# Iamctb/ImageStitching

Measured on AMD Instinct MI355X. Metric: stitched megapixels/sec (9x12 MP vertical), higher is better.
Workload: dtype u8

## Files before the change

imagestitching_amd/__init__.py:

```python
from ._lib import (FILTER_BILINEAR, FILTER_NEAREST, HORIZONTAL, VERTICAL, StitchError, last_error)
from .stitch import (DEFAULT_OPTS, Bitmap, GroupJob, StitchGroup, Stitcher, StitchJob, StitchPlan, decode_files_device, decode_image, decode_png, encode_png, encode_png_batch_device, encode_png_device, encode_jpeg, encode_jpeg_device, encode_jpeg_batch_device, stitch_jpeg, stitch_jpeg_batch, image_info, last_phase_times, plan, set_phase_timing,
                     launch_jobs, stitch, stitch_batch, stitch_files, stitch_png, stitch_png_batch, decode_bitmaps, upload_bitmap, preview_device, preview_fit, thumbnail_layout, thumbnails, thumbnails_device, debug_cells, debug_png_grid, debug_jpeg_gpu_coefficients, scaled_size, decode_scale_fit, thumbnails_from_files, find_overlaps, find_overlaps_device, overlap_rows, crop_overlaps, image_color, icc_tables, convert_color_device)

__all__ = ["stitch", "stitch_batch", "launch_jobs", "stitch_png", "stitch_png_batch", "encode_png", "encode_png_device", "encode_png_batch_device", "encode_jpeg", "encode_jpeg_device", "stitch_jpeg", "decode_png", "decode_image", "decode_files_device", "image_info", "set_phase_timing", "last_phase_times", "stitch_files", "decode_bitmaps", "upload_bitmap", "preview_device", "preview_fit", "thumbnail_layout", "thumbnails", "thumbnails_device", "thumbnails_from_files", "find_overlaps", "find_overlaps_device", "overlap_rows", "crop_overlaps", "image_color", "icc_tables", "convert_color_device", "scaled_size", "decode_scale_fit", "debug_cells", "debug_png_grid", "debug_jpeg_gpu_coefficients", "Bitmap", "plan", "Stitcher", "StitchGroup", "GroupJob", "StitchJob", "StitchPlan", "StitchError",
           "DEFAULT_OPTS"]
```

imagestitching_amd/_lib.py:

```python
import ctypes as C
import os

import torch

_HERE = os.path.dirname(os.path.abspath(__file__))
LIB_PATH = os.path.join(_HERE, "libimagestitch.so")
if os.environ.get("IST_TUNING") == "1" and os.environ.get("IST_LIB_PATH"):
    LIB_PATH = os.environ["IST_LIB_PATH"]

VERTICAL, HORIZONTAL = 0, 1
MODE_MIN, MODE_MAX, MODE_ORIGINAL = 0, 1, 2
PLATFORM_OTHER, PLATFORM_IOS, PLATFORM_ANDROID = 0, 1, 2
FILTER_NEAREST, FILTER_BILINEAR, FILTER_AREA, FILTER_CUBIC = 0, 1, 2, 3
PATH_FILL, PATH_COPY, PATH_SAMPLE, PATH_GENERAL, PATH_SAMPLE_LDS, PATH_SWAP_LDS, PATH_SAMPLE_STREAM, PATH_AREA_STREAM, PATH_CUBIC_STREAM = range(9)
SPLIT_IMAGE, SPLIT_BAND, SPLIT_ROWS, SPLIT_AUTO = 0, 1, 2, 3
THUMB_FILL, THUMB_FIT = 0, 1
TURN_FLIP_X, TURN_FLIP_Y, TURN_TRANSPOSE = 1, 2, 4

IST_OK, IST_NOTHING_TO_DO = 0, 1
ERROR_NAMES = {-1: "IST_E_INVALID", -2: "IST_E_SIZE_UNAVAILABLE", -3: "IST_E_OUTPUT_SIZE", -4: "IST_E_NO_CONTEXT",
               -5: "IST_E_NO_DEVICE", -6: "IST_E_DECODE", -7: "IST_E_UNSUPPORTED", -8: "IST_E_NOMEM", -9: "IST_E_HIP"}


class ImageDesc(C.Structure):
    _fields_ = [("width", C.c_int32), ("height", C.c_int32), ("orientation", C.c_int32),
                ("bmp_width", C.c_int32), ("bmp_height", C.c_int32), ("opaque", C.c_int32),
                ("file_size", C.c_int64)]


class Limits(C.Structure):
    _fields_ = [("platform", C.c_int32), ("reserved", C.c_int32), ("max_side", C.c_double),
                ("max_pixels", C.c_double), ("max_super_sample", C.c_double)]


class Rect(C.Structure):
    _fields_ = [("image", C.c_int32), ("orientation", C.c_int32),
                ("dx", C.c_double), ("dy", C.c_double), ("dw", C.c_double), ("dh", C.c_double)]


class Plan(C.Structure):
    _fields_ = [("out_w", C.c_double), ("out_h", C.c_double), ("scale_down", C.c_double),
                ("super_sample", C.c_double), ("canvas_w", C.c_int64), ("canvas_h", C.c_int64),
                ("big_task", C.c_int32), ("n_rects", C.c_int32), ("rects", C.POINTER(Rect))]


class Op(C.Structure):
    _fields_ = [("kind", C.c_int32), ("image", C.c_int32), ("m", C.c_double * 6), ("s", C.c_double * 4),
                ("d", C.c_double * 4), ("rgba", C.c_uint8 * 4), ("reserved", C.c_int32)]


class Region(C.Structure):
    _fields_ = [("x", C.c_int32), ("y", C.c_int32), ("w", C.c_int32), ("h", C.c_int32)]


class Part(C.Structure):
    _fields_ = [("image", C.c_int32), ("op", C.c_int32), ("slot", C.c_int32),
                ("X0", C.c_int32), ("Y0", C.c_int32), ("X1", C.c_int32), ("Y1", C.c_int32),
                ("sx0", C.c_int32), ("sy0", C.c_int32), ("sx1", C.c_int32), ("sy1", C.c_int32), ("in_place", C.c_int32)]


class FlatCell(C.Structure):
    _fields_ = [("path", C.c_int32), ("image", C.c_int32), ("X0", C.c_int32), ("Y0", C.c_int32), ("X1", C.c_int32), ("Y1", C.c_int32),
                ("src_offset", C.c_int64), ("bg", C.c_uint32), ("opaque", C.c_int32)]


class DebugCell(C.Structure):
    _fields_ = [("path", C.c_int32), ("tile_w", C.c_int32), ("tile_h", C.c_int32), ("sub_h", C.c_int32),
                ("X0", C.c_int32), ("Y0", C.c_int32), ("X1", C.c_int32), ("Y1", C.c_int32), ("tiles", C.c_int64)]


class StitchRequest(C.Structure):
    _fields_ = [("images", C.POINTER(ImageDesc)), ("src", C.POINTER(C.c_void_p)), ("src_pitch", C.POINTER(C.c_size_t)),
                ("n_images", C.c_int32), ("direction", C.c_int32), ("mode", C.c_int32), ("gap", C.c_double),
                ("limits", C.POINTER(Limits)), ("filter", C.c_int32), ("reserved", C.c_int32)]


class JobInfo(C.Structure):
    _fields_ = [("canvas_w", C.c_int64), ("canvas_h", C.c_int64), ("n_ops", C.c_int32), ("n_cells", C.c_int32),
                ("n_tiles", C.c_int64), ("out_pixels", C.c_int64), ("src_pixels_touched", C.c_int64),
                ("algorithmic_bytes", C.c_int64), ("tiles_fill", C.c_int64), ("tiles_copy", C.c_int64),
                ("tiles_sample", C.c_int64), ("tiles_general", C.c_int64)]


class Preview(C.Structure):
    _fields_ = [("box_w", C.c_double), ("box_h", C.c_double), ("width", C.c_int32), ("height", C.c_int32),
                ("pixels", C.POINTER(C.c_uint8))]


class ThumbSpec(C.Structure):
    _fields_ = [("cell_w", C.c_int32), ("cell_h", C.c_int32), ("mode", C.c_int32), ("apply_orientation", C.c_int32)]


class ThumbItem(C.Structure):
    _fields_ = [("width", C.c_int32), ("height", C.c_int32), ("src_x", C.c_int32), ("src_y", C.c_int32), ("src_w", C.c_int32),
                ("src_h", C.c_int32), ("turn", C.c_int32), ("reserved", C.c_int32), ("offset", C.c_int64)]


class OverlapOpts(C.Structure):
    _fields_ = [("tolerance", C.c_int32), ("min_rows", C.c_int32), ("min_informative", C.c_int32), ("reserved", C.c_int32)]


class Overlap(C.Structure):
    _fields_ = [("header", C.c_int32), ("footer", C.c_int32), ("overlap", C.c_int32), ("reserved", C.c_int32), ("cost", C.c_int64)]


class JpegCoefInfo(C.Structure):
    _fields_ = [("ok", C.c_int32), ("launches", C.c_int32), ("ncomp", C.c_int32), ("reserved", C.c_int32),
                ("blocks_x", C.c_int32 * 3), ("blocks_y", C.c_int32 * 3)]


class ColorTables(C.Structure):
    _fields_ = [("kind", C.c_int32), ("mq", (C.c_int32 * 3) * 3), ("dec", (C.c_uint16 * 256) * 3)]


COLOR_PROFILE_IGNORE, COLOR_PROFILE_SRGB = 0, 1
COLOR_NONE, COLOR_IDENTITY, COLOR_CONVERT, COLOR_UNSUPPORTED = 0, 1, 2, 3

SYMBOLS = [
    ("ist_abi_version", C.c_int, []),
    ("ist_last_error", C.c_char_p, []),
    ("ist_device_count", C.c_int, []),
    ("ist_debug_device_allocs", C.c_int64, []),
    ("ist_debug_live_handles", C.c_int, [C.POINTER(C.c_int64)]),
    ("ist_debug_gpu_entropy_files", C.c_int64, []),
    ("ist_debug_gpu_entropy_sync_launches", C.c_int64, []),
    ("ist_debug_jpeg_gpu_coefficients", C.c_int, [C.c_void_p, C.c_char_p, C.c_int64, C.POINTER(C.c_void_p), C.POINTER(C.c_int64), C.POINTER(JpegCoefInfo)]),
    ("ist_debug_direct_images", C.c_int64, []),
    ("ist_debug_host_sink_stitches", C.c_int64, []),
    ("ist_debug_flat_launches", C.c_int64, []),
    ("ist_debug_duplex_stitches", C.c_int64, []),
    ("ist_debug_batch_launches", C.c_int64, []),
    ("ist_debug_png_batch_launches", C.c_int64, []),
    ("ist_limits_default", None, [C.c_int, C.POINTER(Limits)]),
    ("ist_limits_unlimited", None, [C.POINTER(Limits)]),
    ("ist_plan_compute", C.c_int, [C.POINTER(ImageDesc), C.c_int, C.c_int, C.c_int, C.c_double, C.POINTER(Limits), C.POINTER(Plan)]),
    ("ist_plan_free", None, [C.POINTER(Plan)]),
    ("ist_plan_ops", C.c_int, [C.POINTER(Plan), C.POINTER(ImageDesc), C.c_int, C.POINTER(Op), C.POINTER(C.c_int)]),
    ("ist_op_box", C.c_int, [C.POINTER(Op), C.c_int64, C.c_int64, C.c_int, C.POINTER(C.c_int32)]),
    ("ist_debug_flat_form", C.c_int, [C.c_int64, C.c_int64, C.POINTER(C.c_uint8), C.POINTER(Op), C.c_int, C.POINTER(ImageDesc), C.c_int, C.c_int,
                                      C.POINTER(Region), C.POINTER(C.c_int64), C.POINTER(C.c_int64), C.POINTER(FlatCell), C.c_int, C.POINTER(C.c_int)]),
    ("ist_debug_cells", C.c_int, [C.c_int64, C.c_int64, C.POINTER(C.c_uint8), C.POINTER(Op), C.c_int, C.POINTER(ImageDesc), C.c_int, C.c_int,
                                  C.POINTER(Region), C.POINTER(DebugCell), C.c_int, C.POINTER(C.c_int), C.POINTER(C.c_int), C.POINTER(C.c_int)]),
    ("ist_shard_parts", C.c_int, [C.POINTER(Op), C.c_int, C.c_int64, C.c_int64, C.POINTER(ImageDesc), C.c_int, C.c_int, C.c_int, C.c_int,
                                  C.POINTER(Part), C.c_int, C.POINTER(C.c_int)]),
    ("ist_shard_row_cuts", C.c_int, [C.c_int64, C.c_int, C.POINTER(C.c_int32)]),
    ("ist_shard_resolve", C.c_int, [C.POINTER(Op), C.c_int, C.c_int64, C.c_int64, C.POINTER(ImageDesc), C.c_int, C.c_int, C.c_int]),
    ("ist_ctx_create", C.c_void_p, [C.c_int]),
    ("ist_ctx_destroy", None, [C.c_void_p]),
    ("ist_ctx_sync", C.c_int, [C.c_void_p]),
    ("ist_ctx_set_png_level", C.c_int, [C.c_void_p, C.c_int]),
    ("ist_ctx_set_png_color", C.c_int, [C.c_void_p, C.c_int]),
    ("ist_ctx_set_png_filter", C.c_int, [C.c_void_p, C.c_int]),
    ("ist_ctx_set_png_match", C.c_int, [C.c_void_p, C.c_int]),
    ("ist_job_create", C.c_void_p, [C.c_void_p, C.c_int64, C.c_int64, C.POINTER(C.c_uint8), C.POINTER(Op), C.c_int,
                                    C.POINTER(ImageDesc), C.c_int, C.c_int, C.POINTER(Region)]),
    ("ist_job_info_get", C.c_int, [C.c_void_p, C.POINTER(JobInfo)]),
    ("ist_job_preferred_dst_pitch", C.c_size_t, [C.c_void_p]),
    ("ist_job_launch", C.c_int, [C.c_void_p, C.POINTER(C.c_void_p), C.POINTER(C.c_size_t), C.c_int, C.c_void_p, C.c_size_t, C.c_void_p]),
    ("ist_jobs_launch", C.c_int, [C.POINTER(C.c_void_p), C.c_int, C.POINTER(C.c_void_p), C.POINTER(C.c_size_t), C.POINTER(C.c_int),
                                  C.POINTER(C.c_void_p), C.POINTER(C.c_size_t), C.c_void_p]),
    ("ist_job_destroy", None, [C.c_void_p]),
    ("ist_group_create", C.c_void_p, [C.POINTER(C.c_int), C.c_int]),
    ("ist_group_destroy", None, [C.c_void_p]),
    ("ist_group_slots", C.c_int, [C.c_void_p]),
    ("ist_group_device", C.c_int, [C.c_void_p, C.c_int]),
    ("ist_group_job_create", C.c_void_p, [C.c_void_p, C.c_int64, C.c_int64, C.POINTER(C.c_uint8), C.POINTER(Op), C.c_int,
                                          C.POINTER(ImageDesc), C.c_int, C.c_int, C.c_int]),
    ("ist_group_job_destroy", None, [C.c_void_p]),
    ("ist_group_job_parts", C.c_int, [C.c_void_p, C.POINTER(Part), C.c_int, C.POINTER(C.c_int)]),
    ("ist_group_job_launch", C.c_int, [C.c_void_p, C.POINTER(C.c_void_p), C.POINTER(C.c_size_t), C.c_int, C.c_void_p, C.c_size_t]),
    ("ist_group_sync", C.c_int, [C.c_void_p]),
    ("ist_group_stitch_rgba8", C.c_int, [C.c_void_p, C.POINTER(ImageDesc), C.POINTER(C.c_void_p), C.POINTER(C.c_size_t), C.c_int,
                                         C.c_int, C.c_int, C.c_double, C.POINTER(Limits), C.c_int, C.c_int, C.POINTER(Plan),
                                         C.POINTER(C.POINTER(C.c_uint8))]),
    ("ist_stitch_rgba8_multi", C.c_int, [C.POINTER(C.c_int), C.c_int, C.POINTER(ImageDesc), C.POINTER(C.c_void_p), C.POINTER(C.c_size_t), C.c_int,
                                         C.c_int, C.c_int, C.c_double, C.POINTER(Limits), C.c_int, C.c_int, C.POINTER(Plan),
                                         C.POINTER(C.POINTER(C.c_uint8))]),
    ("ist_stitch_rgba8", C.c_int, [C.c_void_p, C.POINTER(ImageDesc), C.POINTER(C.c_void_p), C.POINTER(C.c_size_t), C.c_int,
                                   C.c_int, C.c_int, C.c_double, C.POINTER(Limits), C.c_int, C.POINTER(Plan),
                                   C.POINTER(C.POINTER(C.c_uint8))]),
    ("ist_stitch_rgba8_batch", C.c_int, [C.c_void_p, C.POINTER(StitchRequest), C.c_int, C.POINTER(Plan), C.POINTER(C.POINTER(C.c_uint8))]),
    ("ist_stitch_png_batch", C.c_int, [C.c_void_p, C.POINTER(StitchRequest), C.c_int, C.POINTER(Plan), C.POINTER(C.POINTER(C.c_uint8)),
                                       C.POINTER(C.c_int64)]),
    ("ist_render_rgba8", C.c_int, [C.c_void_p, C.c_int64, C.c_int64, C.POINTER(C.c_uint8), C.POINTER(Op), C.c_int,
                                   C.POINTER(ImageDesc), C.POINTER(C.c_void_p), C.POINTER(C.c_size_t), C.c_int, C.c_int,
                                   C.POINTER(Region), C.c_void_p, C.c_size_t]),
    ("ist_free", None, [C.c_void_p]),
    ("ist_pool_trim", None, []),
    ("ist_png_info", C.c_int, [C.c_void_p, C.c_int64, C.POINTER(C.c_int32), C.POINTER(C.c_int32)]),
    ("ist_png_decode_rgba8", C.c_int, [C.c_void_p, C.c_int64, C.c_void_p, C.c_size_t, C.c_int64]),
    ("ist_jpeg_info", C.c_int, [C.c_void_p, C.c_int64, C.POINTER(C.c_int32), C.POINTER(C.c_int32), C.POINTER(C.c_int32)]),
    ("ist_jpeg_decode_rgba8", C.c_int, [C.c_void_p, C.c_void_p, C.c_int64, C.c_void_p, C.c_size_t, C.c_int64]),
    ("ist_image_info", C.c_int, [C.c_void_p, C.c_int64, C.POINTER(C.c_int32), C.POINTER(C.c_int32), C.POINTER(C.c_int32)]),
    ("ist_image_decode_rgba8", C.c_int, [C.c_void_p, C.c_void_p, C.c_int64, C.c_void_p, C.c_size_t, C.c_int64]),
    ("ist_decode_files_device", C.c_int, [C.c_void_p, C.POINTER(C.c_char_p), C.POINTER(C.c_int64), C.c_int, C.POINTER(C.c_void_p), C.POINTER(C.c_size_t),
                                          C.POINTER(C.c_int64), C.POINTER(ImageDesc)]),
    ("ist_jpeg_scaled_size", C.c_int, [C.c_int32, C.c_int32, C.c_int32, C.POINTER(C.c_int32), C.POINTER(C.c_int32)]),
    ("ist_decode_scale_fit", C.c_int, [C.c_int32, C.c_int32, C.c_int32, C.c_int32]),
    ("ist_image_decode_rgba8_scaled", C.c_int, [C.c_void_p, C.c_void_p, C.c_int64, C.c_int32, C.c_void_p, C.c_size_t, C.c_int64]),
    ("ist_decode_files_device_scaled", C.c_int, [C.c_void_p, C.POINTER(C.c_char_p), C.POINTER(C.c_int64), C.c_int, C.POINTER(C.c_int32),
                                                 C.POINTER(C.c_void_p), C.POINTER(C.c_size_t), C.POINTER(C.c_int64), C.POINTER(ImageDesc)]),
    ("ist_debug_jpeg_scaled_launches", C.c_int64, []),
    ("ist_ctx_set_timing", C.c_int, [C.c_void_p, C.c_int]),
    ("ist_ctx_last_timing", C.c_int, [C.c_void_p, C.POINTER(C.c_double), C.c_int]),
    ("ist_stitch_files_png", C.c_int, [C.c_void_p, C.POINTER(C.c_char_p), C.POINTER(C.c_int64), C.c_int, C.c_int, C.c_int, C.c_double,
                                       C.POINTER(Limits), C.c_int, C.POINTER(Plan), C.POINTER(C.POINTER(C.c_uint8)), C.POINTER(C.c_int64)]),
    ("ist_stitch_paths_png", C.c_int, [C.c_void_p, C.POINTER(C.c_char_p), C.c_int, C.c_int, C.c_int, C.c_double,
                                       C.POINTER(Limits), C.c_int, C.POINTER(Plan), C.POINTER(C.POINTER(C.c_uint8)), C.POINTER(C.c_int64)]),
    ("ist_png_bound", C.c_int64, [C.c_int64, C.c_int64]),
    ("ist_png_encode_device", C.c_int, [C.c_void_p, C.c_void_p, C.c_size_t, C.c_int64, C.c_int64, C.c_void_p, C.c_int64,
                                        C.POINTER(C.c_int64), C.c_void_p]),
    ("ist_png_encode_batch_device", C.c_int, [C.c_void_p, C.POINTER(C.c_void_p), C.POINTER(C.c_size_t), C.POINTER(C.c_int64), C.POINTER(C.c_int64),
                                              C.c_int, C.POINTER(C.c_void_p), C.POINTER(C.c_int64), C.POINTER(C.c_int64), C.c_void_p]),
    ("ist_png_encode_rgba8", C.c_int, [C.c_void_p, C.c_void_p, C.c_size_t, C.c_int64, C.c_int64,
                                       C.POINTER(C.POINTER(C.c_uint8)), C.POINTER(C.c_int64)]),
    ("ist_render_png", C.c_int, [C.c_void_p, C.c_int64, C.c_int64, C.POINTER(C.c_uint8), C.POINTER(Op), C.c_int,
                                 C.POINTER(ImageDesc), C.POINTER(C.c_void_p), C.POINTER(C.c_size_t), C.c_int, C.c_int,
                                 C.POINTER(C.POINTER(C.c_uint8)), C.POINTER(C.c_int64)]),
    ("ist_stitch_png", C.c_int, [C.c_void_p, C.POINTER(ImageDesc), C.POINTER(C.c_void_p), C.POINTER(C.c_size_t), C.c_int,
                                 C.c_int, C.c_int, C.c_double, C.POINTER(Limits), C.c_int, C.POINTER(Plan),
                                 C.POINTER(C.POINTER(C.c_uint8)), C.POINTER(C.c_int64)]),
    ("ist_bitmap_upload", C.c_void_p, [C.c_void_p, C.POINTER(ImageDesc), C.c_void_p, C.c_size_t]),
    ("ist_bitmaps_decode", C.c_int, [C.c_void_p, C.POINTER(C.c_char_p), C.POINTER(C.c_int64), C.c_int, C.POINTER(C.c_void_p)]),
    ("ist_bitmaps_decode_scaled", C.c_int, [C.c_void_p, C.POINTER(C.c_char_p), C.POINTER(C.c_int64), C.c_int, C.POINTER(C.c_int32), C.POINTER(C.c_void_p)]),
    ("ist_bitmap_desc", C.c_int, [C.c_void_p, C.POINTER(ImageDesc)]),
    ("ist_bitmap_download", C.c_int, [C.c_void_p, C.c_void_p, C.c_size_t, C.c_int64]),
    ("ist_bitmap_retain", None, [C.c_void_p]),
    ("ist_bitmap_release", None, [C.c_void_p]),
    ("ist_stitch_bitmaps_rgba8", C.c_int, [C.c_void_p, C.POINTER(C.c_void_p), C.c_int, C.c_int, C.c_int, C.c_double, C.POINTER(Limits), C.c_int,
                                           C.POINTER(Plan), C.POINTER(C.POINTER(C.c_uint8))]),
    ("ist_stitch_bitmaps_png", C.c_int, [C.c_void_p, C.POINTER(C.c_void_p), C.c_int, C.c_int, C.c_int, C.c_double, C.POINTER(Limits), C.c_int,
                                         C.POINTER(Plan), C.POINTER(C.POINTER(C.c_uint8)), C.POINTER(C.c_int64)]),
    ("ist_debug_bitmap_bytes", C.c_int64, []),
    ("ist_preview_fit", C.c_int, [C.c_int64, C.c_int64, C.c_double, C.c_double, C.POINTER(C.c_int32), C.POINTER(C.c_int32)]),
    ("ist_preview_device", C.c_int, [C.c_void_p, C.c_void_p, C.c_size_t, C.c_int64, C.c_int64, C.c_int, C.c_void_p, C.c_size_t,
                                     C.c_int32, C.c_int32, C.c_void_p]),
    ("ist_stitch_png_preview", C.c_int, [C.c_void_p, C.POINTER(ImageDesc), C.POINTER(C.c_void_p), C.POINTER(C.c_size_t), C.c_int,
                                         C.c_int, C.c_int, C.c_double, C.POINTER(Limits), C.c_int, C.POINTER(Plan),
                                         C.POINTER(C.POINTER(C.c_uint8)), C.POINTER(C.c_int64), C.POINTER(Preview)]),
    ("ist_stitch_bitmaps_png_preview", C.c_int, [C.c_void_p, C.POINTER(C.c_void_p), C.c_int, C.c_int, C.c_int, C.c_double, C.POINTER(Limits), C.c_int,
                                                 C.POINTER(Plan), C.POINTER(C.POINTER(C.c_uint8)), C.POINTER(C.c_int64), C.POINTER(Preview)]),
    ("ist_stitch_files_png_preview", C.c_int, [C.c_void_p, C.POINTER(C.c_char_p), C.POINTER(C.c_int64), C.c_int, C.c_int, C.c_int, C.c_double,
                                               C.POINTER(Limits), C.c_int, C.POINTER(Plan), C.POINTER(C.POINTER(C.c_uint8)), C.POINTER(C.c_int64),
                                               C.POINTER(Preview)]),
    ("ist_stitch_paths_png_preview", C.c_int, [C.c_void_p, C.POINTER(C.c_char_p), C.c_int, C.c_int, C.c_int, C.c_double,
                                               C.POINTER(Limits), C.c_int, C.POINTER(Plan), C.POINTER(C.POINTER(C.c_uint8)), C.POINTER(C.c_int64),
                                               C.POINTER(Preview)]),
    ("ist_bitmap_preview", C.c_int, [C.c_void_p, C.c_void_p, C.c_int32, C.c_int32, C.c_void_p, C.c_size_t]),
    ("ist_debug_preview_launches", C.c_int64, []),
    ("ist_debug_preview_geometry", C.c_int, [C.c_int64, C.c_int64, C.c_int32, C.c_int32, C.POINTER(C.c_int32)]),
    ("ist_debug_png_grid", C.c_int, [C.c_int64, C.c_int64, C.c_int, C.POINTER(C.c_int64)]),
    ("ist_thumb_layout", C.c_int, [C.POINTER(ImageDesc), C.c_int, C.POINTER(ThumbSpec), C.POINTER(ThumbItem), C.POINTER(C.c_int64)]),
    ("ist_thumbs_device", C.c_int, [C.c_void_p, C.POINTER(ImageDesc), C.POINTER(C.c_void_p), C.POINTER(C.c_size_t), C.c_int, C.POINTER(ThumbSpec),
                                    C.c_void_p, C.c_int64, C.POINTER(ThumbItem), C.c_void_p]),
    ("ist_bitmaps_thumbs", C.c_int, [C.c_void_p, C.POINTER(C.c_void_p), C.c_int, C.POINTER(ThumbSpec), C.POINTER(ThumbItem),
                                     C.POINTER(C.POINTER(C.c_uint8))]),
    ("ist_debug_thumb_launches", C.c_int64, []),
    ("ist_jpeg_quant_tables", C.c_int, [C.c_int, C.POINTER(C.c_uint8), C.POINTER(C.c_uint8)]),
    ("ist_jpeg_bound", C.c_int64, [C.c_int64, C.c_int64, C.c_int]),
    ("ist_jpeg_encode_device", C.c_int, [C.c_void_p, C.c_void_p, C.c_size_t, C.c_int64, C.c_int64, C.c_int, C.c_int, C.c_void_p, C.c_int64,
                                         C.POINTER(C.c_int64), C.c_void_p]),
    ("ist_jpeg_encode_rgba8", C.c_int, [C.c_void_p, C.c_void_p, C.c_size_t, C.c_int64, C.c_int64, C.c_int, C.c_int,
                                        C.POINTER(C.POINTER(C.c_uint8)), C.POINTER(C.c_int64)]),
    ("ist_stitch_jpeg", C.c_int, [C.c_void_p, C.POINTER(ImageDesc), C.POINTER(C.c_void_p), C.POINTER(C.c_size_t), C.c_int,
                                  C.c_int, C.c_int, C.c_double, C.POINTER(Limits), C.c_int, C.c_int, C.c_int, C.POINTER(Plan),
                                  C.POINTER(C.POINTER(C.c_uint8)), C.POINTER(C.c_int64)]),
    ("ist_stitch_bitmaps_jpeg", C.c_int, [C.c_void_p, C.POINTER(C.c_void_p), C.c_int, C.c_int, C.c_int, C.c_double, C.POINTER(Limits), C.c_int,
                                          C.c_int, C.c_int, C.POINTER(Plan), C.POINTER(C.POINTER(C.c_uint8)), C.POINTER(C.c_int64)]),
    ("ist_debug_jpeg_encode_launches", C.c_int64, []),
    ("ist_jpeg_batch_layout", C.c_int64, [C.POINTER(C.c_int64), C.POINTER(C.c_int64), C.POINTER(C.c_int), C.c_int, C.c_int64, C.c_void_p, C.c_int64]),
    ("ist_jpeg_encode_batch_device", C.c_int, [C.c_void_p, C.POINTER(C.c_void_p), C.POINTER(C.c_size_t), C.POINTER(C.c_int64), C.POINTER(C.c_int64),
                                               C.POINTER(C.c_int), C.POINTER(C.c_int), C.c_int, C.POINTER(C.c_void_p), C.POINTER(C.c_int64),
                                               C.POINTER(C.c_int64), C.c_void_p]),
    ("ist_stitch_jpeg_batch", C.c_int, [C.c_void_p, C.POINTER(StitchRequest), C.c_int, C.POINTER(C.c_int), C.POINTER(C.c_int), C.POINTER(Plan),
                                        C.POINTER(C.POINTER(C.c_uint8)), C.POINTER(C.c_int64)]),
    ("ist_debug_jpeg_batch_launches", C.c_int64, []),
    ("ist_jpeg_optimal_table", C.c_int, [C.POINTER(C.c_int64), C.POINTER(C.c_uint8), C.POINTER(C.c_uint8), C.POINTER(C.c_int)]),
    ("ist_debug_jpeg_histogram_launches", C.c_int64, []),
    ("ist_debug_jpeg_counts", C.c_int, [C.c_void_p, C.POINTER(C.c_int64), C.c_int64]),
# ... 46 lines not shown
```

imagestitching_amd/csrc/ist_ctx.h:

```cpp
#ifndef IST_CTX_H_
#define IST_CTX_H_

#include <hip/hip_runtime_api.h>

#include <atomic>
#include <memory>
#include <mutex>
#include <vector>

#include "ist_jpeg.h"

#include "ist_device.h"
#include "ist_host.h"
#include "ist_internal.h"
#include "ist_launch.h"

struct ist_ctx {
  int device = 0;
  ist::DevBuf scratch_src;
  ist::DevBuf scratch_dst;
  ist::DevBuf scratch_dec;
  ist::DevBuf scratch_huff;
  ist::DevBuf scratch_png;
  ist::DevBuf scratch_file;
  ist::DevBuf scratch_jpg;
  ist::DevBuf scratch_jpg_counts;
  ist::DevBuf scratch_arena;
  ist::DevBuf scratch_ent;
  std::vector<ist::Event> img_event;
  std::vector<ist::DevBuf> img_huff;
  std::unique_ptr<ist::WorkerPool> workers;
  std::vector<ist::ScanBuf> scan_bufs;
  std::vector<ist::ScanBuf> file_bufs;
  ist::Event render_done;
  static constexpr int kTablePool = 32;
  std::vector<ist::DevBuf> table_pool;
  std::mutex table_mu;
  std::mutex mu;
  std::atomic<uint32_t> settings{ist::kDefaultSettings};
  std::unique_ptr<ist::Stager> stager;
  double last_ms[IST_PHASE_COUNT] = {0, 0, 0, 0, 0, 0, 0, 0};
  struct LastUse : ist::Event { ~LastUse() { if (e) (void)hipEventSynchronize(e); } };
  static constexpr int kBatchRing = 4;
  struct BatchSlot { ist::PinnedBuf host; ist::DevBuf dev; bool pending = false; LastUse done; };
  BatchSlot batch_ring[kBatchRing];
  int batch_next = 0;
  std::mutex batch_mu;
  struct BatchHalf {
    ist::DevBuf tab, src, dst;
    ist::DevBuf file;
    ist::Event kernel_done;
    ist::Event read_done;
  };
  BatchHalf batch_half[2];
  ist::DevBuf scratch_prev;
  LastUse prev_done; bool prev_pending = false; hipStream_t prev_last = nullptr;
  ist_job* prev_job = nullptr;
  int64_t prev_job_key[5] = {0, 0, 0, 0, 0};
  std::mutex prev_mu;
  ist::DevBuf prev_out;
  ist::Event prev_ready;
  ist::DevBuf scratch_ovl;
  ist::PinnedBuf ovl_host;
  int64_t ovl_rows = 0;
  size_t ovl_sig_at = 0;
  ist::Stream stream;
  ist::Stream aux;
  ist::Stream render;
  ist::Stream png2;
  ist::Stream prev_stream;
  std::vector<ist::Stream> img_stream;
  std::vector<hipStream_t> streams() const {
    std::vector<hipStream_t> v;
    for (const ist::Stream* s : {&stream, &aux, &render, &png2, &prev_stream}) if (*s) v.push_back(*s);
    for (const ist::Stream& s : img_stream) v.push_back(s);
    return v;
  }
};

namespace ist {
inline Settings settings_of(const ist_ctx* ctx) { return ctx ? settings_unpack(ctx->settings.load(std::memory_order_relaxed)) : Settings{}; }
struct DevTables {
  DevOp* ops = nullptr;
  DevCell* cells = nullptr;
  DevBand* bands = nullptr;
  int32_t* stacks = nullptr;
  DevTile* tiles = nullptr;
};
}

struct ist_job {
  ist_ctx* ctx = nullptr;
  ist::Compiled host;
  std::unique_ptr<ist::FlatTwin> flat;
  ist::DevTables flat_dt;
  ist::DevBuf d_tables;
  static constexpr int kStreams = 4;
  hipStream_t launched_on[kStreams] = {nullptr, nullptr, nullptr, nullptr};
  int n_launched_on = 0;
  bool launched = false, launched_many = false;
  std::mutex launch_mu;
  ist::DevTables dt;
  int max_image = -1;
};

#define IST_HIP(expr) do { const hipError_t e_ = (expr); if (e_ != hipSuccess) return ist::fail(IST_E_HIP, std::string(#expr) + ": " + hipGetErrorString(e_)); } while (0)
#define IST_HIP_OR(expr, msg) do { if ((expr) != hipSuccess) { (void)hipGetLastError(); return ist::fail(IST_E_HIP, msg); } } while (0)

namespace ist {

inline size_t arena_take(size_t* off, size_t bytes) { const size_t at = *off; *off += round256(bytes); return at; }

ist_job* job_compile(ist_ctx* ctx, int64_t canvas_w, int64_t canvas_h, const uint8_t clear_rgba[4], const ist_op* ops, int n_ops,
                     const ist_image_desc* images, int n_images, int filter, const ist_region* clip);
struct TableLayout { size_t bytes[2][5] = {}; size_t at[2][5] = {}; const void* from[2][5] = {}; size_t total = 0; };
TableLayout table_layout(const ist_job& job);
void pack_tables(const TableLayout& L, uint8_t* blob);
void point_tables(ist_job* job, const TableLayout& L, uint8_t* base);
int job_launch_args(const ist_job* job, const void* const* src, const size_t* src_pitch, int n_images, void* dst, size_t dst_pitch,
                    LaunchArgs* out, const Compiled** out_run, bool* out_flat);
void note_launch_stream(ist_job* job, void* stream);
void count_flat_launches(int64_t n);

int batch_take_slot(ist_ctx* ctx, size_t bytes, ist_ctx::BatchSlot** out);

inline Stager& stager_of(ist_ctx* ctx) { if (!ctx->stager) ctx->stager.reset(new Stager(ctx->device)); return *ctx->stager; }
inline WorkerPool& workers_of(ist_ctx* ctx) { if (!ctx->workers) ctx->workers.reset(new WorkerPool()); return *ctx->workers; }
int ensure_aux(ist_ctx* ctx);
int ensure_render(ist_ctx* ctx);
int read_back_pooled(const void* dev, size_t bytes, hipStream_t stream, uint8_t** out);
int png_to_host(ist_ctx* ctx, const PngForm& form, const void* canvas, size_t pitch, int64_t w, int64_t h, void* dfile, uint8_t** out_png, int64_t* out_len,
                const std::function<int(int64_t, void*)>& need_rows = nullptr, int64_t slab_rows_hint = 0, ist_preview* preview = nullptr);

int jpeg_to_host(ist_ctx* ctx, const void* canvas, size_t pitch, int64_t w, int64_t h, int quality, int subsampling, uint8_t** out_jpeg,
                 int64_t* out_len);
int jpeg_check_options(const char* who, int quality, int subsampling);
int jpeg_check_export(const char* who, int64_t w, int64_t h, int quality, int subsampling);

int preview_check(ist_preview* pv);
inline void preview_clear(ist_preview* pv) { if (pv) { pv->width = pv->height = 0; pv->pixels = nullptr; } }
int preview_enqueue(ist_ctx* ctx, const void* src, size_t src_pitch, int64_t w, int64_t h, bool opaque, void* dst, size_t dst_pitch,
                    int32_t pw, int32_t ph, hipStream_t stream);
void bitmap_view(const ist_bitmap* b, int* device, const uint8_t** row0, size_t* pitch, ist_image_desc* desc);
int overlap_run(ist_ctx* ctx, const void* const* src, const size_t* pitch, const ist_image_desc* descs, int n, const ist_overlap_opts* opts,
                ist_overlap* out);
int overlap_check_desc(const ist_image_desc& d, int i);
struct PreviewTail {
  ist_ctx* ctx; const void* canvas; size_t pitch; int64_t w, h; ist_preview* pv;
  int32_t pw = 0, ph = 0;
  uint8_t* host = nullptr;
  bool queued = false;
  PreviewTail(ist_ctx* c, const void* cv, size_t p, int64_t w_, int64_t h_, ist_preview* v) : ctx(c), canvas(cv), pitch(p), w(w_), h(h_), pv(v) {}
  ~PreviewTail();
  int prepare();
  int queue(hipStream_t reader);
  int finish();
};

}

#endif
```

imagestitching_amd/csrc/ist_decode.cpp:

```cpp
#include <hip/hip_runtime_api.h>

#include <algorithm>
#include <atomic>
#include <chrono>
#include <cstdio>
#include <cstdlib>
#include <cstring>
#include <mutex>

#include "ist_decode.h"
#include "ist_webp.h"

using namespace ist;

namespace {
std::atomic<int64_t> g_gpu_entropy_files{0};
std::atomic<int64_t> g_gpu_entropy_sync_launches{0};

void jpeg_layout(const JpegImage& J, size_t* off, JpegDevLayout* L, int denom = 1) {
  std::memset(L, 0, sizeof(*L));
  for (int c = 0; c < J.ncomp; ++c) {
    const JpegComp& C = J.comp[c];
    const size_t nblk = static_cast<size_t>(C.blocks_x) * C.blocks_y;
    const size_t S = denom > 1 ? static_cast<size_t>(jpeg_scaled_idct_size(8 / denom, C.h, C.v, J.hmax, J.vmax)) : 8;
    L->coef[c] = arena_take(off, nblk * 128);
    L->q[c] = arena_take(off, 128);
    L->plane[c] = arena_take(off, nblk * S * S);
  }
}
void jpeg_layout_sparse(const JpegImage& J, size_t* off, JpegDevLayout* L) {
  for (int c = 0; c < J.ncomp; ++c) {
    const JpegComp& C = J.comp[c];
    if (!C.sparse) continue;
    const size_t nblk = static_cast<size_t>(C.blocks_x) * C.blocks_y;
    L->ent[c] = arena_take(off, C.ent.size() * 4 + 4); L->start[c] = arena_take(off, nblk * 4); L->cnt[c] = arena_take(off, nblk);
  }
}

JpegDeviceJob jpeg_device_job(const JpegImage& J, uint8_t* d, const JpegDevLayout& L, uint8_t* d_out, size_t out_pitch) {
  JpegDeviceJob job;
  job.width = J.width; job.height = J.height; job.ncomp = J.ncomp; job.hmax = J.hmax; job.vmax = J.vmax; job.rgb = J.rgb;
  for (int c = 0; c < 3; ++c) { job.d_coef[c] = nullptr; job.q_host[c] = nullptr; job.d_plane[c] = nullptr; job.h[c] = job.v[c] = 1; job.blocks_x[c] = job.blocks_y[c] = 0; }
  for (int c = 0; c < J.ncomp; ++c) {
    const JpegComp& C = J.comp[c];
    job.d_coef[c] = reinterpret_cast<int16_t*>(d + L.coef[c]);
    job.q_host[c] = C.q;
    job.d_plane[c] = d + L.plane[c];
    job.h[c] = C.h; job.v[c] = C.v; job.blocks_x[c] = C.blocks_x; job.blocks_y[c] = C.blocks_y;
  }
  job.out = d_out; job.out_pitch = out_pitch;
  return job;
}

int jpeg_enqueue(const JpegImage& J, uint8_t* d, uint8_t* d_ent, const JpegDevLayout& L, uint8_t* d_out, size_t out_pitch, hipStream_t stream, bool coef_on_device = false,
                 bool chroma_done = false, int denom = 1) {
  JpegDeviceJob job = jpeg_device_job(J, d, L, d_out, out_pitch);
  job.chroma_done = chroma_done; job.denom = denom;
  for (int c = 0; c < J.ncomp; ++c) {
    const JpegComp& C = J.comp[c];
    const size_t nblk = static_cast<size_t>(C.blocks_x) * C.blocks_y;
    int16_t* d_coef = reinterpret_cast<int16_t*>(d + L.coef[c]);
    if (coef_on_device) {
    } else if (C.sparse) {
      IST_HIP(hipMemsetAsync(d_coef, 0, nblk * 128, stream));
      if (!d_ent) return fail(IST_E_INVALID, "JPEG sparse coefficients without a device arena");
      if (!C.ent.empty()) IST_HIP(hipMemcpyAsync(d_ent + L.ent[c], C.ent.data(), C.ent.size() * 4, hipMemcpyHostToDevice, stream));
      IST_HIP(hipMemcpyAsync(d_ent + L.start[c], C.start.data(), nblk * 4, hipMemcpyHostToDevice, stream));
      IST_HIP(hipMemcpyAsync(d_ent + L.cnt[c], C.cnt.data(), nblk, hipMemcpyHostToDevice, stream));
      const int rc = jpeg_launch_scatter(reinterpret_cast<const uint32_t*>(d_ent + L.ent[c]), reinterpret_cast<const uint32_t*>(d_ent + L.start[c]), d_ent + L.cnt[c], d_coef, static_cast<int>(nblk), stream);
      if (rc) return rc;
    } else {
      if (C.coef.size() != nblk * 64) return fail(IST_E_DECODE, "JPEG component without coefficients");
      IST_HIP(hipMemcpyAsync(d_coef, C.coef.data(), nblk * 128, hipMemcpyHostToDevice, stream));
    }
  }
  return denom > 1 ? jpeg_launch_reconstruct_scaled(job, stream) : jpeg_launch_reconstruct(job, stream);
}

bool valid_denom(int d) { return d == 1 || d == 2 || d == 4 || d == 8; }

int jpeg_decode_rgba8(const char* who, ist_ctx* ctx, const uint8_t* file, int64_t len, int denom, uint8_t* out, size_t out_pitch, int64_t out_rows) {
  if (!ctx) return fail(IST_E_NO_CONTEXT, "无法获取绘图上下文");
  JpegImage J;
  int rc = jpeg_parse_and_entropy_decode(file, len, &J, false);
  if (rc) return rc;
  int sw = J.width, sh = J.height;
  jpeg_scaled_size(J.width, J.height, denom, &sw, &sh);
  if (!out || out_pitch < static_cast<size_t>(sw) * 4 || out_rows < sh) return fail(IST_E_INVALID, std::string(who) + ": output buffer too small");
  const bool to_srgb = settings_of(ctx).color_profile == IST_COLOR_PROFILE_SRGB;
  std::lock_guard<std::mutex> lock(ctx->mu);
  DeviceGuard g(ctx->device);
  size_t off = 0;
  JpegDevLayout L;
  jpeg_layout(J, &off, &L, denom);
  jpeg_layout_sparse(J, &off, &L);
  const size_t row = static_cast<size_t>(sw) * 4;
  const size_t o_out = arena_take(&off, row * sh);
  uint8_t* d = nullptr;
  rc = ctx->scratch_arena.grow(off);
  if (rc) return rc;
  d = static_cast<uint8_t*>(ctx->scratch_arena.p);
  rc = jpeg_enqueue(J, d, d, L, d + o_out, row, ctx->stream, false, false, denom);
  if (rc) return rc;
  if (to_srgb) {
    ist_color_tables t;
    if (image_color_tables(file, len, &t) == IST_COLOR_CONVERT) { rc = launch_color_convert(d + o_out, row, sw, sh, t, ctx->stream); if (rc) return rc; }
  }
  std::vector<RowsCopy> down{RowsCopy{d + o_out, nullptr, out, out_pitch, row, static_cast<size_t>(sh)}};
  rc = stager_of(ctx).download(down, ctx->stream);
  (void)hipStreamSynchronize(ctx->stream);
  return rc;
}

bool is_jpeg(const uint8_t* f, int64_t n) { return f && n >= 2 && f[0] == 0xFF && f[1] == 0xD8; }
bool is_misc(const uint8_t* f, int64_t n) { return f && n >= 4 && ((f[0] == 'B' && f[1] == 'M') || !std::memcmp(f, "GIF8", 4)); }
}

extern "C" {

int ist_jpeg_info(const uint8_t* file, int64_t len, int32_t* width, int32_t* height, int32_t* orientation) {
  JpegImage J;
  const int rc = jpeg_parse_and_entropy_decode(file, len, &J, true);
  if (rc) return rc;
  if (width) *width = J.width;
  if (height) *height = J.height;
  if (orientation) *orientation = J.orientation;
  return IST_OK;
}

int ist_jpeg_decode_rgba8(ist_ctx* ctx, const uint8_t* file, int64_t len, uint8_t* out, size_t out_pitch, int64_t out_rows) {
  return jpeg_decode_rgba8("ist_jpeg_decode_rgba8", ctx, file, len, 1, out, out_pitch, out_rows);
}

int ist_misc_info(const uint8_t* file, int64_t len, int32_t* w, int32_t* h);
int ist_misc_decode_rgba8(const uint8_t* file, int64_t len, uint8_t* out, size_t pitch, int64_t out_rows);

int ist_image_info(const uint8_t* file, int64_t len, int32_t* width, int32_t* height, int32_t* orientation) {
  if (is_jpeg(file, len)) return ist_jpeg_info(file, len, width, height, orientation);
  if (is_webp(file, len)) return webp_info(file, len, width, height, orientation);
  if (orientation) *orientation = 0;
  if (is_misc(file, len)) return ist_misc_info(file, len, width, height);
  return ist_png_info(file, len, width, height);
}

int ist_image_decode_rgba8(ist_ctx* ctx, const uint8_t* file, int64_t len, uint8_t* out, size_t out_pitch, int64_t out_rows) {
  if (is_jpeg(file, len)) return ist_jpeg_decode_rgba8(ctx, file, len, out, out_pitch, out_rows);
  if (is_misc(file, len)) return ist_misc_decode_rgba8(file, len, out, out_pitch, out_rows);
  if (is_webp(file, len)) return webp_decode_rgba8(file, len, out, out_pitch, out_rows);
  return ist_png_decode_rgba8(file, len, out, out_pitch, out_rows);
}

int ist_image_decode_rgba8_scaled(ist_ctx* ctx, const uint8_t* file, int64_t len, int32_t denom, uint8_t* out, size_t out_pitch, int64_t out_rows) {
  if (!valid_denom(denom)) return fail(IST_E_INVALID, "ist_image_decode_rgba8_scaled: the file's denominator " + std::to_string(denom) + " is not 1, 2, 4 or 8");
  if (is_jpeg(file, len)) return jpeg_decode_rgba8("ist_image_decode_rgba8_scaled", ctx, file, len, denom, out, out_pitch, out_rows);
  return ist_image_decode_rgba8(ctx, file, len, out, out_pitch, out_rows);
}

int ist_jpeg_scaled_size(int32_t w, int32_t h, int32_t denom, int32_t* sw, int32_t* sh) {
  if (w < 1 || h < 1 || !valid_denom(denom) || !sw || !sh) return fail(IST_E_INVALID, "ist_jpeg_scaled_size: bad argument");
  int a = 0, b = 0;
  jpeg_scaled_size(w, h, denom, &a, &b);
  *sw = a; *sh = b;
  return IST_OK;
}

int ist_decode_scale_fit(int32_t w, int32_t h, int32_t min_w, int32_t min_h) {
  if (w < 1 || h < 1 || min_w < 1 || min_h < 1) return fail(IST_E_INVALID, "ist_decode_scale_fit: bad argument");
  for (int d = 8; d > 1; d /= 2)
    if ((static_cast<int64_t>(w) + d - 1) / d >= min_w && (static_cast<int64_t>(h) + d - 1) / d >= min_h) return d;
  return 1;
}

}

namespace ist {

Phases::Phases(ist_ctx* c, bool timing) : ctx(c), record(timing) {
  static const bool env = std::getenv("IST_TIMING") != nullptr;
  print = env; on = env || record;
  if (record) for (double& v : c->last_ms) v = 0.0;
  t_prev = std::chrono::steady_clock::now();
}
void Phases::lap(int phase, const char* what, hipStream_t st) {
  if (!on) return;
  if (st) (void)hipStreamSynchronize(st);
  const auto t = std::chrono::steady_clock::now();
  const double ms = std::chrono::duration<double, std::milli>(t - t_prev).count();
  if (print) std::fprintf(stderr, "[ist timing] %-28s %8.2f ms\n", what, ms);
  if (record && phase >= 0 && phase < IST_PHASE_COUNT) ctx->last_ms[phase] += ms;
  t_prev = t;
}

constexpr int kImgStreams = 8;

static int ensure_image_lanes(ist_ctx* ctx, int n) {
  const size_t want = static_cast<size_t>(std::min(n, kImgStreams));
  while (ctx->img_stream.size() < want) {
    Stream st;
    const int rc = st.ensure();
    if (rc) return rc;
    ctx->img_stream.push_back(std::move(st));
  }
  while (ctx->img_event.size() < static_cast<size_t>(n)) {
    Event ev;
    const int rc = ev.ensure();
    if (rc) return rc;
    ctx->img_event.push_back(std::move(ev));
  }
  if (ctx->img_huff.size() < static_cast<size_t>(n)) ctx->img_huff.resize(static_cast<size_t>(n));
  if (ctx->scan_bufs.size() < static_cast<size_t>(n)) ctx->scan_bufs.resize(static_cast<size_t>(n));
  return IST_OK;
}

FileDecoder::FileDecoder(ist_ctx* ctx, const uint8_t* const* files, const int64_t* lens, int n, Phases* ph, int color_profile, const int32_t* denom)
    : ctx_(ctx), files_(files), lens_(lens), n_(n), ph_(ph), to_srgb_(color_profile == IST_COLOR_PROFILE_SRGB), denom_(denom), dec_(static_cast<size_t>(n)),
      on_gpu_(static_cast<size_t>(n), 0), taken_(static_cast<size_t>(n), 0), uploaded_(static_cast<size_t>(n), 0), started_(static_cast<size_t>(n), 0),
      chroma_done_(static_cast<size_t>(n), 0), jo_(static_cast<size_t>(n)) {}
FileDecoder::~FileDecoder() {
  join_all();
  for (int i = 0; i < n_; ++i) if (started_[static_cast<size_t>(i)]) (void)hipStreamSynchronize(stream_of(i));
  for (int i = 0; i < n_ && static_cast<size_t>(i) < ctx_->scan_bufs.size(); ++i) {
    ScanBuf& mine = dec_[static_cast<size_t>(i)].G.stream;
    if (mine.capacity() > ctx_->scan_bufs[static_cast<size_t>(i)].capacity() && mine.capacity() <= (8u << 20)) ctx_->scan_bufs[static_cast<size_t>(i)].swap(mine);
  }
}

int FileDecoder::headers() {
  static const bool gpu_huffman = std::getenv("IST_JPEG_HOST_HUFFMAN") == nullptr;
  gpu_huffman_ = gpu_huffman;
  for (int i = 0; i < n_; ++i) {
    Dec& D = dec_[static_cast<size_t>(i)];
    const uint8_t* f = files_[i]; const int64_t len = lens_[i];
    D.jpeg = is_jpeg(f, len);
    int rc;
    if (D.jpeg) {
      rc = jpeg_parse_and_entropy_decode(f, len, &D.J, true);
      D.w = D.J.width; D.h = D.J.height; D.orient = D.J.orientation;
    } else {
      int32_t w = 0, h = 0, o = 0;
      rc = ist_image_info(f, len, &w, &h, &o);
      D.w = w; D.h = h; D.orient = o;
    }
    if (rc != IST_OK) return fail(rc, "图片" + std::to_string(i) + "解码异常: " + g_last_error);
  }
  return IST_OK;
}
std::vector<ist_image_desc> FileDecoder::descs(const int64_t* lens) const {
  std::vector<ist_image_desc> descs(static_cast<size_t>(n_));
  for (int i = 0; i < n_; ++i) {
    const Dec& D = dec(i);
    ist_image_desc& d = descs[static_cast<size_t>(i)];
    std::memset(&d, 0, sizeof d);
    d.width = D.w; d.height = D.h; d.orientation = D.orient ? D.orient : 1; d.opaque = D.jpeg ? 1 : 0; d.file_size = lens[i];
    if (denom_of(i) > 1) { int sw = 0, sh = 0; jpeg_scaled_size(D.w, D.h, denom_of(i), &sw, &sh); d.bmp_width = sw; d.bmp_height = sh; }
  }
  return descs;
}
void FileDecoder::layout(size_t* off) { for (int i = 0; i < n_; ++i) if (dec_[static_cast<size_t>(i)].jpeg) jpeg_layout(dec_[static_cast<size_t>(i)].J, off, &jo_[static_cast<size_t>(i)], denom_of(i)); }
int FileDecoder::denom_of(int i) const { return denom_ && dec_[static_cast<size_t>(i)].jpeg ? denom_[i] : 1; }

int FileDecoder::start(uint8_t* arena, uint8_t* const* img, const size_t* pitch) {
  arena_ = arena; img_ = img; pitch_ = pitch;
  const int rc = ensure_image_lanes(ctx_, n_);
  if (rc) return rc;
  workers_of(ctx_).run(n_, [this](int i) { worker(i); });
  running_ = true;
  if (!ph_->on) return IST_OK;
  join_all();
  int rc2 = first_error(); if (rc2) return rc2;
  for (int i = 0; i < n_; ++i) if (uploaded_[static_cast<size_t>(i)]) (void)hipStreamSynchronize(stream_of(i));
  ph_->lap(IST_PHASE_HOST_DECODE, "decode on host threads (+ scan uploads)", nullptr);
  rc2 = huffman_all(ctx_->stream); if (rc2) return rc2;
  ph_->lap(IST_PHASE_ENTROPY_GPU, "entropy decode (GPU)", ctx_->stream);
  for (int i = 0; i < n_; ++i) { rc2 = take(i, ctx_->stream); if (rc2) return rc2; }
  ph_->lap(IST_PHASE_RECONSTRUCT, "H2D + JPEG reconstruct (GPU)", ctx_->stream);
  return IST_OK;
}

int FileDecoder::take(int i, hipStream_t consumer) {
  const size_t k = static_cast<size_t>(i);
  if (taken_[k]) return IST_OK;
  int rc = huffman_all(consumer);
  if (rc) return rc;
  rc = chroma_all(consumer);
  if (rc) return rc;
  taken_[k] = 1;
  rc = place(i, consumer);
  if (rc) return rc;
  const Dec& D = dec_[k];
  if (!to_srgb_ || D.color.kind != IST_COLOR_CONVERT) return IST_OK;
  int bw = D.w, bh = D.h;
  if (denom_of(i) > 1) jpeg_scaled_size(D.w, D.h, denom_of(i), &bw, &bh);
  return launch_color_convert(img_[i], pitch_[i], bw, bh, D.color, consumer);
}

int FileDecoder::place(int i, hipStream_t consumer) {
  const size_t k = static_cast<size_t>(i);
  int rc = IST_OK;
  Dec& D = dec_[k];
  if (on_gpu_[k]) return jpeg_enqueue(D.J, arena_, nullptr, jo_[k], img_[i], pitch_[i], consumer, true, chroma_done_[k] != 0, denom_of(i));
  const size_t row = static_cast<size_t>(D.w) * 4;
  if (!D.jpeg) {
    std::vector<RowsCopy> up;
    if (pitch_[i] != row) for (int y = 0; y < D.h; ++y) up.push_back(RowsCopy{img_[i] + static_cast<size_t>(y) * pitch_[i], D.px.data() + static_cast<size_t>(y) * row, nullptr, row, row, 1});
    else up.push_back(RowsCopy{img_[i], D.px.data(), nullptr, row, row, static_cast<size_t>(D.h)});
    return stager_of(ctx_).upload(up, consumer);
  }
  if (D.G.eligible) {
    D.G.eligible = false;
    JpegImage host;
    rc = jpeg_parse_and_entropy_decode(files_[i], lens_[i], &host, false, nullptr);
    if (rc) return fail(rc, "图片" + std::to_string(i) + "解码异常: " + g_last_error);
    D.J = std::move(host);
  }
  size_t need = 0;
  JpegDevLayout L = jo_[k];
  jpeg_layout_sparse(D.J, &need, &L);
  if (need) {
    (void)hipStreamSynchronize(consumer);
    rc = ctx_->scratch_ent.grow(need, need / 2);
    if (rc) return rc;
  }
  return jpeg_enqueue(D.J, arena_, static_cast<uint8_t*>(ctx_->scratch_ent.p), L, img_[i], pitch_[i], consumer, false, false, denom_of(i));
}

int FileDecoder::finish(hipStream_t consumer) {
  for (int i = 0; i < n_; ++i) { const int rc = take(i, consumer); if (rc) { join_all(); return rc; } }
  return IST_OK;
}
int FileDecoder::gpu_decoded() const { int g = 0; for (char v : on_gpu_) g += v ? 1 : 0; return g; }

hipStream_t FileDecoder::stream_of(int i) const { return ctx_->img_stream[static_cast<size_t>(i % kImgStreams) % ctx_->img_stream.size()]; }
void FileDecoder::join_all() { if (running_) { ctx_->workers->wait(); running_ = false; } }
int FileDecoder::first_error() {
  for (int i = 0; i < n_; ++i) if (dec_[static_cast<size_t>(i)].rc != IST_OK) return fail(dec_[static_cast<size_t>(i)].rc, "图片" + std::to_string(i) + "解码异常: " + dec_[static_cast<size_t>(i)].err);
  return IST_OK;
}
int FileDecoder::huffman_all(hipStream_t consumer) {
  if (huff_done_) return IST_OK;
  tl_mark("decoder: waiting for the per-image host work");
  join_all();
  tl_mark("decoder: host work of every image done");
  int rc = first_error();
  if (rc) return rc;
  huff_done_ = true;
  std::vector<JpegGpuItem> items; std::vector<int> who;
  for (int i = 0; i < n_; ++i) {
    const size_t k = static_cast<size_t>(i);
    Dec& D = dec_[k];
    if (!D.jpeg || !D.G.eligible) continue;
    JpegGpuItem it; it.J = &D.J; it.S = &D.G;
    for (int c = 0; c < 3; ++c) it.d_coef[c] = c < D.J.ncomp ? reinterpret_cast<int16_t*>(arena_ + jo_[k].coef[c]) : nullptr;
    if (uploaded_[k]) {
      it.d_stream = static_cast<const uint8_t*>(ctx_->img_huff[k].p);
      IST_HIP_OR(hipStreamWaitEvent(consumer, ctx_->img_event[k], 0), "hipStreamWaitEvent failed");
    }
    items.push_back(it); who.push_back(i);
  }
  std::vector<uint8_t> okv;
  int launches = 0;
  rc = jpeg_gpu_entropy_decode(items, &okv, consumer, &ctx_->scratch_huff, &launches);
  g_gpu_entropy_sync_launches.fetch_add(launches, std::memory_order_relaxed);
  if (rc) return rc;
  for (size_t q = 0; q < who.size(); ++q) {
    on_gpu_[static_cast<size_t>(who[q])] = okv[q] ? 1 : 0;
    if (okv[q]) g_gpu_entropy_files.fetch_add(1, std::memory_order_relaxed);
  }
  return IST_OK;
}
int FileDecoder::chroma_all(hipStream_t consumer) {
  if (chroma_batch_done_) return IST_OK;
  chroma_batch_done_ = true;
  std::vector<JpegDeviceJob> chroma;
  for (int i = 0; i < n_; ++i) {
    const size_t k = static_cast<size_t>(i);
    if (!on_gpu_[k] || dec_[k].J.ncomp != 3 || denom_of(i) > 1) continue;
    chroma.push_back(jpeg_device_job(dec_[k].J, arena_, jo_[k], nullptr, 0));
    chroma_done_[k] = 1;
  }
  if (!chroma.empty()) return jpeg_launch_chroma_idct(chroma.data(), static_cast<int>(chroma.size()), consumer);
  return IST_OK;
}
void FileDecoder::worker(int i) {
  const size_t k = static_cast<size_t>(i);
  Dec& D = dec_[k];
  DeviceGuard dg(ctx_->device);
  const uint8_t* f = files_[i]; const int64_t len = lens_[i];
  auto failed = [&](int rc) { D.rc = rc; D.err = g_last_error; };
  if (to_srgb_) image_color_tables(f, len, &D.color);
  if (!D.jpeg) {
    D.px.resize(static_cast<size_t>(D.w) * D.h * 4);
    const int rc = ist_image_decode_rgba8(nullptr, f, len, D.px.data(), static_cast<size_t>(D.w) * 4, D.h);
    if (rc) failed(rc);
    return;
  }
  JpegImage full;
  if (k < ctx_->scan_bufs.size()) D.G.stream.swap(ctx_->scan_bufs[k]);
  static const bool flip = tuning_mode() && std::getenv("IST_JPEG_SECOND_READ_444") != nullptr;
  std::vector<uint8_t> flipped;
  if (flip) {
    flipped.assign(f, f + len);
    for (int64_t q = 2; q + 12 < len; ++q) if (flipped[static_cast<size_t>(q)] == 0xFF && flipped[static_cast<size_t>(q) + 1] == 0xC0) { flipped[static_cast<size_t>(q) + 11] = 0x11; break; }
    f = flipped.data();
  }
  const int rc = jpeg_parse_and_entropy_decode(f, len, &full, false, gpu_huffman_ ? &D.G : nullptr);
  if (rc) { failed(rc); return; }
  bool same = full.width == D.w && full.height == D.h && full.ncomp == D.J.ncomp && full.hmax == D.J.hmax && full.vmax == D.J.vmax &&
              full.mcus_x == D.J.mcus_x && full.mcus_y == D.J.mcus_y;
  for (int c = 0; same && c < full.ncomp; ++c)
    same = full.comp[c].h == D.J.comp[c].h && full.comp[c].v == D.J.comp[c].v && full.comp[c].blocks_x == D.J.comp[c].blocks_x &&
           full.comp[c].blocks_y == D.J.comp[c].blocks_y;
  if (!same) { g_last_error = "JPEG frame header changed between two reads"; failed(IST_E_DECODE); return; }
  D.J = std::move(full);
  if (!D.G.eligible) return;
  const size_t bytes = D.G.stream.size();
  if (ctx_->img_huff[k].grow(bytes, bytes / 4)) return;
  hipStream_t st = stream_of(i);
  started_[k] = 1;
  if (hipMemcpyAsync(ctx_->img_huff[k].p, D.G.stream.data(), bytes, hipMemcpyHostToDevice, st) != hipSuccess ||
      hipEventRecord(ctx_->img_event[k], st) != hipSuccess) { (void)hipGetLastError(); return; }
  uploaded_[k] = 1;
}

int check_denoms(const char* who, const int32_t* denom, int n) {
  for (int i = 0; denom && i < n; ++i)
    if (!valid_denom(denom[i])) return fail(IST_E_INVALID, std::string(who) + ": the denominator of image " + std::to_string(i) + " is " + std::to_string(denom[i]) + ", not 1, 2, 4 or 8");
  return IST_OK;
}

int decode_files_locked(ist_ctx* ctx, const uint8_t* const* files, const int64_t* lens, int n, const int32_t* denom,
                        const std::function<int(const std::vector<ist_image_desc>&, uint8_t**, size_t*)>& place) {
  DeviceGuard g(ctx->device);
  const Settings set = settings_of(ctx);
  Phases ph(ctx, set.timing);
  FileDecoder fd(ctx, files, lens, n, &ph, set.color_profile, denom);
  int rc = fd.headers();
  if (rc) return rc;
  const std::vector<ist_image_desc> descs = fd.descs(lens);
  std::vector<uint8_t*> img(static_cast<size_t>(n), nullptr);
  std::vector<size_t> pitch(static_cast<size_t>(n), 0);
  rc = place(descs, img.data(), pitch.data());
  if (rc) return rc;
  size_t off = 0;
  fd.layout(&off);
  rc = ctx->scratch_dec.grow(off ? off : 256);
  if (rc) return rc;
  ph.lap(IST_PHASE_PLAN_ARENA, "device arena", nullptr);
  rc = fd.start(static_cast<uint8_t*>(ctx->scratch_dec.p), img.data(), pitch.data());
  if (rc == IST_OK) rc = fd.finish(ctx->stream);
  if (hipStreamSynchronize(ctx->stream) != hipSuccess) { (void)hipGetLastError(); if (rc == IST_OK) rc = fail(IST_E_HIP, "hipStreamSynchronize failed"); }
  return rc;
}

}

extern "C" {

int64_t ist_debug_gpu_entropy_files(void) { return g_gpu_entropy_files.load(std::memory_order_relaxed); }
int64_t ist_debug_gpu_entropy_sync_launches(void) { return g_gpu_entropy_sync_launches.load(std::memory_order_relaxed); }

int ist_debug_jpeg_gpu_coefficients(ist_ctx* ctx, const uint8_t* file, int64_t len, int16_t* const* planes, const int64_t* plane_elems,
                                    ist_jpeg_coef_info* info) {
  if (!file || len <= 0 || !info || (planes && !plane_elems)) return fail(IST_E_INVALID, "ist_debug_jpeg_gpu_coefficients: bad argument");
  std::memset(info, 0, sizeof *info);
  JpegImage J;
  JpegGpuScan G;
  int rc = jpeg_parse_and_entropy_decode(file, len, &J, false, &G);
  if (rc) return rc;
  if (!G.eligible) return fail(IST_E_UNSUPPORTED, "ist_debug_jpeg_gpu_coefficients: not a file the GPU entropy decoder takes");
  info->ncomp = J.ncomp;
  for (int c = 0; c < J.ncomp; ++c) { info->blocks_x[c] = J.comp[c].blocks_x; info->blocks_y[c] = J.comp[c].blocks_y; }
  if (!planes) return IST_OK;
  size_t off = 0, o_coef[3] = {0, 0, 0}, nblk[3] = {0, 0, 0};
  for (int c = 0; c < J.ncomp; ++c) {
    nblk[c] = static_cast<size_t>(J.comp[c].blocks_x) * J.comp[c].blocks_y;
    if (!planes[c] || plane_elems[c] < 0 || static_cast<uint64_t>(plane_elems[c]) < nblk[c] * 64) return fail(IST_E_INVALID, "ist_debug_jpeg_gpu_coefficients: plane " + std::to_string(c) + " is too small");
    o_coef[c] = arena_take(&off, nblk[c] * 128);
  }
  if (!ctx) return fail(IST_E_NO_CONTEXT, "无法获取绘图上下文");
  std::lock_guard<std::mutex> lock(ctx->mu);
  DeviceGuard g(ctx->device);
  rc = ctx->scratch_arena.grow(off);
  if (rc) return rc;
  uint8_t* d = static_cast<uint8_t*>(ctx->scratch_arena.p);
  JpegGpuItem it; it.J = &J; it.S = &G;
  for (int c = 0; c < 3; ++c) it.d_coef[c] = c < J.ncomp ? reinterpret_cast<int16_t*>(d + o_coef[c]) : nullptr;
  std::vector<JpegGpuItem> items(1, it);
  std::vector<uint8_t> okv;
  int launches = 0;
  rc = jpeg_gpu_entropy_decode(items, &okv, ctx->stream, &ctx->scratch_huff, &launches);
  g_gpu_entropy_sync_launches.fetch_add(launches, std::memory_order_relaxed);
  if (rc) return rc;
  info->launches = launches;
  info->ok = !okv.empty() && okv[0] ? 1 : 0;
  if (info->ok)
    for (int c = 0; c < J.ncomp; ++c) IST_HIP(hipMemcpyAsync(planes[c], d + o_coef[c], nblk[c] * 128, hipMemcpyDeviceToHost, ctx->stream));
  IST_HIP(hipStreamSynchronize(ctx->stream));
  return IST_OK;
}

int ist_ctx_set_color_profile(ist_ctx* ctx, int profile) {
  if (!ctx) return fail(IST_E_NO_CONTEXT, "无法获取绘图上下文");
  return settings_set(&ctx->settings, kColorProfile, profile);
}

int ist_color_convert_device(ist_ctx* ctx, void* ptr, size_t pitch, int64_t w, int64_t h, const ist_color_tables* tables, void* stream) {
  if (!ctx) return fail(IST_E_NO_CONTEXT, "无法获取绘图上下文");
  if (!ptr || !tables || w < 1 || h < 1) return fail(IST_E_INVALID, "ist_color_convert_device: bad argument");
  if (pitch / 4 < static_cast<uint64_t>(w) || (pitch & 3) || (reinterpret_cast<uintptr_t>(ptr) & 3)) return fail(IST_E_INVALID, "ist_color_convert_device: a short or unaligned pitch, or an unaligned pointer");
  if (tables->kind == IST_COLOR_IDENTITY) return IST_OK;
  if (tables->kind != IST_COLOR_CONVERT) return fail(IST_E_INVALID, "ist_color_convert_device: the tables are neither IST_COLOR_CONVERT nor IST_COLOR_IDENTITY");
  DeviceGuard g(ctx->device);
  return launch_color_convert(static_cast<uint8_t*>(ptr), pitch, w, h, *tables, stream);
}

int ist_ctx_set_timing(ist_ctx* ctx, int on) {
  if (!ctx) return fail(IST_E_NO_CONTEXT, "无法获取绘图上下文");
  return settings_set(&ctx->settings, kTiming, on != 0);
}

int ist_ctx_last_timing(ist_ctx* ctx, double* ms, int n) {
  if (!ctx || !ms || n < 0) return fail(IST_E_INVALID, "ist_ctx_last_timing: bad argument");
  for (int k = 0; k < n; ++k) ms[k] = k < IST_PHASE_COUNT ? ctx->last_ms[k] : 0.0;
  return IST_OK;
}

int ist_decode_files_device_scaled(ist_ctx* ctx, const uint8_t* const* files, const int64_t* lens, int n_images, const int32_t* denom, void* const* dst,
                                   const size_t* dst_pitch, const int64_t* dst_rows, ist_image_desc* out_descs) {
  if (!ctx) return fail(IST_E_NO_CONTEXT, "无法获取绘图上下文");
  if (n_images <= 0) return IST_NOTHING_TO_DO;
  if (!files || !lens || !dst || !dst_pitch || !dst_rows) return fail(IST_E_INVALID, "ist_decode_files_device: NULL argument");
  if (n_images > kMaxImages) return fail(IST_E_UNSUPPORTED, "more than 128 images in one call");
  const int rc = check_denoms("ist_decode_files_device_scaled", denom, n_images);
  if (rc) return rc;
  std::lock_guard<std::mutex> lock(ctx->mu);
  return decode_files_locked(ctx, files, lens, n_images, denom, [&](const std::vector<ist_image_desc>& descs, uint8_t** img, size_t* pitch) -> int {
    for (int i = 0; i < n_images; ++i) {
      const ist_image_desc& D = descs[static_cast<size_t>(i)];
      const int bw = bitmap_w(D), bh = bitmap_h(D);
      if (!dst[i] || dst_pitch[i] < static_cast<size_t>(bw) * 4 || (dst_pitch[i] & 3) || dst_rows[i] < bh || (reinterpret_cast<uintptr_t>(dst[i]) & 3))
        return fail(IST_E_INVALID, "ist_decode_files_device: the buffer of image " + std::to_string(i) + " is too small for " + std::to_string(bw) + "x" + std::to_string(bh));
      img[i] = static_cast<uint8_t*>(dst[i]);
      pitch[i] = dst_pitch[i];
      if (out_descs) out_descs[i] = D;
    }
    return IST_OK;
  });
}

int ist_decode_files_device(ist_ctx* ctx, const uint8_t* const* files, const int64_t* lens, int n_images, void* const* dst,
                            const size_t* dst_pitch, const int64_t* dst_rows, ist_image_desc* out_descs) {
  return ist_decode_files_device_scaled(ctx, files, lens, n_images, nullptr, dst, dst_pitch, dst_rows, out_descs);
}

}
```

imagestitching_amd/csrc/ist_decode.h:

```cpp
#ifndef IST_DECODE_H_
#define IST_DECODE_H_

#include <chrono>
#include <functional>
#include <string>
#include <vector>

#include "ist_ctx.h"
#include "ist_icc.h"

namespace ist {

struct Dec { int rc = 0; std::string err; bool jpeg = false; JpegImage J; JpegGpuScan G; int w = 0, h = 0, orient = 0; std::vector<uint8_t> px;
             ist_color_tables color = {}; };

struct Phases {
  ist_ctx* ctx; bool record, print, on;
  std::chrono::steady_clock::time_point t_prev;
  Phases(ist_ctx* c, bool timing);
  void lap(int phase, const char* what, hipStream_t st);
};

struct JpegDevLayout { size_t coef[3], q[3], plane[3], ent[3], start[3], cnt[3]; };

class FileDecoder {
 public:
  FileDecoder(ist_ctx* ctx, const uint8_t* const* files, const int64_t* lens, int n, Phases* ph, int color_profile, const int32_t* denom = nullptr);
  ~FileDecoder();
  int headers();
  const Dec& dec(int i) const { return dec_[static_cast<size_t>(i)]; }
  std::vector<ist_image_desc> descs(const int64_t* lens) const;
  void layout(size_t* off);
  int start(uint8_t* arena, uint8_t* const* img, const size_t* pitch);
  int take(int i, hipStream_t consumer);
  int finish(hipStream_t consumer);
  int gpu_decoded() const;

 private:
  hipStream_t stream_of(int i) const;
  int denom_of(int i) const;
  void join_all();
  int first_error();
  int huffman_all(hipStream_t consumer);
  int chroma_all(hipStream_t consumer);
  void worker(int i);
  int place(int i, hipStream_t consumer);

  ist_ctx* ctx_; const uint8_t* const* files_; const int64_t* lens_; int n_; Phases* ph_; const bool to_srgb_; const int32_t* denom_;
  std::vector<Dec> dec_;
  bool running_ = false;
  std::vector<char> on_gpu_, taken_, uploaded_, started_, chroma_done_;
  std::vector<JpegDevLayout> jo_;
  uint8_t* arena_ = nullptr; uint8_t* const* img_ = nullptr; const size_t* pitch_ = nullptr;
  bool gpu_huffman_ = true, huff_done_ = false, chroma_batch_done_ = false;
};

int check_denoms(const char* who, const int32_t* denom, int n);
int decode_files_locked(ist_ctx* ctx, const uint8_t* const* files, const int64_t* lens, int n, const int32_t* denom,
                        const std::function<int(const std::vector<ist_image_desc>&, uint8_t**, size_t*)>& place);

}

#endif
```

imagestitching_amd/csrc/ist_jpeg.cpp:

```cpp
#include <cstdlib>
#include <cstring>
#include <new>
#include <vector>

#include "ist_internal.h"
#include "ist_icc.h"
#include "ist_jpeg.h"

#include <emmintrin.h>

namespace ist {

namespace {

const uint8_t kZigzag[64] = {0, 1, 8, 16, 9, 2, 3, 10, 17, 24, 32, 25, 18, 11, 4, 5, 12, 19, 26, 33, 40, 48,
                             41, 34, 27, 20, 13, 6, 7, 14, 21, 28, 35, 42, 49, 56, 57, 50, 43, 36, 29, 22,
                             15, 23, 30, 37, 44, 51, 58, 59, 52, 45, 38, 31, 39, 46, 53, 60, 61, 54, 47, 55, 62, 63};

struct Huff {
  bool present = false;
  uint8_t bits[17] = {0};
  uint8_t vals[256] = {0};
  int32_t maxcode[18];
  int32_t valptr[17];
// ... 121 lines not shown
    if (jfif) J->rgb = false;
    else if (adobe) J->rgb = adobe_transform == 0;
    else J->rgb = J->comp[0].id == 'R' && J->comp[1].id == 'G' && J->comp[2].id == 'B';
  };
  auto latch = [&](int c) -> bool {
    if (latched[c]) return true;
    if (!have_q[J->comp[c].tq]) return false;
    std::memcpy(J->comp[c].q, qt[J->comp[c].tq], sizeof J->comp[c].q);
    latched[c] = true;
    return true;
  };
  int64_t pos = 2;
  *J = JpegImage();
  while (pos + 4 <= n) {
    if (f[pos] != 0xFF) { ++pos; continue; }
    const int m = f[pos + 1];
    if (m == 0xFF) { ++pos; continue; }
    if (m == 0xD8 || m == 0x01 || (m >= 0xD0 && m <= 0xD7)) { pos += 2; continue; }
    if (m == 0xD9) break;
    const int64_t len = be16(f + pos + 2);
    if (len < 2 || pos + 2 + len > n) return fail(IST_E_DECODE, "truncated JPEG segment");
    const uint8_t* d = f + pos + 4; const int64_t dl = len - 2;
    if (m == 0xE1 && J->orientation == 0) J->orientation = exif_orientation(d, static_cast<size_t>(dl));
    else if (m == 0xE0 && dl >= 14 && std::memcmp(d, "JFIF\0", 5) == 0) jfif = true;
    else if (m == 0xEE && dl >= 12 && std::memcmp(d, "Adobe", 5) == 0) { adobe = true; adobe_transform = d[11]; }
    else if (m == 0xDB) {
      int64_t o = 0;
      while (o < dl) {
        const int pq = d[o] >> 4, tq = d[o] & 15; ++o;
        if (tq > 3 || o + (pq ? 128 : 64) > dl) return fail(IST_E_DECODE, "bad JPEG quantisation table");
        for (int i = 0; i < 64; ++i) { qt[tq][kZigzag[i]] = static_cast<uint16_t>(pq ? be16(d + o + 2 * i) : d[o + i]); }
        o += pq ? 128 : 64;
        have_q[tq] = true;
      }
    } else if (m == 0xC4) {
      int64_t o = 0;
      while (o + 17 <= dl) {
        const int tc = d[o] >> 4, th = d[o] & 15;
        if (tc > 1 || th > 3) return fail(IST_E_DECODE, "bad JPEG Huffman table");
        Huff& h = tc ? ac[th] : dc[th];
        int cnt = 0;
        for (int i = 1; i <= 16; ++i) { h.bits[i] = d[o + i]; cnt += h.bits[i]; }
        if (cnt > 256 || o + 17 + cnt > dl) return fail(IST_E_DECODE, "bad JPEG Huffman table");
        std::memcpy(h.vals, d + o + 17, static_cast<size_t>(cnt));
        h.present = true;
        if (!h.build()) return fail(IST_E_DECODE, "bad JPEG Huffman table");
        o += 17 + cnt;
      }
    } else if (m == 0xDD) { if (dl >= 2) restart_interval = static_cast<int>(be16(d)); }
    else if (m == 0xC0 || m == 0xC1 || m == 0xC2) {
      if (have_sof) return fail(IST_E_DECODE, "JPEG with more than one frame header");
      progressive = (m == 0xC2);
      if (dl < 6) return fail(IST_E_DECODE, "bad JPEG frame header");
      if (d[0] != 8) return fail(IST_E_UNSUPPORTED, "only 8-bit JPEG is supported");
      J->height = static_cast<int>(be16(d + 1)); J->width = static_cast<int>(be16(d + 3)); J->ncomp = d[5];
      if (J->width < 1 || J->height < 1) return fail(IST_E_DECODE, "bad JPEG size");
      if (J->ncomp != 1 && J->ncomp != 3) return fail(IST_E_UNSUPPORTED, "only greyscale and YCbCr JPEG are supported");
      if (dl < 6 + 3 * J->ncomp) return fail(IST_E_DECODE, "bad JPEG frame header");
      int hmax = 1, vmax = 1;
      for (int c = 0; c < J->ncomp; ++c) {
        JpegComp& C = J->comp[c];
        C.id = d[6 + 3 * c]; C.h = d[7 + 3 * c] >> 4; C.v = d[7 + 3 * c] & 15; C.tq = d[8 + 3 * c];
        if (C.h < 1 || C.h > 2 || C.v < 1 || C.v > 2 || C.tq > 3) return fail(IST_E_UNSUPPORTED, "JPEG sampling factors beyond 2 are not supported");
        hmax = std::max(hmax, C.h); vmax = std::max(vmax, C.v);
        for (int p = 0; p < c; ++p) if (J->comp[p].id == C.id) return fail(IST_E_DECODE, "JPEG frame names a component twice");
      }
      if (J->ncomp == 3 && (J->comp[1].h != 1 || J->comp[1].v != 1 || J->comp[2].h != 1 || J->comp[2].v != 1))
        return fail(IST_E_UNSUPPORTED, "unusual JPEG sampling layout (chroma must be 1x1)");
      if (J->ncomp == 1) { J->comp[0].h = J->comp[0].v = 1; hmax = vmax = 1; }
      colour_space();
      J->hmax = hmax; J->vmax = vmax;
      J->mcus_x = (J->width + 8 * hmax - 1) / (8 * hmax); J->mcus_y = (J->height + 8 * vmax - 1) / (8 * vmax);
      for (int c = 0; c < J->ncomp; ++c) {
        JpegComp& C = J->comp[c];
        C.blocks_x = J->mcus_x * C.h; C.blocks_y = J->mcus_y * C.v;
      }
      have_sof = true;
      if (header_only) return IST_OK;
    } else if (m >= 0xC3 && m <= 0xCF && m != 0xC4 && m != 0xC8 && m != 0xCC) return fail(IST_E_UNSUPPORTED, "this JPEG process (lossless / arithmetic) is not supported");
    else if (m == 0xDA) {
      if (!have_sof) return fail(IST_E_DECODE, "JPEG scan before frame header");
      if (J->scans == 0) colour_space();
      if (dl < 1) return fail(IST_E_DECODE, "bad JPEG scan header");
      const int ns = d[0];
      if (ns < 1 || ns > J->ncomp || dl < 1 + 2 * ns + 3) return fail(IST_E_DECODE, "bad JPEG scan header");
      int ci[3], td[3], ta[3];
      for (int s = 0; s < ns; ++s) {
        const int id = d[1 + 2 * s]; ci[s] = -1;
        for (int c = 0; c < J->ncomp; ++c) if (J->comp[c].id == id) ci[s] = c;
        if (ci[s] < 0) return fail(IST_E_DECODE, "JPEG scan names an unknown component");
        for (int p = 0; p < s; ++p) if (ci[p] == ci[s]) return fail(IST_E_DECODE, "JPEG scan names a component twice");
        td[s] = d[2 + 2 * s] >> 4; ta[s] = d[2 + 2 * s] & 15;
        if (td[s] > 3 || ta[s] > 3) return fail(IST_E_DECODE, "JPEG scan uses an undefined Huffman table");
      }
      const int Ss = d[1 + 2 * ns], Se = d[2 + 2 * ns], Ah = d[3 + 2 * ns] >> 4, Al = d[3 + 2 * ns] & 15;
      if (progressive) {
        if (Ss > Se || Se > 63 || Al > 13 || Ah > 13 || (Ss == 0 && Se != 0) || (Ss > 0 && ns != 1) || (Ah != 0 && Ah != Al + 1))
          return fail(IST_E_DECODE, "bad progressive JPEG scan parameters");
      } else if (Ss != 0 || Se != 63 || Ah != 0 || Al != 0) return fail(IST_E_DECODE, "bad JPEG scan parameters");
      const bool dc_scan = Ss == 0, need_ac = !progressive || !dc_scan, need_dc = dc_scan && Ah == 0;
      for (int s = 0; s < ns; ++s) {
        if ((need_dc && !dc[td[s]].present) || (need_ac && !ac[ta[s]].present)) return fail(IST_E_DECODE, "JPEG scan uses an undefined Huffman table");
      }
      int mcu_blocks = 0;
      for (int s2 = 0; s2 < ns; ++s2) mcu_blocks += J->comp[ci[s2]].h * J->comp[ci[s2]].v;
      int dc_ids[2] = {-1, -1}, ac_ids[2] = {-1, -1}, dc_local[4] = {0, 0, 0, 0}, ac_local[4] = {0, 0, 0, 0};
      bool two_tables = true;
      for (int s2 = 0; s2 < ns; ++s2) {
        auto local = [&](int (&ids)[2], int id) { for (int q = 0; q < 2; ++q) { if (ids[q] == id) return q; if (ids[q] < 0) { ids[q] = id; return q; } } return -1; };
        dc_local[s2] = local(dc_ids, td[s2]); ac_local[s2] = local(ac_ids, ta[s2]);
        if (dc_local[s2] < 0 || ac_local[s2] < 0) two_tables = false;
      }
      if (gs && !progressive && J->scans == 0 && ns == J->ncomp && two_tables && mcu_blocks <= 10 &&
          (f + n) - (d + dl) < (1ll << 28)) {
        for (int c = 0; c < J->ncomp; ++c)
          if (!latch(c)) return fail(IST_E_DECODE, "JPEG component uses an undefined quantisation table");
        gs->slots = 0;
        for (int s2 = 0; s2 < ns; ++s2) {
          const JpegComp& C = J->comp[ci[s2]];
          for (int k = 0; k < C.h * C.v; ++k) { gs->slot_comp[gs->slots] = static_cast<uint8_t>(ci[s2]); gs->slot_idx[gs->slots] = static_cast<uint8_t>(k); ++gs->slots; }
          gs->dc_tab[ci[s2]] = static_cast<uint8_t>(dc_local[s2]); gs->ac_tab[ci[s2]] = static_cast<uint8_t>(ac_local[s2]);
        }
        std::memset(&gs->tables, 0, sizeof gs->tables);
        for (int t = 0; t < 4; ++t) {
          const bool is_ac = t >= 2;
          const int id = is_ac ? ac_ids[t - 2] : dc_ids[t];
          if (id < 0) continue;
          const Huff& h = is_ac ? ac[id] : dc[id];
          const int look_bits = is_ac ? kJpegAcLookBits : kJpegDcLookBits;
          uint16_t* look = is_ac ? gs->tables.look_ac[t - 2] : gs->tables.look_dc[t];
          int code = 0, k = 0;
          for (int l = 1; l <= look_bits; ++l) {
            for (int i = 0; i < h.bits[l]; ++i, ++k, ++code) {
              const uint16_t e = static_cast<uint16_t>((l << 8) | h.vals[k]);
              uint16_t* at = look + (static_cast<size_t>(code) << (look_bits - l));
              std::fill(at, at + (size_t{1} << (look_bits - l)), e);
            }
            code <<= 1;
          }
          JpegHuffTail& o = gs->tables.tail[t];
          for (int q = 0; q < 8; ++q) {
            const int l = 9 + q;
            o.lim[q] = static_cast<uint32_t>(h.mincode[l] + h.bits[l]) << (16 - l);
            if (q < 7) o.vptr[q] = static_cast<uint8_t>(h.valptr[l + 1]);
          }
          std::memcpy(o.vals, h.vals, sizeof o.vals);
        }
        const uint8_t* q = d + dl; const uint8_t* qe = f + n;
        gs->iv.clear();
        const uint32_t total_mcus = static_cast<uint32_t>(J->mcus_x) * static_cast<uint32_t>(J->mcus_y);
        const uint32_t ri = static_cast<uint32_t>(restart_interval);
        const uint32_t n_iv = ri ? (total_mcus + ri - 1) / ri : 0;
        bool in_sequence = n_iv <= kMaxGpuIntervals;
        gs->stream.clear();
        if (in_sequence && !gs->stream.reserve(static_cast<size_t>(qe - q) + static_cast<size_t>(n_iv) * 272 + 32)) return fail(IST_E_NOMEM, "out of memory for the JPEG scan");
        uint8_t* const base = gs->stream.data();
        uint8_t* out = base;
        size_t iv_start = 0; uint32_t next_rst = 0;
        auto close_interval = [&]() {
          const uint32_t k = static_cast<uint32_t>(gs->iv.size());
          const size_t at = static_cast<size_t>(out - base);
          JpegGpuInterval I;
          I.byte_off = static_cast<uint32_t>(iv_start); I.mcu0 = k * ri; I.n_mcus = std::min(ri, total_mcus - k * ri);
          I.bits = static_cast<int64_t>(at - iv_start) * 8;
          gs->iv.push_back(I);
          size_t pad = (256 - at % 256) % 256;
          if (pad < 16) pad += 256;
          std::memset(out, 0, pad);
          out += pad;
          iv_start = at + pad;
        };
        const __m128i all_ff = _mm_set1_epi8(static_cast<char>(0xFF));
        while (in_sequence && q < qe) {
          while (q + 16 <= qe) {
            const __m128i v = _mm_loadu_si128(reinterpret_cast<const __m128i*>(q));
            _mm_storeu_si128(reinterpret_cast<__m128i*>(out), v);
            const int m = _mm_movemask_epi8(_mm_cmpeq_epi8(v, all_ff));
            if (m) { const int k = __builtin_ctz(static_cast<unsigned>(m)); q += k; out += k; break; }
            q += 16; out += 16;
          }
          if (q >= qe) break;
          if (*q != 0xFF) { *out++ = *q++; continue; }
          if (q + 1 < qe && q[1] == 0x00) { *out++ = 0xFF; q += 2; continue; }
          if (q + 1 < qe && q[1] == 0xFF) { q += 1; continue; }
          if (q + 1 < qe && q[1] >= 0xD0 && q[1] <= 0xD7) {
            if (!ri || q[1] != 0xD0 + next_rst || gs->iv.size() + 1 >= n_iv) { in_sequence = false; break; }
            close_interval();
            next_rst = (next_rst + 1) & 7u;
            q += 2;
            continue;
          }
          break;
        }
        if (in_sequence && ri) {
          close_interval();
          if (gs->iv.size() != n_iv) in_sequence = false;
        }
        if (in_sequence) {
          if (ri) {
            gs->bits = static_cast<int64_t>(out - base) * 8;
          } else {
            gs->bits = static_cast<int64_t>(out - base) * 8;
            std::memset(out, 0, 16);
            out += 16;
          }
          gs->stream.set_size(static_cast<size_t>(out - base));
          gs->eligible = true;
          pos = q - f;
          J->scans++;
          continue;
        }
        gs->stream.clear(); gs->iv.clear();
      }
      for (int s = 0; s < ns; ++s)
        if (!latch(ci[s])) return fail(IST_E_DECODE, "JPEG component uses an undefined quantisation table");
      for (int c = 0; c < J->ncomp; ++c) {
        JpegComp& C = J->comp[c];
        const size_t nblk = static_cast<size_t>(C.blocks_x) * C.blocks_y;
        if (progressive) {
          if (C.coef.empty() && !C.coef.alloc_zero(nblk * 64)) return fail(IST_E_NOMEM, "out of memory for the JPEG coefficients");
        } else if (!C.sparse) {
          C.sparse = true;
          C.start.assign(nblk, 0); C.cnt.assign(nblk, 0);
          C.ent.reserve(2 * static_cast<size_t>(n) + 1024);
        }
      }
      BitReader br; br.p = d + dl; br.end = f + n;
      int pred[3] = {0, 0, 0}, eobrun = 0;
      const bool interleaved = ns > 1;
      int mx, my;
      if (interleaved) { mx = J->mcus_x; my = J->mcus_y; }
      else {
        const JpegComp& C = J->comp[ci[0]];
        mx = (((J->width * C.h + J->hmax - 1) / J->hmax) + 7) / 8;
        my = (((J->height * C.v + J->vmax - 1) / J->vmax) + 7) / 8;
      }
      int until_restart = restart_interval, next_rst = 0;
      for (int y = 0; y < my; ++y) {
        for (int x = 0; x < mx; ++x) {
          if (restart_interval && until_restart == 0) {
            br.reset();
            while (br.p + 1 < br.end && !(br.p[0] == 0xFF && br.p[1] >= 0xD0 && br.p[1] <= 0xD7)) ++br.p;
            if (br.p + 1 >= br.end) return fail(IST_E_DECODE, "JPEG restart marker missing");
            if ((br.p[1] & 7) != next_rst) return fail(IST_E_DECODE, "JPEG restart markers out of order");
            br.p += 2; next_rst = (next_rst + 1) & 7;
            pred[0] = pred[1] = pred[2] = 0; eobrun = 0;
            until_restart = restart_interval;
          }
          for (int s = 0; s < ns; ++s) {
            JpegComp& C = J->comp[ci[s]];
            const int bh = interleaved ? C.h : 1, bv = interleaved ? C.v : 1;
            for (int by = 0; by < bv; ++by) for (int bx = 0; bx < bh; ++bx) {
              const int gx = x * bh + bx, gy = y * bv + by;
              const size_t bi = static_cast<size_t>(gy) * C.blocks_x + gx;
              int16_t* blk = progressive ? C.coef.data() + bi * 64 : nullptr;
              if (!progressive) {
                const size_t first = C.ent.size();
                C.ent.resize(first + 64);
                uint32_t* e = C.ent.data() + first;
                int t = decode_symbol(br, dc[td[s]]);
                if (t < 0 || t > 11) return fail(IST_E_DECODE, "corrupt JPEG entropy data (DC)");
                const int diff = t ? extend(br.get(t), t) : 0;
                pred[s] += diff;
                if (pred[s]) *e++ = static_cast<uint32_t>(static_cast<uint16_t>(static_cast<int16_t>(pred[s])));
                const Huff& hac = ac[ta[s]];
                for (int k = 1; k < 64;) {
                  const int fa = hac.fast_ac[br.peek(16) >> 7];
                  if (fa) {
                    k += (fa >> 4) & 15;
                    if (k > 63) return fail(IST_E_DECODE, "corrupt JPEG entropy data (run)");
                    br.skip(fa & 15);
                    *e++ = (static_cast<uint32_t>(kZigzag[k]) << 16) | static_cast<uint16_t>(static_cast<int16_t>(fa >> 8));
                    ++k;
                    continue;
                  }
                  const int rs = decode_symbol(br, hac);
                  if (rs < 0) return fail(IST_E_DECODE, "corrupt JPEG entropy data (AC)");
                  const int r = rs >> 4, sz = rs & 15;
                  if (sz == 0) { if (r == 15) { k += 16; continue; } break; }
                  k += r;
                  if (k > 63) return fail(IST_E_DECODE, "corrupt JPEG entropy data (run)");
                  const int v = extend(br.get(sz), sz);
                  if (v) *e++ = (static_cast<uint32_t>(kZigzag[k]) << 16) | static_cast<uint16_t>(static_cast<int16_t>(v));
                  ++k;
                }
                const size_t used = static_cast<size_t>(e - (C.ent.data() + first));
                C.ent.resize(first + used);
                C.start[bi] = static_cast<uint32_t>(first);
                C.cnt[bi] = static_cast<uint8_t>(used);
              } else if (dc_scan && Ah == 0) {
                const int t = decode_symbol(br, dc[td[s]]);
                if (t < 0 || t > 11) return fail(IST_E_DECODE, "corrupt JPEG entropy data (DC)");
                pred[s] += t ? extend(br.get(t), t) : 0;
                blk[0] = static_cast<int16_t>(pred[s] * (1 << Al));
              } else if (dc_scan) {
                if (br.get(1)) blk[0] = static_cast<int16_t>(blk[0] | (1 << Al));
              } else if (Ah == 0) {
                if (eobrun > 0) { --eobrun; continue; }
                for (int k = Ss; k <= Se;) {
                  const int rs = decode_symbol(br, ac[ta[s]]);
                  if (rs < 0) return fail(IST_E_DECODE, "corrupt JPEG entropy data (AC)");
                  const int r = rs >> 4, sz = rs & 15;
                  if (sz == 0) {
                    if (r == 15) { k += 16; continue; }
                    eobrun = (1 << r) - 1;
                    if (r) eobrun += static_cast<int>(br.get(r));
                    break;
                  }
                  k += r;
                  if (k > Se) return fail(IST_E_DECODE, "corrupt JPEG entropy data (run)");
                  blk[kZigzag[k]] = static_cast<int16_t>(extend(br.get(sz), sz) * (1 << Al));
                  ++k;
                }
              } else {
                const int p1 = 1 << Al, m1 = -(1 << Al);
                auto refine = [&](int16_t* c) {
                  if (br.get(1) && (*c & p1) == 0) *c = static_cast<int16_t>(*c + (*c >= 0 ? p1 : m1));
                };
                int k = Ss;
                if (eobrun == 0) {
                  for (; k <= Se; ++k) {
                    const int rs = decode_symbol(br, ac[ta[s]]);
                    if (rs < 0) return fail(IST_E_DECODE, "corrupt JPEG entropy data (AC)");
                    int r = rs >> 4, val = 0;
                    const int sz = rs & 15;
                    if (sz) {
                      if (sz != 1) return fail(IST_E_DECODE, "corrupt JPEG entropy data (refinement)");
                      val = br.get(1) ? p1 : m1;
                    } else if (r != 15) {
                      eobrun = 1 << r;
                      if (r) eobrun += static_cast<int>(br.get(r));
                      break;
                    }
                    for (; k <= Se; ++k) {
                      int16_t* c = blk + kZigzag[k];
                      if (*c != 0) refine(c);
                      else if (--r < 0) break;
                    }
                    if (val) {
                      if (k > Se) return fail(IST_E_DECODE, "corrupt JPEG entropy data (run)");
                      blk[kZigzag[k]] = static_cast<int16_t>(val);
                    }
                  }
                }
                if (eobrun > 0) {
                  for (; k <= Se; ++k) { int16_t* c = blk + kZigzag[k]; if (*c != 0) refine(c); }
                  --eobrun;
                }
              }
            }
          }
// ... 64 lines not shown
```

imagestitching_amd/csrc/ist_jpeg.h:

```cpp
#ifndef IST_JPEG_H_
#define IST_JPEG_H_

#include <cstdint>
#include <cstdlib>
#include <utility>
#include <vector>

namespace ist {

class CoefBuf {
 public:
  CoefBuf() = default;
  ~CoefBuf() { std::free(p_); }
  CoefBuf(const CoefBuf&) = delete;
  CoefBuf& operator=(const CoefBuf&) = delete;
  CoefBuf(CoefBuf&& o) noexcept : p_(o.p_), n_(o.n_) { o.p_ = nullptr; o.n_ = 0; }
  CoefBuf& operator=(CoefBuf&& o) noexcept { if (this != &o) { std::free(p_); p_ = o.p_; n_ = o.n_; o.p_ = nullptr; o.n_ = 0; } return *this; }
  bool alloc_zero(size_t n) { std::free(p_); p_ = static_cast<int16_t*>(std::calloc(n ? n : 1, sizeof(int16_t))); n_ = p_ ? n : 0; return p_ != nullptr; }
  bool empty() const { return n_ == 0; }
  size_t size() const { return n_; }
  int16_t* data() { return p_; }
  const int16_t* data() const { return p_; }
  const int16_t* begin() const { return p_; }
  const int16_t* end() const { return p_ + n_; }
 private:
  int16_t* p_ = nullptr; size_t n_ = 0;
};

struct JpegComp {
  int id = 0, h = 1, v = 1, tq = 0;
  int blocks_x = 0, blocks_y = 0;
  uint16_t q[64];
  CoefBuf coef;
  bool sparse = false;
  std::vector<uint32_t> ent, start;
  std::vector<uint8_t> cnt;
};

struct JpegImage {
  int width = 0, height = 0, ncomp = 0;
  int hmax = 1, vmax = 1, mcus_x = 0, mcus_y = 0;
  int orientation = 0;
  int scans = 0;
  bool rgb = false;
  JpegComp comp[3];
};

struct alignas(16) JpegHuffTail {
  uint32_t lim[8];
  uint8_t vptr[8];
  uint8_t pad_[8];
  uint8_t vals[256];
};
#ifndef IST_AC_LOOK_BITS
#define IST_AC_LOOK_BITS 9
#endif
constexpr int kJpegDcLookBits = 9, kJpegAcLookBits = IST_AC_LOOK_BITS;
struct alignas(16) JpegGpuTables {
  uint16_t look_dc[2][1 << kJpegDcLookBits];
  uint16_t look_ac[2][1 << kJpegAcLookBits];
  JpegHuffTail tail[4];
};
struct JpegGpuInterval { uint32_t byte_off, mcu0, n_mcus; int64_t bits; };
class ScanBuf {
 public:
  ScanBuf() = default;
  ~ScanBuf() { std::free(p_); }
  ScanBuf(const ScanBuf&) = delete;
  ScanBuf& operator=(const ScanBuf&) = delete;
  ScanBuf(ScanBuf&& o) noexcept { swap(o); }
  ScanBuf& operator=(ScanBuf&& o) noexcept { swap(o); return *this; }
  void swap(ScanBuf& o) noexcept { std::swap(p_, o.p_); std::swap(n_, o.n_); std::swap(cap_, o.cap_); }
  const uint8_t* data() const { return p_; }
  uint8_t* data() { return p_; }
  size_t size() const { return n_; }
  size_t capacity() const { return cap_; }
  bool empty() const { return n_ == 0; }
  void clear() { n_ = 0; }
  void set_size(size_t n) { n_ = n; }
  bool reserve(size_t want) {
    if (want <= cap_) return true;
    std::free(p_);
    p_ = static_cast<uint8_t*>(std::malloc(want)); cap_ = p_ ? want : 0; n_ = 0;
    return p_ != nullptr;
  }
 private:
  uint8_t* p_ = nullptr; size_t n_ = 0, cap_ = 0;
};
struct JpegGpuScan {
  bool eligible = false;
  std::vector<JpegGpuInterval> iv;
  ScanBuf stream;
  int64_t bits = 0;
  int slots = 0;
  uint8_t slot_comp[10], slot_idx[10];
  uint8_t dc_tab[3], ac_tab[3];
  JpegGpuTables tables;
};

int jpeg_parse_and_entropy_decode(const uint8_t* file, int64_t len, JpegImage* out, bool header_only, JpegGpuScan* gpu_scan = nullptr);

struct JpegDeviceJob {
  int width, height, ncomp, hmax, vmax;
  int h[3], v[3], blocks_x[3], blocks_y[3];
  const int16_t* d_coef[3];
  const uint16_t* q_host[3];
  uint8_t* d_plane[3];
  bool rgb = false;
  uint8_t* out; size_t out_pitch;
  bool chroma_done = false;
  int denom = 1;
};
inline void jpeg_scaled_size(int w, int h, int denom, int* sw, int* sh) {
  const int64_t N = 8 / denom;
  *sw = static_cast<int>((w * N + 7) / 8); *sh = static_cast<int>((h * N + 7) / 8);
}
inline int jpeg_scaled_idct_size(int N, int h, int v, int hmax, int vmax) {
  int S = N;
  while (S < 8 && (hmax * N) % (h * S * 2) == 0 && (vmax * N) % (v * S * 2) == 0) S *= 2;
  return S;
}
int jpeg_launch_reconstruct_scaled(const JpegDeviceJob& job, void* stream);
int jpeg_launch_reconstruct(const JpegDeviceJob& job, void* stream);
int jpeg_launch_chroma_idct(const JpegDeviceJob* jobs, int n_jobs, void* stream);
int jpeg_launch_scatter(const uint32_t* d_ent, const uint32_t* d_start, const uint8_t* d_cnt, int16_t* d_coef, int n_blocks, void* stream);
std::vector<int16_t> jpeg_dense_coefficients(const JpegComp& c);

struct JpegGpuItem { const JpegImage* J; const JpegGpuScan* S; int16_t* d_coef[3]; const uint8_t* d_stream = nullptr; };
struct DevBuf;
int jpeg_gpu_entropy_decode(const std::vector<JpegGpuItem>& items, std::vector<uint8_t>* ok, void* stream, DevBuf* scratch = nullptr,
                            int* launches = nullptr);

}

#endif
```

imagestitching_amd/csrc/ist_jpeg_gpu.hip:

```cpp
#include <hip/hip_runtime.h>

#include <chrono>
#include <cstdio>
#include <cstdlib>
#include <cstring>
#include <string>
#include <vector>

#include "ist_host.h"
#include "ist_internal.h"
#include "ist_jpeg.h"

namespace ist {

namespace {

#ifndef IST_SUB_BITS
#define IST_SUB_BITS 1024
#endif
constexpr int kSubBits = IST_SUB_BITS;
#ifndef IST_SYNC_THREADS
#define IST_SYNC_THREADS 128
#endif
constexpr int kSyncThreads = IST_SYNC_THREADS;
// ... 424 lines not shown
      uint32_t sp = 0, scz = 0;
      if (live && i != 0) {
        const bool has_left = e > kGhosts - n_ghost;
        if (A.pass == 0) {
          if (it == 0 || !has_left) { sp = i * static_cast<uint32_t>(kSubBits); scz = 0; }
          else { sp = ex_p[e - 1]; scz = ex_cz[e - 1]; }
        } else {
          if (it == 0 || tid == 0) { sp = A.in_p[g - 1]; scz = A.in_cz[g - 1]; }
          else { sp = ex_p[e - 1]; scz = ex_cz[e - 1]; }
        }
      }
      const bool redo = live && !(have && st_p == sp && st_cz == scz);
      if (redo) {
        State S; S.p = sp; S.c = scz >> 8; S.z = scz & 255u;
        T = run_count(&sh, fast, pair, first_bit, S, limit, i * static_cast<uint32_t>(kSubBits) + kCheckBits, have, my_p, my_cz, T, ck
#ifdef IST_SYNC_DEBUG
                      , dbg_iters
#endif
                      );
        my_p = S.p; my_cz = (S.c << 8) | S.z;
        st_p = sp; st_cz = scz; have = true;
      }
      __syncthreads();
      if (live) { ex_p[e] = my_p; ex_cz[e] = my_cz; }
#ifdef IST_SYNC_DEBUG
      {
        const uint64_t now = wall_clock64();
        if (it == 0) { dbg_pass0 = now; dbg_c1 = clock64(); atomicMax(&dbg_max_iters, dbg_iters & 0xFFFFu); atomicAdd(&dbg_miss, dbg_iters >> 16); } else dbg_longest = max(dbg_longest, now - dbg_prev);
        dbg_prev = now; ++dbg_passes;
        dbg_redo_lanes += __syncthreads_count(redo ? 1 : 0);
      }
#endif
      if (!__syncthreads_or(redo ? 1 : 0)) { settled = true; break; }
    }
#ifdef IST_SYNC_DEBUG
    if (A.pass == 0 && tid == 0 && blockIdx.x < 8192) {
      uint32_t* q = g_sync_dbg + 8 * blockIdx.x;
      q[0] = dbg_passes; q[1] = static_cast<uint32_t>(wall_clock64() - dbg_t0); q[2] = static_cast<uint32_t>(dbg_staged - dbg_t0);
      q[3] = static_cast<uint32_t>(dbg_pass0 - dbg_staged); q[4] = static_cast<uint32_t>(dbg_longest); q[5] = dbg_redo_lanes;
      q[6] = static_cast<uint32_t>(dbg_c1 - dbg_c0); q[7] = dbg_max_iters | 0x80000000u | (min(dbg_miss, 0x7FFFu) << 16);
    }
#endif
  }
  if (live && owned) {
    atomicAdd(&tot[tid >> 7][0], T.blocks); atomicAdd(&tot[tid >> 7][1], static_cast<uint32_t>(T.dc[0]));
    atomicAdd(&tot[tid >> 7][2], static_cast<uint32_t>(T.dc[1])); atomicAdd(&tot[tid >> 7][3], static_cast<uint32_t>(T.dc[2]));
  }
  __syncthreads();
  if (tid < 4 * kHalves) A.half_total[(kHalves * blockIdx.x + (tid >> 2)) * 4 + (tid & 3)] = tot[tid >> 2][tid & 3];
  if (!live || !owned) return;
  const bool last = tid == kSyncThreads - 1 || i + 1 == static_cast<uint32_t>(sh.img.n_sub);
  if (A.pass == 0 || !settled || (last && (A.in_p[g] != my_p || A.in_cz[g] != my_cz))) {
    if (A.pass == 0 ? (tid == 0) : true) *A.changed = 1u;
  }
  A.out_p[g] = my_p; A.out_cz[g] = my_cz;
  A.tally[4 * g] = T.blocks; A.tally[4 * g + 1] = static_cast<uint32_t>(T.dc[0]); A.tally[4 * g + 2] = static_cast<uint32_t>(T.dc[1]); A.tally[4 * g + 3] = static_cast<uint32_t>(T.dc[2]);
  A.start_p[g] = st_p; A.start_cz[g] = st_cz;
  uint32_t* q = A.checks + 6 * static_cast<size_t>(g);
  q[0] = ck.p; q[1] = ck.cz; q[2] = ck.t.blocks; q[3] = static_cast<uint32_t>(ck.t.dc[0]); q[4] = static_cast<uint32_t>(ck.t.dc[1]); q[5] = static_cast<uint32_t>(ck.t.dc[2]);
}

struct WriteArgs { const DevImg* imgs; const uint16_t* sub_img; const uint32_t* p; const uint32_t* cz; const uint32_t* tally; const uint32_t* half_total; };

__global__ __launch_bounds__(kWriteThreads) void ist_jpeg_write_kernel(const WriteArgs A) {
  __shared__ WgShared<kWriteThreads> sh;
  __shared__ uint32_t slots[kWriteThreads * 33];
  uint32_t (*sc)[kWriteThreads] = reinterpret_cast<uint32_t (*)[kWriteThreads]>(slots);
  static_assert(4 * kWriteThreads <= kWriteThreads * 33, "the scan arrays fit in the slots");
  __shared__ uint32_t base[4];
  const int tid = threadIdx.x;
  const int g0 = blockIdx.x * kWriteThreads, g = g0 + tid;
  const DevImg* gimg = &A.imgs[A.sub_img[blockIdx.x]];
  const uint32_t first_bit = static_cast<uint32_t>(g0 - gimg->first_sub) * static_cast<uint32_t>(kSubBits);
  uint32_t* slot = slots + tid * 33;
#pragma unroll
  for (int q = 0; q < 32; ++q) slot[q] = 0u;
  if (tid < 4) base[tid] = 0u;
  load_record(&sh, gimg);
  load_stream(&sh, gimg, first_bit);
  const DevImg& I = sh.img;
  const uint32_t i = static_cast<uint32_t>(g - I.first_sub);
  const bool live = i < static_cast<uint32_t>(I.n_sub);
  {
    uint32_t acc[4] = {0u, 0u, 0u, 0u};
    for (int u = I.first_sub / kWriteThreads + tid; u < static_cast<int>(blockIdx.x); u += kWriteThreads)
      for (int c = 0; c < 4; ++c) acc[c] += A.half_total[4 * u + c];
    for (int c = 0; c < 4; ++c) if (acc[c]) atomicAdd(&base[c], acc[c]);
  }
  uint32_t mine[4];
  for (int c = 0; c < 4; ++c) { mine[c] = live ? A.tally[4 * g + c] : 0u; sc[c][tid] = mine[c]; }
  __syncthreads();
  for (int off = 1; off < kWriteThreads; off <<= 1) {
    uint32_t t[4];
    for (int c = 0; c < 4; ++c) t[c] = tid >= off ? sc[c][tid - off] : 0u;
    __syncthreads();
    for (int c = 0; c < 4; ++c) sc[c][tid] += t[c];
    __syncthreads();
  }
  uint32_t ex[4];
  for (int c = 0; c < 4; ++c) ex[c] = base[c] + sc[c][tid] - mine[c];
  __syncthreads();
  for (int k = tid; k < 4 * kWriteThreads; k += kWriteThreads) slots[k] = 0u;
  __syncthreads();
  if (!live) return;
  State S;
  if (i == 0) { S.p = 0; S.c = 0; S.z = 0; } else { S.p = A.p[g - 1]; S.c = A.cz[g - 1] >> 8; S.z = A.cz[g - 1] & 255u; }
  const uint64_t end = static_cast<uint64_t>(i + 1) * static_cast<uint64_t>(kSubBits);
  const uint32_t limit = static_cast<uint32_t>(end < static_cast<uint64_t>(I.bits) ? end : static_cast<uint64_t>(I.bits));
  run_write(&sh, first_bit, slot, S, limit, ex[0], static_cast<int32_t>(ex[1]), static_cast<int32_t>(ex[2]), static_cast<int32_t>(ex[3]));
}

}

int jpeg_gpu_entropy_decode(const std::vector<JpegGpuItem>& items, std::vector<uint8_t>* ok, void* stream_, DevBuf* scratch, int* launches) {
  hipStream_t stream = static_cast<hipStream_t>(stream_);
  if (launches) *launches = 0;
  const size_t n_img = items.size();
  static const bool timing = std::getenv("IST_TIMING") != nullptr;
  auto t_prev = std::chrono::steady_clock::now();
  auto lap = [&](const char* what) {
    if (!timing) return;
    (void)hipStreamSynchronize(stream);
    const auto t = std::chrono::steady_clock::now();
    std::fprintf(stderr, "[ist timing]   huffman/%-20s %7.2f ms\n", what, std::chrono::duration<double, std::milli>(t - t_prev).count());
    t_prev = t;
  };
  ok->assign(n_img, 0);
  if (n_img == 0) return IST_OK;
#define JG_HIP(e) do { const hipError_t e_ = (e); if (e_ != hipSuccess) return fail(IST_E_HIP, std::string(#e) + ": " + hipGetErrorString(e_)); } while (0)
  size_t off = 0;
  auto take = [&](size_t bytes) { const size_t at = off; off += (bytes + 255) & ~static_cast<size_t>(255); return at; };
  struct Unit { size_t item; uint32_t byte_off; };
  std::vector<Unit> units;
  std::vector<size_t> o_stream(n_img), o_tab(n_img), first_unit(n_img + 1);
  std::vector<DevImg> H;
  int64_t n_sub_total = 0;
  std::vector<char> skip(n_img, 0);
  {
    size_t total = 0;
    for (size_t k = 0; k < n_img; ++k) total += items[k].S->iv.empty() ? 1 : items[k].S->iv.size();
    while (total > 65535) {
      size_t worst = n_img, most = 1;
      for (size_t k = 0; k < n_img; ++k) if (!skip[k] && items[k].S->iv.size() > most) { most = items[k].S->iv.size(); worst = k; }
      if (worst == n_img) break;
      skip[worst] = 1; total -= most;
    }
  }
  for (size_t k = 0; k < n_img; ++k) {
    const JpegImage& J = *items[k].J; const JpegGpuScan& S = *items[k].S;
    first_unit[k] = units.size();
    if (skip[k]) { o_stream[k] = 0; continue; }
    if (S.bits >= (1ll << 32) - 65536) return fail(IST_E_UNSUPPORTED, "JPEG scan too large for the GPU entropy decoder");
    if (S.slots < 1 || S.slots > 10) return fail(IST_E_DECODE, "JPEG scan with more than 10 blocks per MCU");
    if (S.iv.empty() && S.stream.size() != static_cast<size_t>(S.bits / 8) + 16) return fail(IST_E_INVALID, "JPEG scan buffer without its padding");
    if (!S.iv.empty()) {
      int64_t at = 0;
      bool tiled = true;
      for (const JpegGpuInterval& V : S.iv) { tiled = tiled && V.n_mcus > 0 && static_cast<int64_t>(V.mcu0) == at; at += V.n_mcus; }
      if (!tiled || at != static_cast<int64_t>(J.mcus_x) * J.mcus_y) { skip[k] = 1; o_stream[k] = 0; continue; }
    }
    o_stream[k] = items[k].d_stream ? 0 : take(S.stream.size());
    const size_t n_units = S.iv.empty() ? 1 : S.iv.size();
    for (size_t u = 0; u < n_units; ++u) {
      DevImg I;
      std::memset(&I, 0, sizeof I);
      uint32_t byte_off = 0;
      if (S.iv.empty()) {
        I.bits = S.bits;
        I.total_blocks = J.mcus_x * J.mcus_y * S.slots;
      } else {
        const JpegGpuInterval& V = S.iv[u];
        if (V.byte_off % 256 != 0 || V.bits < 0 || V.bits % 8 != 0 || static_cast<size_t>(V.byte_off) + static_cast<size_t>(V.bits / 8) + 16 > S.stream.size() ||
            static_cast<int64_t>(V.mcu0) + V.n_mcus > static_cast<int64_t>(J.mcus_x) * J.mcus_y)
          return fail(IST_E_INVALID, "JPEG restart interval outside its scan");
        byte_off = V.byte_off;
        I.bits = V.bits;
        I.total_blocks = static_cast<int32_t>(V.n_mcus) * S.slots;
        I.mcu0 = static_cast<int32_t>(V.mcu0);
      }
      I.first_sub = static_cast<int32_t>(n_sub_total & 0x7fffffff);
      I.n_sub = static_cast<int32_t>((I.bits + kSubBits - 1) / kSubBits);
      if (I.n_sub < 1) I.n_sub = 1;
      n_sub_total += (static_cast<int64_t>(I.n_sub) + (kSyncThreads - 1)) & ~static_cast<int64_t>(kSyncThreads - 1);
      I.slots = S.slots; I.mcus_x = J.mcus_x;
      std::memcpy(I.slot_comp, S.slot_comp, 10); std::memcpy(I.slot_idx, S.slot_idx, 10);
      std::memcpy(I.dc_tab, S.dc_tab, 3); std::memcpy(I.ac_tab, S.ac_tab, 3);
      for (int c = 0; c < J.ncomp; ++c) {
        I.coef[c] = items[k].d_coef[c];
        I.h[c] = J.comp[c].h; I.v[c] = J.comp[c].v; I.blocks_x[c] = J.comp[c].blocks_x;
      }
      for (int c = J.ncomp; c < 3; ++c) I.h[c] = I.v[c] = 1;
      H.push_back(I);
      units.push_back(Unit{k, byte_off});
    }
  }
  first_unit[n_img] = units.size();
  const size_t n_unit = units.size();
  if (n_unit > 65535 || n_unit == 0) return IST_OK;
  if (n_sub_total >= (1ll << 31)) return fail(IST_E_UNSUPPORTED, "too much JPEG data for one GPU entropy-decode batch");
  const int ns = static_cast<int>(n_sub_total);
  const int n_half = ns / kWriteThreads;
  const size_t o_small = off;
  for (size_t k = 0; k < n_img; ++k) o_tab[k] = take(sizeof(items[k].S->tables));
  const size_t o_img = take(sizeof(DevImg) * n_unit), o_sub = take(2 * static_cast<size_t>(n_half));
  const size_t small_bytes = off - o_small;
  const size_t o_p0 = take(4 * static_cast<size_t>(ns)), o_p1 = take(4 * static_cast<size_t>(ns)), o_cz0 = take(4 * static_cast<size_t>(ns)), o_cz1 = take(4 * static_cast<size_t>(ns));
  const size_t o_sp = take(4 * static_cast<size_t>(ns)), o_scz = take(4 * static_cast<size_t>(ns));
  const size_t o_checks = take(24 * static_cast<size_t>(ns));
  const size_t o_tally = take(16 * static_cast<size_t>(ns)), o_half = take(16 * static_cast<size_t>(n_half)), o_flag = take(4), o_err = take(4 * n_unit);
  DevBuf one_off;
  DevBuf& block = scratch ? *scratch : one_off;
  if (block.grow(off, scratch ? off / 4 : 0)) return fail(IST_E_NOMEM, "out of device memory for the Huffman decoder");
  uint8_t* const d = static_cast<uint8_t*>(block.p);
  const size_t res_bytes = 256 + 16 * static_cast<size_t>(n_half) + 4 * n_unit;
  struct Pin { uint8_t* p; ~Pin() { if (p) pool_give(p); } } pin{static_cast<uint8_t*>(pool_take(small_bytes + res_bytes))};
  if (!pin.p) return fail(IST_E_NOMEM, "out of pinned host memory for the Huffman decoder");
  struct Idle { hipStream_t s; ~Idle() { (void)hipStreamSynchronize(s); } } idle{stream};
  uint8_t* hs = pin.p;
  volatile uint32_t* h_flag = reinterpret_cast<volatile uint32_t*>(pin.p + small_bytes);
  uint32_t* h_half = reinterpret_cast<uint32_t*>(pin.p + small_bytes + 256);
  uint32_t* h_err = h_half + 4 * static_cast<size_t>(n_half);
  std::memset(hs, 0, small_bytes);
  uint16_t* half_img = reinterpret_cast<uint16_t*>(hs + (o_sub - o_small));
  for (size_t k = 0; k < n_img; ++k) {
    const JpegGpuScan& S = *items[k].S;
    if (skip[k]) continue;
    if (!items[k].d_stream) JG_HIP(hipMemcpyAsync(d + o_stream[k], S.stream.data(), S.stream.size(), hipMemcpyHostToDevice, stream));
    std::memcpy(hs + (o_tab[k] - o_small), &S.tables, sizeof(S.tables));
  }
  for (size_t u = 0; u < n_unit; ++u) {
    const size_t k = units[u].item;
    H[u].stream = (items[k].d_stream ? items[k].d_stream : d + o_stream[k]) + units[u].byte_off;
    H[u].tables = reinterpret_cast<const JpegGpuTables*>(d + o_tab[k]);
    H[u].err = reinterpret_cast<uint32_t*>(d + o_err) + u;
    for (int i = 0; i < ((H[u].n_sub + (kSyncThreads - 1)) & ~(kSyncThreads - 1)); i += kWriteThreads) half_img[static_cast<size_t>((H[u].first_sub + i) / kWriteThreads)] = static_cast<uint16_t>(u);
  }
  JG_HIP(hipMemsetAsync(d + o_err, 0, 4 * n_unit, stream));
  std::memcpy(hs + (o_img - o_small), H.data(), sizeof(DevImg) * n_unit);
  JG_HIP(hipMemcpyAsync(d + o_small, hs, small_bytes, hipMemcpyHostToDevice, stream));
  lap("alloc + uploads");
  const DevImg* d_img = reinterpret_cast<const DevImg*>(d + o_img);
  const uint16_t* d_sub = reinterpret_cast<const uint16_t*>(d + o_sub);
  uint32_t* P[2] = {reinterpret_cast<uint32_t*>(d + o_p0), reinterpret_cast<uint32_t*>(d + o_p1)};
  uint32_t* CZ[2] = {reinterpret_cast<uint32_t*>(d + o_cz0), reinterpret_cast<uint32_t*>(d + o_cz1)};
  uint32_t* d_tally = reinterpret_cast<uint32_t*>(d + o_tally);
  uint32_t* d_half = reinterpret_cast<uint32_t*>(d + o_half);
  uint32_t* d_flag = reinterpret_cast<uint32_t*>(d + o_flag);
  int cur = 0, passes_run = 0;
  bool converged = false;
  for (int pass = 0; pass < kMaxPasses; ++pass) {
    passes_run = pass + 1;
    JG_HIP(hipMemsetAsync(d_flag, 0, 4, stream));
    SyncArgs A{d_img, d_sub, P[cur], CZ[cur], P[cur ^ 1], CZ[cur ^ 1], d_tally, reinterpret_cast<uint32_t*>(d + o_sp), reinterpret_cast<uint32_t*>(d + o_scz), reinterpret_cast<uint32_t*>(d + o_checks), d_half, d_flag, pass};
    hipLaunchKernelGGL(ist_jpeg_sync_kernel, dim3(static_cast<unsigned>(ns / kSyncThreads)), dim3(kSyncBlock), 0, stream, A);
    JG_HIP(hipGetLastError());
    cur ^= 1;
#ifdef IST_SYNC_DEBUG
    if (pass == 0) {
      JG_HIP(hipStreamSynchronize(stream));
      const unsigned nwg = std::min<unsigned>(8192u, static_cast<unsigned>(ns / kSyncThreads));
      std::vector<uint32_t> dbg(8 * static_cast<size_t>(nwg));
      JG_HIP(hipMemcpyFromSymbol(dbg.data(), HIP_SYMBOL(g_sync_dbg), dbg.size() * 4));
      std::vector<uint32_t> tot, p0, st, passes, longest, cyc, iters; uint64_t redo = 0; uint32_t tmin = 0, tmax = 0;
      for (unsigned w = 0; w < nwg; ++w) { const uint32_t* q = &dbg[8 * w]; if (!q[7]) continue; passes.push_back(q[0]); tot.push_back(q[1]); st.push_back(q[2]); p0.push_back(q[3]); longest.push_back(q[4]); redo += q[5];
        cyc.push_back(q[6]); iters.push_back(q[7] & 0xFFFFu); tmax += (q[7] >> 16) & 0x7FFFu; }
      auto pct = [](std::vector<uint32_t> v, double f) { std::sort(v.begin(), v.end()); return v.empty() ? 0u : v[static_cast<size_t>(f * (v.size() - 1))]; };
      std::fprintf(stderr, "[sync debug] %zu workgroups; ticks of 10 ns.  total p50 %u p90 %u max %u | staging p50 %u max %u | pass 0 p50 %u p90 %u max %u | passes p50 %u p90 %u max %u | longest later pass p50 %u max %u | lane re-decodes %llu | pass 0: clock64 ticks p50 %u, loop trips of the busiest lane p50 %u; misses (general step, all lanes of all workgroups, pass 0) %u\n",
                   tot.size(), pct(tot, .5), pct(tot, .9), pct(tot, 1.0), pct(st, .5), pct(st, 1.0), pct(p0, .5), pct(p0, .9), pct(p0, 1.0), pct(passes, .5), pct(passes, .9), pct(passes, 1.0),
                   pct(longest, .5), pct(longest, 1.0), static_cast<unsigned long long>(redo), pct(cyc, .5), pct(iters, .5), tmax - tmin);
    }
#endif
    if (pass == 0) continue;
    *h_flag = 1u;
    JG_HIP(hipMemcpyAsync(const_cast<uint32_t*>(h_flag), d_flag, 4, hipMemcpyDeviceToHost, stream));
    JG_HIP(hipStreamSynchronize(stream));
    tl_mark("huffman: synchronisation launch done, pass", static_cast<long>(pass));
    if (!*h_flag) { converged = true; break; }
  }
  if (launches) *launches = passes_run;
  if (timing) std::fprintf(stderr, "[ist timing] GPU Huffman: %d subsequences of %d bits, %s after %d launches\n", ns, kSubBits, converged ? "fixed point" : "NO fixed point", passes_run);
  if (!converged) { JG_HIP(hipStreamSynchronize(stream)); return IST_OK; }
  lap("sync passes");
  WriteArgs W{d_img, d_sub, P[cur], CZ[cur], d_tally, d_half};
  hipLaunchKernelGGL(ist_jpeg_write_kernel, dim3(static_cast<unsigned>(n_half)), dim3(kWriteThreads), 0, stream, W);
  JG_HIP(hipGetLastError());
  lap("write");
  const uint32_t* half = h_half; const uint32_t* err = h_err;
  JG_HIP(hipMemcpyAsync(h_half, d_half, 16 * static_cast<size_t>(n_half), hipMemcpyDeviceToHost, stream));
  JG_HIP(hipMemcpyAsync(h_err, d + o_err, 4 * n_unit, hipMemcpyDeviceToHost, stream));
  JG_HIP(hipStreamSynchronize(stream));
  tl_mark("huffman: writing pass done, validation read back");
  for (size_t k = 0; k < n_img; ++k) {
    bool good = !skip[k];
    for (size_t w = first_unit[k]; w < first_unit[k + 1]; ++w) {
      const DevImg& I = H[w];
      uint32_t blocks = 0;
      for (int u = I.first_sub / kWriteThreads; u < (I.first_sub + ((I.n_sub + (kSyncThreads - 1)) & ~(kSyncThreads - 1))) / kWriteThreads; ++u) blocks += half[4 * static_cast<size_t>(u)];
      good = good && blocks == static_cast<uint32_t>(I.total_blocks) && err[w] == 0;
    }
    (*ok)[k] = good ? 1 : 0;
  }
  lap("validation");
#undef JG_HIP
  return IST_OK;
}

}
// ... 1 lines not shown
```

imagestitching_amd/stitch.py:

```python
import ctypes as C
import os

import numpy as np

from . import _lib as L

_DIRECTIONS = {"vertical": L.VERTICAL, "horizontal": L.HORIZONTAL}
_MODES = {"min": L.MODE_MIN, "max": L.MODE_MAX, "original": L.MODE_ORIGINAL}
_FILTERS = {"nearest": L.FILTER_NEAREST, "bilinear": L.FILTER_BILINEAR, "area": L.FILTER_AREA, "cubic": L.FILTER_CUBIC}
FILTER_EDGE_AA = 0x100


def edge_aa_of(o):
    v = o.get("edgeAA")
    return (o.get("platform") is not None) if v is None else bool(v)


def _filter_of(o):
    return _FILTERS[o["filter"]] | (FILTER_EDGE_AA if edge_aa_of(o) else 0)
_PLATFORMS = {"ios": L.PLATFORM_IOS, "android": L.PLATFORM_ANDROID, "devtools": L.PLATFORM_OTHER,
              "windows": L.PLATFORM_OTHER, "mac": L.PLATFORM_OTHER, "other": L.PLATFORM_OTHER}

DEFAULT_OPTS = {
    "mode": "min",
# ... 518 lines not shown
        return
    st = stream if stream is not None else torch.cuda.current_stream(outs[0].device)
    handles = (C.c_void_p * n)(*[j._h for j in jobs])
    counts = (C.c_int * n)(*[j.n_images for j in jobs])
    total = max(1, sum(j.n_images for j in jobs))
    ptrs, pitches = (C.c_void_p * total)(), (C.c_size_t * total)()
    at = 0
    for j, ss in zip(jobs, srcs):
        if len(ss) > j.n_images:
            raise ValueError("launch_jobs: more sources than the job has images")
        for i, t in enumerate(ss):
            ptrs[at + i] = 0 if t is None else t.data_ptr()
            pitches[at + i] = 0 if t is None else t.stride(0)
        at += j.n_images
    dst = (C.c_void_p * n)(*[o.data_ptr() for o in outs])
    dpitch = (C.c_size_t * n)(*[o.stride(0) for o in outs])
    L.check(L.lib.ist_jobs_launch(handles, n, ptrs, pitches, counts, dst, dpitch, C.c_void_p(st.cuda_stream)))


def _take_pixels(out, w, h):
    import weakref
    raw = (C.c_uint8 * (w * h * 4)).from_address(C.addressof(out.contents))
    weakref.finalize(raw, L.lib.ist_free, C.cast(out, C.c_void_p))
    return np.frombuffer(raw, np.uint8).reshape(h, w, 4)


def render_ops(canvas_w, canvas_h, ops, n_ops, descs, srcs, filter="bilinear", clear=(0, 0, 0, 0), region=None, device=0):
    n = len(srcs)
    descs, ptrs, pitches, keep = _host_sources(srcs, descs=descs, holes=True)
    reg, rw, rh = None, int(canvas_w), int(canvas_h)
    if region is not None:
        x, y, w, h = [int(v) for v in region]
        reg = C.byref(L.Region(x, y, w, h))
        rw, rh = min(canvas_w, x + w) - max(0, x), min(canvas_h, y + h) - max(0, y)
    data = np.empty((rh, rw, 4), np.uint8)
    clr = (C.c_uint8 * 4)(*clear)
    f = (_FILTERS[filter] if isinstance(filter, str) else int(filter))
    L.check(L.lib.ist_render_rgba8(_ctx(device), int(canvas_w), int(canvas_h), clr, ops, int(n_ops), descs, ptrs, pitches, n,
                                   f, reg, data.ctypes.data, data.strides[0]))
    return data


def stitch_via_c_abi(images, direction, opts=None, device=0):
    r = stitch(images, direction, opts, device)
    if r is not None:
        r["data"] = r["data"].copy()
    return r


def _take_png(out, n, copy=True):
    if copy:
        try:
            return C.string_at(out, n.value)
        finally:
            L.lib.ist_free(out)
    import weakref
    arr = (C.c_uint8 * n.value).from_address(C.addressof(out.contents))
    weakref.finalize(arr, L.lib.ist_free, C.cast(out, C.c_void_p))
    return memoryview(arr).cast("B")


def decode_png(data):
    buf = bytes(data)
    w, h = C.c_int32(0), C.c_int32(0)
    L.check(L.lib.ist_png_info(buf, len(buf), C.byref(w), C.byref(h)))
    out = np.empty((h.value, w.value, 4), np.uint8)
    L.check(L.lib.ist_png_decode_rgba8(buf, len(buf), out.ctypes.data, out.strides[0], out.shape[0]))
    return out


def image_info(data):
    buf = bytes(data)
    w, h, o = C.c_int32(0), C.c_int32(0), C.c_int32(0)
    L.check(L.lib.ist_image_info(buf, len(buf), C.byref(w), C.byref(h), C.byref(o)))
    return w.value, h.value, o.value


_SCALES = (1, 2, 4, 8)


def scaled_size(w, h, scale):
    sw, sh = C.c_int32(0), C.c_int32(0)
    L.check(L.lib.ist_jpeg_scaled_size(int(w), int(h), int(scale), C.byref(sw), C.byref(sh)))
    return sw.value, sh.value


def decode_scale_fit(w, h, min_w, min_h):
    d = L.lib.ist_decode_scale_fit(int(w), int(h), int(min_w), int(min_h))
    L.check(d if d < 0 else 0)
    return d


def _scales(scale, blobs, who):
    n = len(blobs)
    ds = [int(d) for d in _per_file(scale, n, who + ": scale")]
    for i, d in enumerate(ds):
        if d not in _SCALES:
            raise L.StitchError(-1, "%s: the scale of image %d is %d, not 1, 2, 4 or 8" % (who, i, d))
    return ds, (None if all(d == 1 for d in ds) else (C.c_int32 * max(1, n))(*ds))


def _is_jpeg(buf):
    return buf[:2] == b"\xff\xd8"


def decode_image(data, device=0, scale=1, profile="ignore"):
    buf = bytes(data)
    _color_profile(profile)
    (d,), _ = _scales(scale, [buf], "decode_image")
    w, h, _ = image_info(buf)
    jpeg = _is_jpeg(buf)
    if jpeg and d > 1:
        w, h = scaled_size(w, h, d)
    out = np.empty((h, w, 4), np.uint8)
    ctx = _ctx_color(device, profile) if jpeg else None
    if d == 1:
        L.check(L.lib.ist_image_decode_rgba8(ctx, buf, len(buf), out.ctypes.data, out.strides[0], out.shape[0]))
    else:
        L.check(L.lib.ist_image_decode_rgba8_scaled(ctx, buf, len(buf), d, out.ctypes.data, out.strides[0], out.shape[0]))
    return out


def decode_files_device(blobs, device=0, out=None, scale=1, profile="ignore"):
    import torch
    n = len(blobs)
    _color_profile(profile)
    ds, cden = _scales(scale, blobs, "decode_files_device")
    sizes = [image_info(b) for b in blobs]
    sizes = [scaled_size(w, h, d) + (o,) if d > 1 and _is_jpeg(b) else (w, h, o) for (w, h, o), d, b in zip(sizes, ds, blobs)]
    dev = torch.device("cuda", device)
    if out is None:
        out = [torch.empty((h + 1, w, 4), dtype=torch.uint8, device=dev)[:h] for (w, h, _) in sizes]
    else:
        for d in {t.device for t in out}:
            torch.cuda.current_stream(d).synchronize()
    files = (C.c_char_p * n)(*blobs)
    lens = (C.c_int64 * n)(*[len(b) for b in blobs])
    dst, pitch, rows = (C.c_void_p * n)(), (C.c_size_t * n)(), (C.c_int64 * n)()
    for i, t in enumerate(out):
        dst[i], pitch[i], rows[i] = t.data_ptr(), t.stride(0), t.shape[0]
    descs = (L.ImageDesc * n)()
    ctx = _ctx_color(device, profile)
    if cden is None:
        L.check(L.lib.ist_decode_files_device(ctx, files, lens, n, dst, pitch, rows, descs))
    else:
        L.check(L.lib.ist_decode_files_device_scaled(ctx, files, lens, n, cden, dst, pitch, rows, descs))
    imgs = [{"width": d.width, "height": d.height, "orientation": d.orientation, "opaque": bool(d.opaque), "fileSize": d.file_size} for d in descs]
    for im, d in zip(imgs, descs):
        if d.bmp_width or d.bmp_height:
            im["bmpWidth"], im["bmpHeight"] = int(d.bmp_width), int(d.bmp_height)
    return out, imgs


def debug_jpeg_gpu_coefficients(blob, device=0):
    info = L.JpegCoefInfo()
    L.check(L.lib.ist_debug_jpeg_gpu_coefficients(None, blob, len(blob), None, None, C.byref(info)))
    planes = [np.zeros((info.blocks_y[c], info.blocks_x[c], 64), np.int16) for c in range(info.ncomp)]
    ptrs = (C.c_void_p * 3)(*[p.ctypes.data for p in planes])
    elems = (C.c_int64 * 3)(*[p.size for p in planes])
    L.check(L.lib.ist_debug_jpeg_gpu_coefficients(_ctx(device), blob, len(blob), ptrs, elems, C.byref(info)))
    return {"ok": bool(info.ok), "launches": int(info.launches), "planes": planes if info.ok else None}


PHASES = ("host_decode", "plan_arena", "entropy_gpu", "reconstruct", "stitch", "png", "d2h")


def last_phase_times(device=0):
    ms = (C.c_double * 8)()
    L.check(L.lib.ist_ctx_last_timing(_ctx(device), ms, 8))
    return {k: ms[i] for i, k in enumerate(PHASES)}


def set_phase_timing(on, device=0):
    L.check(L.lib.ist_ctx_set_timing(_ctx(device), 1 if on else 0))


def stitch_files(paths, direction, opts=None, out_path=None, device=0, copy=True):
    o = _merge(opts, color=True)
    form = _opts_png_form(o)
    _color_profile(o["colorProfile"])
    n = len(paths)
    if n == 0:
        return None
    cpaths = (C.c_char_p * n)(*[os.fsencode(p) for p in paths])
    cplan, out, ln = L.Plan(), C.POINTER(C.c_uint8)(), C.c_int64(0)
    pv = _preview_arg(o)
    fn = L.lib.ist_stitch_paths_png if pv is None else L.lib.ist_stitch_paths_png_preview
    _ctx_color(device, o["colorProfile"])
    size = _plan_size(L.check(fn(_ctx_png(device, form), cpaths, n, *_plan_args(direction, o), C.byref(cplan), C.byref(out), C.byref(ln),
                                 *([] if pv is None else [C.byref(pv)]))), cplan)
    if size is None:
        return None
    w, h = size
    res = {"width": w, "height": h, "png": _take_png(out, ln, copy)}
    if pv is not None:
        res["preview"] = _take_preview(pv)
    if out_path:
        with open(out_path, "wb") as f:
            f.write(res["png"])
    return res


def encode_png(pixels, device=0, level=None, color=None, row_filter=None, match=None):
    form = _png_form(level, color, row_filter, match)
    a, ptr, pitch = _host_rows(_rgba(pixels))
    out, n = C.POINTER(C.c_uint8)(), C.c_int64(0)
    L.check(L.lib.ist_png_encode_rgba8(_ctx_png(device, form), ptr, pitch, a.shape[1], a.shape[0], C.byref(out), C.byref(n)))
    return _take_png(out, n)


def stitch_png(images, direction, opts=None, device=0):
    o = _merge(opts, overlap=True)
    _opts_png_form(o)
    return _stitch(images, direction, o, device, "png")


def encode_png_device(canvas, out=None, stream=None, device=None, level=None, color=None, row_filter=None, match=None):
    form = _png_form(level, color, row_filter, match)
    import torch
    _check_canvas(canvas, "encode_png_device: ")
    h, w = int(canvas.shape[0]), int(canvas.shape[1])
    out, off, dst, cap = _file_out(out, L.lib.ist_png_bound(w, h), canvas.device)
    st = stream if stream is not None else torch.cuda.current_stream(canvas.device)
    n = C.c_int64(0)
    dev = canvas.device.index if device is None else device
    L.check(L.lib.ist_png_encode_device(_ctx_png(dev or 0, form), C.c_void_p(canvas.data_ptr()), canvas.stride(0), w, h,
                                        C.c_void_p(dst), cap, C.byref(n), C.c_void_p(st.cuda_stream)))
    return out[off:off + n.value], n.value


JPEG_SUBSAMPLING = {"444": 0, "420": 1}
JPEG_OPTIMIZE = 0x100


def _jpeg_args(quality, subsampling, optimize=False):
    if not isinstance(optimize, bool):
        raise TypeError("optimize: expected a bool")
    if isinstance(quality, bool) or not isinstance(quality, (int, np.integer)):
        raise TypeError("quality: expected an integer 1..100")
    if not 1 <= int(quality) <= 100:
        raise ValueError("quality must be 1..100")
    if str(subsampling) not in JPEG_SUBSAMPLING:
        raise ValueError("subsampling must be '420' or '444'")
    return int(quality), JPEG_SUBSAMPLING[str(subsampling)] | (JPEG_OPTIMIZE if optimize else 0)


def encode_jpeg(pixels, quality=90, subsampling="420", device=0, optimize=False):
    q, ss = _jpeg_args(quality, subsampling, optimize)
    a = _rgba(pixels)
    if a.shape[0] < 1 or a.shape[1] < 1:
        raise TypeError("expected an HxWx4 uint8 RGBA array")
    a, ptr, pitch = _host_rows(a, align=4)
    out, n = C.POINTER(C.c_uint8)(), C.c_int64(0)
    L.check(L.lib.ist_jpeg_encode_rgba8(_ctx(device), ptr, pitch, a.shape[1], a.shape[0], q, ss, C.byref(out), C.byref(n)))
    return _take_png(out, n)


def encode_jpeg_device(canvas, quality=90, subsampling="420", out=None, stream=None, optimize=False):
    import torch
    q, ss = _jpeg_args(quality, subsampling, optimize)
    _check_canvas(canvas, "encode_jpeg_device: ")
    h, w = int(canvas.shape[0]), int(canvas.shape[1])
    out, off, dst, cap = _file_out(out, L.lib.ist_jpeg_bound(w, h, ss), canvas.device)
    st = stream if stream is not None else torch.cuda.current_stream(canvas.device)
    n = C.c_int64(0)
    L.check(L.lib.ist_jpeg_encode_device(_ctx(canvas.device.index or 0), C.c_void_p(canvas.data_ptr()), canvas.stride(0), w, h, q, ss,
                                         C.c_void_p(dst), cap, C.byref(n), C.c_void_p(st.cuda_stream)))
    return out[off:off + n.value], n.value


def stitch_jpeg(images, direction, opts=None, device=0):
    opts = dict(opts or {})
    jpeg = _jpeg_args(opts.pop("quality", 90), opts.pop("subsampling", "420"), opts.pop("optimize", False))
    o = _merge(opts, overlap=True)
    _no_preview(o, "stitch_jpeg", "previews are built beside the PNG export")
    if o.get("devices") is not None:
        raise TypeError("stitch_jpeg: devices= does not apply (the JPEG export runs on one GPU)")
    return _stitch(images, direction, o, device, "jpeg", jpeg)


def _per_file(value, n, name):
    if isinstance(value, (list, tuple)):
        if len(value) != n:
            raise ValueError("%s: expected one value or a sequence of length %d, got %d" % (name, n, len(value)))
        return list(value)
    return [value] * n


def encode_jpeg_batch_device(canvases, quality=90, subsampling="420", outs=None, stream=None, optimize=False):
    canvases = list(canvases)
    n = len(canvases)
    if n == 0:
        return []
    args = []
    for k, (q, s, o) in enumerate(zip(_per_file(quality, n, "quality"), _per_file(subsampling, n, "subsampling"), _per_file(optimize, n, "optimize"))):
        try:
            args.append(_jpeg_args(q, s, o))
        except (TypeError, ValueError) as e:
            raise type(e)("file %d: %s" % (k, e)) from None
    qs, ss = (C.c_int * n)(*[a[0] for a in args]), (C.c_int * n)(*[a[1] for a in args])
    return _encode_batch_device(L.lib.ist_jpeg_encode_batch_device, _ctx, "encode_jpeg_batch_device", canvases,
                                lambda k, w, h: L.lib.ist_jpeg_bound(w, h, ss[k]), outs, stream, (qs, ss))


def stitch_jpeg_batch(requests, device=0):
    reqs = list(requests)
    if not reqs:
        return []
    n = len(reqs)
    plain, qs, ss = [], (C.c_int * n)(), (C.c_int * n)()
    for k, r in enumerate(reqs):
        if not isinstance(r, (tuple, list)) or len(r) not in (2, 3):
            raise TypeError("request %d: expected (images, direction) or (images, direction, opts)" % k)
        opts = dict(r[2] or {}) if len(r) == 3 else {}
# ... 472 lines not shown
```

include/imagestitch.h:

```cpp
#ifndef IMAGESTITCH_H_
#define IMAGESTITCH_H_

#include <stddef.h>
#include <stdint.h>

#ifdef __cplusplus
extern "C" {
#endif

#define IST_API __attribute__((visibility("default")))

#define IST_ABI_VERSION 2

enum {
  IST_OK = 0,
  IST_NOTHING_TO_DO = 1,
  IST_E_INVALID = -1,
  IST_E_SIZE_UNAVAILABLE = -2,
  IST_E_OUTPUT_SIZE = -3,
  IST_E_NO_CONTEXT = -4,
  IST_E_NO_DEVICE = -5,
  IST_E_DECODE = -6,
  IST_E_UNSUPPORTED = -7,
  IST_E_NOMEM = -8,
  IST_E_HIP = -9
};

enum { IST_VERTICAL = 0, IST_HORIZONTAL = 1 };
enum { IST_MODE_MIN = 0, IST_MODE_MAX = 1, IST_MODE_ORIGINAL = 2 };
enum { IST_PLATFORM_OTHER = 0, IST_PLATFORM_IOS = 1, IST_PLATFORM_ANDROID = 2 };
enum { IST_OP_FILL = 0, IST_OP_DRAW = 1, IST_OP_HOLE = 2 };
enum { IST_FILTER_NEAREST = 0, IST_FILTER_BILINEAR = 1, IST_FILTER_AREA = 2, IST_FILTER_CUBIC = 3 };
enum { IST_FILTER_EDGE_AA = 0x100 };

typedef struct ist_image_desc {
  int32_t width, height;
  int32_t orientation;
  int32_t bmp_width, bmp_height;
  int32_t opaque;
  int64_t file_size;
} ist_image_desc;

typedef struct ist_limits {
  int32_t platform;
  int32_t reserved;
  double max_side;
  double max_pixels;
  double max_super_sample;
} ist_limits;

typedef struct ist_rect {
  int32_t image, orientation;
  double dx, dy, dw, dh;
} ist_rect;

typedef struct ist_plan {
  double out_w, out_h;
  double scale_down;
  double super_sample;
  int64_t canvas_w, canvas_h;
  int32_t big_task;
  int32_t n_rects;
  ist_rect* rects;
} ist_plan;

typedef struct ist_op {
  int32_t kind, image;
  double m[6];
  double s[4];
  double d[4];
  uint8_t rgba[4];
  int32_t reserved;
} ist_op;

typedef struct ist_region { int32_t x, y, w, h; } ist_region;

typedef struct ist_job_info {
  int64_t canvas_w, canvas_h;
  int32_t n_ops, n_cells;
  int64_t n_tiles;
  int64_t out_pixels;
  int64_t src_pixels_touched;
  int64_t algorithmic_bytes;
  int64_t tiles_fill, tiles_copy, tiles_sample, tiles_general;
} ist_job_info;

typedef struct ist_ctx ist_ctx;
typedef struct ist_job ist_job;

IST_API int ist_abi_version(void);
IST_API const char* ist_last_error(void);
IST_API int ist_device_count(void);
IST_API int64_t ist_debug_device_allocs(void);
IST_API int ist_debug_live_handles(int64_t out[4]);
IST_API int64_t ist_debug_gpu_entropy_files(void);
IST_API int64_t ist_debug_gpu_entropy_sync_launches(void);
typedef struct ist_jpeg_coef_info {
  int32_t ok, launches, ncomp, reserved;
  int32_t blocks_x[3], blocks_y[3];
} ist_jpeg_coef_info;
IST_API int ist_debug_jpeg_gpu_coefficients(ist_ctx* ctx, const uint8_t* file, int64_t len, int16_t* const* planes, const int64_t* plane_elems,
                                            ist_jpeg_coef_info* info);
IST_API int64_t ist_debug_direct_images(void);
IST_API int64_t ist_debug_host_sink_stitches(void);
IST_API int64_t ist_debug_flat_launches(void);
IST_API int64_t ist_debug_duplex_stitches(void);
IST_API int64_t ist_debug_batch_launches(void);

IST_API void ist_limits_default(int platform, ist_limits* out);
IST_API void ist_limits_unlimited(ist_limits* out);
IST_API int ist_plan_compute(const ist_image_desc* images, int n_images, int direction, int mode, double gap,
                             const ist_limits* limits, ist_plan* out);
IST_API void ist_plan_free(ist_plan* plan);
IST_API int ist_plan_ops(const ist_plan* plan, const ist_image_desc* images, int n_images, ist_op* ops, int* n_ops);
IST_API int ist_op_box(const ist_op* op, int64_t canvas_w, int64_t canvas_h, int filter, int32_t box[4]);
typedef struct ist_flat_cell {
  int32_t path, image;
  int32_t X0, Y0, X1, Y1;
  int64_t src_offset;
  uint32_t bg;
  int32_t opaque;
} ist_flat_cell;
IST_API int ist_debug_flat_form(int64_t canvas_w, int64_t canvas_h, const uint8_t clear_rgba[4], const ist_op* ops, int n_ops,
                                const ist_image_desc* images, int n_images, int filter, const ist_region* clip, int64_t* pitch,
                                int64_t* dst_offset, ist_flat_cell* cells, int max_cells, int* n_cells);
enum { IST_PATH_FILL = 0, IST_PATH_COPY = 1, IST_PATH_SAMPLE = 2, IST_PATH_GENERAL = 3, IST_PATH_SAMPLE_LDS = 4, IST_PATH_SWAP_LDS = 5,
       IST_PATH_SAMPLE_STREAM = 6, IST_PATH_AREA_STREAM = 7, IST_PATH_CUBIC_STREAM = 8 };
typedef struct ist_debug_cell {
  int32_t path;
  int32_t tile_w, tile_h, sub_h;
  int32_t X0, Y0, X1, Y1;
  int64_t tiles;
} ist_debug_cell;
IST_API int ist_debug_cells(int64_t canvas_w, int64_t canvas_h, const uint8_t clear_rgba[4], const ist_op* ops, int n_ops,
                            const ist_image_desc* images, int n_images, int filter, const ist_region* clip, ist_debug_cell* cells,
                            int max_cells, int* n_cells, int* kernel_kind, int* tile_table);

enum { IST_SPLIT_IMAGE = 0, IST_SPLIT_BAND = 1, IST_SPLIT_ROWS = 2, IST_SPLIT_AUTO = 3 };
typedef struct ist_part {
  int32_t image, op;
  int32_t slot;
  int32_t X0, Y0, X1, Y1;
  int32_t sx0, sy0, sx1, sy1;
  int32_t in_place;
} ist_part;
IST_API int ist_shard_parts(const ist_op* ops, int n_ops, int64_t canvas_w, int64_t canvas_h, const ist_image_desc* images,
                            int n_images, int filter, int n_slots, int split, ist_part* parts, int max_parts, int* n_parts);
IST_API int ist_shard_row_cuts(int64_t canvas_h, int n_slots, int32_t* cuts);
IST_API int ist_shard_resolve(const ist_op* ops, int n_ops, int64_t canvas_w, int64_t canvas_h, const ist_image_desc* images,
                              int n_images, int filter, int split);

IST_API ist_ctx* ist_ctx_create(int device);
IST_API void ist_ctx_destroy(ist_ctx* ctx);
IST_API int ist_ctx_sync(ist_ctx* ctx);
IST_API int ist_ctx_set_png_level(ist_ctx* ctx, int level);
enum { IST_PNG_RGBA = 0, IST_PNG_RGB = 1 };
IST_API int ist_ctx_set_png_color(ist_ctx* ctx, int color);
enum { IST_PNG_FILTER_PAETH = 0, IST_PNG_FILTER_ADAPTIVE = 1 };
IST_API int ist_ctx_set_png_filter(ist_ctx* ctx, int filter);
enum { IST_PNG_MATCH_RUN = 0, IST_PNG_MATCH_WINDOW = 1 };
IST_API int ist_ctx_set_png_match(ist_ctx* ctx, int match);
IST_API ist_job* ist_job_create(ist_ctx* ctx, int64_t canvas_w, int64_t canvas_h, const uint8_t clear_rgba[4],
                                const ist_op* ops, int n_ops, const ist_image_desc* images, int n_images,
                                int filter, const ist_region* clip);
IST_API int ist_job_info_get(const ist_job* job, ist_job_info* out);
IST_API size_t ist_job_preferred_dst_pitch(const ist_job* job);
IST_API int ist_job_launch(ist_job* job, const void* const* src, const size_t* src_pitch, int n_images,
                           void* dst, size_t dst_pitch, void* stream);
IST_API int ist_jobs_launch(ist_job* const* jobs, int n_jobs, const void* const* src, const size_t* src_pitch, const int* n_images,
                            void* const* dst, const size_t* dst_pitch, void* stream);
IST_API void ist_job_destroy(ist_job* job);

IST_API int ist_stitch_rgba8(ist_ctx* ctx, const ist_image_desc* images, const uint8_t* const* src,
                             const size_t* src_pitch, int n_images, int direction, int mode, double gap,
                             const ist_limits* limits, int filter, ist_plan* out_plan, uint8_t** out_pixels);
typedef struct ist_stitch_request {
  const ist_image_desc* images;
  const uint8_t* const* src;
  const size_t* src_pitch;
  int32_t n_images;
  int32_t direction, mode;
  double gap;
  const ist_limits* limits;
  int32_t filter;
  int32_t reserved;
} ist_stitch_request;
IST_API int ist_stitch_rgba8_batch(ist_ctx* ctx, const ist_stitch_request* reqs, int n_reqs, ist_plan* out_plans, uint8_t** out_pixels);
IST_API int ist_render_rgba8(ist_ctx* ctx, int64_t canvas_w, int64_t canvas_h, const uint8_t clear_rgba[4],
                             const ist_op* ops, int n_ops, const ist_image_desc* images,
                             const uint8_t* const* src, const size_t* src_pitch, int n_images, int filter,
                             const ist_region* region, uint8_t* dst, size_t dst_pitch);
IST_API void ist_free(void* p);
IST_API void ist_pool_trim(void);

typedef struct ist_group ist_group;
typedef struct ist_group_job ist_group_job;
IST_API ist_group* ist_group_create(const int* devices, int ndev);
IST_API void ist_group_destroy(ist_group* g);
IST_API int ist_group_slots(const ist_group* g);
IST_API int ist_group_device(const ist_group* g, int slot);
IST_API ist_group_job* ist_group_job_create(ist_group* g, int64_t canvas_w, int64_t canvas_h, const uint8_t clear_rgba[4],
                                            const ist_op* ops, int n_ops, const ist_image_desc* images, int n_images, int filter,
                                            int split);
IST_API void ist_group_job_destroy(ist_group_job* job);
IST_API int ist_group_job_parts(const ist_group_job* job, ist_part* parts, int max_parts, int* n_parts);
IST_API int ist_group_job_launch(ist_group_job* job, const void* const* src, const size_t* src_pitch, int n_parts, void* dst,
                                 size_t dst_pitch);
IST_API int ist_group_sync(ist_group* g);
IST_API int ist_group_stitch_rgba8(ist_group* g, const ist_image_desc* images, const uint8_t* const* src, const size_t* src_pitch,
                                   int n_images, int direction, int mode, double gap, const ist_limits* limits, int filter,
                                   int split, ist_plan* out_plan, uint8_t** out_pixels);
IST_API int ist_stitch_rgba8_multi(const int* devices, int ndev, const ist_image_desc* images, const uint8_t* const* src,
                                   const size_t* src_pitch, int n_images, int direction, int mode, double gap,
                                   const ist_limits* limits, int filter, int split, ist_plan* out_plan, uint8_t** out_pixels);

IST_API int ist_png_info(const uint8_t* file, int64_t len, int32_t* width, int32_t* height);
IST_API int ist_png_decode_rgba8(const uint8_t* file, int64_t len, uint8_t* out, size_t out_pitch, int64_t out_rows);
IST_API int ist_jpeg_info(const uint8_t* file, int64_t len, int32_t* width, int32_t* height, int32_t* orientation);
IST_API int ist_jpeg_decode_rgba8(ist_ctx* ctx, const uint8_t* file, int64_t len, uint8_t* out, size_t out_pitch, int64_t out_rows);
IST_API int ist_image_info(const uint8_t* file, int64_t len, int32_t* width, int32_t* height, int32_t* orientation);
IST_API int ist_image_decode_rgba8(ist_ctx* ctx, const uint8_t* file, int64_t len, uint8_t* out, size_t out_pitch, int64_t out_rows);

IST_API int ist_decode_files_device(ist_ctx* ctx, const uint8_t* const* files, const int64_t* lens, int n_images,
                                    void* const* dst, const size_t* dst_pitch, const int64_t* dst_rows, ist_image_desc* out_descs);
enum { IST_PHASE_HOST_DECODE = 0, IST_PHASE_PLAN_ARENA = 1, IST_PHASE_ENTROPY_GPU = 2, IST_PHASE_RECONSTRUCT = 3, IST_PHASE_STITCH = 4,
       IST_PHASE_PNG = 5, IST_PHASE_D2H = 6, IST_PHASE_COUNT = 8 };
IST_API int ist_ctx_set_timing(ist_ctx* ctx, int on);
IST_API int ist_ctx_last_timing(ist_ctx* ctx, double* ms, int n);

IST_API int ist_jpeg_scaled_size(int32_t w, int32_t h, int32_t denom, int32_t* sw, int32_t* sh);
IST_API int ist_decode_scale_fit(int32_t w, int32_t h, int32_t min_w, int32_t min_h);
IST_API int ist_image_decode_rgba8_scaled(ist_ctx* ctx, const uint8_t* file, int64_t len, int32_t denom, uint8_t* out, size_t out_pitch,
                                          int64_t out_rows);
IST_API int ist_decode_files_device_scaled(ist_ctx* ctx, const uint8_t* const* files, const int64_t* lens, int n_images, const int32_t* denom,
                                           void* const* dst, const size_t* dst_pitch, const int64_t* dst_rows, ist_image_desc* out_descs);
IST_API int64_t ist_debug_jpeg_scaled_launches(void);

IST_API int ist_stitch_files_png(ist_ctx* ctx, const uint8_t* const* files, const int64_t* lens, int n_images,
                                 int direction, int mode, double gap, const ist_limits* limits, int filter,
                                 ist_plan* out_plan, uint8_t** out_png, int64_t* out_len);
IST_API int ist_stitch_paths_png(ist_ctx* ctx, const char* const* paths, int n_images,
                                 int direction, int mode, double gap, const ist_limits* limits, int filter,
                                 ist_plan* out_plan, uint8_t** out_png, int64_t* out_len);

IST_API int64_t ist_png_bound(int64_t w, int64_t h);
IST_API int ist_png_encode_device(ist_ctx* ctx, const void* canvas, size_t pitch, int64_t w, int64_t h, void* out,
                                  int64_t out_cap, int64_t* out_len, void* stream);
IST_API int ist_png_encode_batch_device(ist_ctx* ctx, const void* const* canvases, const size_t* pitch,
                                        const int64_t* w, const int64_t* h, int n, void* const* out,
                                        const int64_t* out_cap, int64_t* out_len, void* stream);
IST_API int64_t ist_debug_png_batch_launches(void);
IST_API int ist_png_encode_rgba8(ist_ctx* ctx, const uint8_t* pixels, size_t pitch, int64_t w, int64_t h,
                                 uint8_t** out_png, int64_t* out_len);
IST_API int ist_render_png(ist_ctx* ctx, int64_t canvas_w, int64_t canvas_h, const uint8_t clear_rgba[4],
                           const ist_op* ops, int n_ops, const ist_image_desc* images, const uint8_t* const* src,
// ... 127 lines not shown
```

Before: 820,400.

## Move JPEG scan byte de-stuffing from host threads onto the GPU

Uploads the raw JPEG entropy-coded scan and removes the 0xFF00 stuffing bytes on the device. It uses three kernels: a per-chunk count, a single-block prefix scan, and a compaction that writes the cleaned stream. The goal is to take the serial host pass that builds the de-stuffed stream off the decode critical path. In exchange it adds a synchronous readback of per-image kept counts and flags before the Huffman batch, plus a host fallback that re-parses any image the device path rejects.

```diff
diff --git a/imagestitching_amd/__init__.py b/imagestitching_amd/__init__.py
--- a/imagestitching_amd/__init__.py
+++ b/imagestitching_amd/__init__.py
@@ -1,6 +1,6 @@
 from ._lib import (FILTER_BILINEAR, FILTER_NEAREST, HORIZONTAL, VERTICAL, StitchError, last_error)
 from .stitch import (DEFAULT_OPTS, Bitmap, GroupJob, StitchGroup, Stitcher, StitchJob, StitchPlan, decode_files_device, decode_image, decode_png, encode_png, encode_png_batch_device, encode_png_device, encode_jpeg, encode_jpeg_device, encode_jpeg_batch_device, stitch_jpeg, stitch_jpeg_batch, image_info, last_phase_times, plan, set_phase_timing,
-                     launch_jobs, stitch, stitch_batch, stitch_files, stitch_png, stitch_png_batch, decode_bitmaps, upload_bitmap, preview_device, preview_fit, thumbnail_layout, thumbnails, thumbnails_device, debug_cells, debug_png_grid, debug_jpeg_gpu_coefficients, scaled_size, decode_scale_fit, thumbnails_from_files, find_overlaps, find_overlaps_device, overlap_rows, crop_overlaps, image_color, icc_tables, convert_color_device)
+                     launch_jobs, stitch, stitch_batch, stitch_files, stitch_png, stitch_png_batch, decode_bitmaps, upload_bitmap, preview_device, preview_fit, thumbnail_layout, thumbnails, thumbnails_device, debug_cells, debug_png_grid, debug_jpeg_gpu_coefficients, debug_jpeg_destuff, scaled_size, decode_scale_fit, thumbnails_from_files, find_overlaps, find_overlaps_device, overlap_rows, crop_overlaps, image_color, icc_tables, convert_color_device)
 
-__all__ = ["stitch", "stitch_batch", "launch_jobs", "stitch_png", "stitch_png_batch", "encode_png", "encode_png_device", "encode_png_batch_device", "encode_jpeg", "encode_jpeg_device", "stitch_jpeg", "decode_png", "decode_image", "decode_files_device", "image_info", "set_phase_timing", "last_phase_times", "stitch_files", "decode_bitmaps", "upload_bitmap", "preview_device", "preview_fit", "thumbnail_layout", "thumbnails", "thumbnails_device", "thumbnails_from_files", "find_overlaps", "find_overlaps_device", "overlap_rows", "crop_overlaps", "image_color", "icc_tables", "convert_color_device", "scaled_size", "decode_scale_fit", "debug_cells", "debug_png_grid", "debug_jpeg_gpu_coefficients", "Bitmap", "plan", "Stitcher", "StitchGroup", "GroupJob", "StitchJob", "StitchPlan", "StitchError",
+__all__ = ["stitch", "stitch_batch", "launch_jobs", "stitch_png", "stitch_png_batch", "encode_png", "encode_png_device", "encode_png_batch_device", "encode_jpeg", "encode_jpeg_device", "stitch_jpeg", "decode_png", "decode_image", "decode_files_device", "image_info", "set_phase_timing", "last_phase_times", "stitch_files", "decode_bitmaps", "upload_bitmap", "preview_device", "preview_fit", "thumbnail_layout", "thumbnails", "thumbnails_device", "thumbnails_from_files", "find_overlaps", "find_overlaps_device", "overlap_rows", "crop_overlaps", "image_color", "icc_tables", "convert_color_device", "scaled_size", "decode_scale_fit", "debug_cells", "debug_png_grid", "debug_jpeg_gpu_coefficients", "debug_jpeg_destuff", "Bitmap", "plan", "Stitcher", "StitchGroup", "GroupJob", "StitchJob", "StitchPlan", "StitchError",
            "DEFAULT_OPTS"]
diff --git a/imagestitching_amd/_lib.py b/imagestitching_amd/_lib.py
--- a/imagestitching_amd/_lib.py
+++ b/imagestitching_amd/_lib.py
@@ -125,6 +125,10 @@
     ("ist_debug_gpu_entropy_files", C.c_int64, []),
     ("ist_debug_gpu_entropy_sync_launches", C.c_int64, []),
     ("ist_debug_jpeg_gpu_coefficients", C.c_int, [C.c_void_p, C.c_char_p, C.c_int64, C.POINTER(C.c_void_p), C.POINTER(C.c_int64), C.POINTER(JpegCoefInfo)]),
+    ("ist_debug_gpu_destuffed_files", C.c_int64, []),
+    ("ist_debug_gpu_destuff_fallbacks", C.c_int64, []),
+    ("ist_debug_jpeg_destuff", C.c_int, [C.c_void_p, C.c_char_p, C.c_int64, C.c_void_p, C.c_int64, C.POINTER(C.c_int64), C.POINTER(C.c_int32)]),
+    ("ist_debug_jpeg_destuff_host", C.c_int, [C.c_char_p, C.c_int64, C.c_void_p, C.c_int64, C.POINTER(C.c_int64)]),
     ("ist_debug_direct_images", C.c_int64, []),
     ("ist_debug_host_sink_stitches", C.c_int64, []),
     ("ist_debug_flat_launches", C.c_int64, []),
diff --git a/imagestitching_amd/csrc/ist_ctx.h b/imagestitching_amd/csrc/ist_ctx.h
--- a/imagestitching_amd/csrc/ist_ctx.h
+++ b/imagestitching_amd/csrc/ist_ctx.h
@@ -29,6 +29,8 @@
   ist::DevBuf scratch_ent;
   std::vector<ist::Event> img_event;
   std::vector<ist::DevBuf> img_huff;
+  std::vector<ist::DevBuf> img_raw, img_meta;
+  ist::DevBuf destuff_res;
   std::unique_ptr<ist::WorkerPool> workers;
   std::vector<ist::ScanBuf> scan_bufs;
   std::vector<ist::ScanBuf> file_bufs;
diff --git a/imagestitching_amd/csrc/ist_decode.cpp b/imagestitching_amd/csrc/ist_decode.cpp
--- a/imagestitching_amd/csrc/ist_decode.cpp
+++ b/imagestitching_amd/csrc/ist_decode.cpp
@@ -16,6 +16,8 @@
 namespace {
 std::atomic<int64_t> g_gpu_entropy_files{0};
 std::atomic<int64_t> g_gpu_entropy_sync_launches{0};
+std::atomic<int64_t> g_gpu_destuffed_files{0};
+std::atomic<int64_t> g_gpu_destuff_fallbacks{0};
 
 void jpeg_layout(const JpegImage& J, size_t* off, JpegDevLayout* L, int denom = 1) {
   std::memset(L, 0, sizeof(*L));
@@ -209,13 +211,15 @@
   }
   if (ctx->img_huff.size() < static_cast<size_t>(n)) ctx->img_huff.resize(static_cast<size_t>(n));
   if (ctx->scan_bufs.size() < static_cast<size_t>(n)) ctx->scan_bufs.resize(static_cast<size_t>(n));
-  return IST_OK;
+  if (ctx->img_raw.size() < static_cast<size_t>(n)) ctx->img_raw.resize(static_cast<size_t>(n));
+  if (ctx->img_meta.size() < static_cast<size_t>(n)) ctx->img_meta.resize(static_cast<size_t>(n));
+  return ctx->destuff_res.grow(8 * static_cast<size_t>(std::max(n, kMaxImages)));
 }
 
 FileDecoder::FileDecoder(ist_ctx* ctx, const uint8_t* const* files, const int64_t* lens, int n, Phases* ph, int color_profile, const int32_t* denom)
     : ctx_(ctx), files_(files), lens_(lens), n_(n), ph_(ph), to_srgb_(color_profile == IST_COLOR_PROFILE_SRGB), denom_(denom), dec_(static_cast<size_t>(n)),
       on_gpu_(static_cast<size_t>(n), 0), taken_(static_cast<size_t>(n), 0), uploaded_(static_cast<size_t>(n), 0), started_(static_cast<size_t>(n), 0),
-      chroma_done_(static_cast<size_t>(n), 0), jo_(static_cast<size_t>(n)) {}
+      chroma_done_(static_cast<size_t>(n), 0), jo_(static_cast<size_t>(n)), raw_(static_cast<size_t>(n), 0) {}
 FileDecoder::~FileDecoder() {
   join_all();
   for (int i = 0; i < n_; ++i) if (started_[static_cast<size_t>(i)]) (void)hipStreamSynchronize(stream_of(i));
@@ -228,6 +232,8 @@
 int FileDecoder::headers() {
   static const bool gpu_huffman = std::getenv("IST_JPEG_HOST_HUFFMAN") == nullptr;
   gpu_huffman_ = gpu_huffman;
+  static const bool gpu_destuff = [] { const char* v = std::getenv("IST_JPEG_GPU_DESTUFF"); return !(tuning_mode() && v && !std::strcmp(v, "0")); }();
+  gpu_destuff_ = gpu_huffman && gpu_destuff;
   for (int i = 0; i < n_; ++i) {
     Dec& D = dec_[static_cast<size_t>(i)];
     const uint8_t* f = files_[i]; const int64_t len = lens_[i];
@@ -269,7 +275,9 @@
   join_all();
   int rc2 = first_error(); if (rc2) return rc2;
   for (int i = 0; i < n_; ++i) if (uploaded_[static_cast<size_t>(i)]) (void)hipStreamSynchronize(stream_of(i));
-  ph_->lap(IST_PHASE_HOST_DECODE, "decode on host threads (+ scan uploads)", nullptr);
+  rc2 = resolve_destuff(ctx_->stream); if (rc2) return rc2;
+  for (int i = 0; i < n_; ++i) if (uploaded_[static_cast<size_t>(i)]) (void)hipStreamSynchronize(stream_of(i));
+  ph_->lap(IST_PHASE_HOST_DECODE, "decode on host threads (+ scan uploads, de-stuffing)", nullptr);
   rc2 = huffman_all(ctx_->stream); if (rc2) return rc2;
   ph_->lap(IST_PHASE_ENTROPY_GPU, "entropy decode (GPU)", ctx_->stream);
   for (int i = 0; i < n_; ++i) { rc2 = take(i, ctx_->stream); if (rc2) return rc2; }
@@ -342,6 +350,8 @@
   join_all();
   tl_mark("decoder: host work of every image done");
   int rc = first_error();
+  if (rc) return rc;
+  rc = resolve_destuff(consumer);
   if (rc) return rc;
   huff_done_ = true;
   std::vector<JpegGpuItem> items; std::vector<int> who;
@@ -359,6 +369,7 @@
   }
   std::vector<uint8_t> okv;
   int launches = 0;
+  tl_mark("decoder: the Huffman batch starts");
   rc = jpeg_gpu_entropy_decode(items, &okv, consumer, &ctx_->scratch_huff, &launches);
   g_gpu_entropy_sync_launches.fetch_add(launches, std::memory_order_relaxed);
   if (rc) return rc;
@@ -394,8 +405,16 @@
     if (rc) failed(rc);
     return;
   }
+  scan_to_device(i, gpu_destuff_);
+}
+
+void FileDecoder::scan_to_device(int i, bool on_device) {
+  const size_t k = static_cast<size_t>(i);
+  Dec& D = dec_[k];
+  const uint8_t* f = files_[i]; const int64_t len = lens_[i];
+  auto failed = [&](int rc) { D.rc = rc; D.err = g_last_error; };
   JpegImage full;
-  if (k < ctx_->scan_bufs.size()) D.G.stream.swap(ctx_->scan_bufs[k]);
+  if (k < ctx_->scan_bufs.size() && D.G.stream.capacity() < ctx_->scan_bufs[k].capacity()) D.G.stream.swap(ctx_->scan_bufs[k]);
   static const bool flip = tuning_mode() && std::getenv("IST_JPEG_SECOND_READ_444") != nullptr;
   std::vector<uint8_t> flipped;
   if (flip) {
@@ -403,6 +422,8 @@
     for (int64_t q = 2; q + 12 < len; ++q) if (flipped[static_cast<size_t>(q)] == 0xFF && flipped[static_cast<size_t>(q) + 1] == 0xC0) { flipped[static_cast<size_t>(q) + 11] = 0x11; break; }
     f = flipped.data();
   }
+  D.G.eligible = false; D.G.raw = false; D.G.host_loop = false; D.G.want_raw = on_device;
+  auto left_the_path = [&]() { if (on_device) g_gpu_destuff_fallbacks.fetch_add(1, std::memory_order_relaxed); };
   const int rc = jpeg_parse_and_entropy_decode(f, len, &full, false, gpu_huffman_ ? &D.G : nullptr);
   if (rc) { failed(rc); return; }
   bool same = full.width == D.w && full.height == D.h && full.ncomp == D.J.ncomp && full.hmax == D.J.hmax && full.vmax == D.J.vmax &&
@@ -410,16 +431,65 @@
   for (int c = 0; same && c < full.ncomp; ++c)
     same = full.comp[c].h == D.J.comp[c].h && full.comp[c].v == D.J.comp[c].v && full.comp[c].blocks_x == D.J.comp[c].blocks_x &&
            full.comp[c].blocks_y == D.J.comp[c].blocks_y;
-  if (!same) { g_last_error = "JPEG frame header changed between two reads"; failed(IST_E_DECODE); return; }
+  if (!same) { left_the_path(); g_last_error = "JPEG frame header changed between two reads"; failed(IST_E_DECODE); return; }
   D.J = std::move(full);
+  if (D.G.host_loop) left_the_path();
   if (!D.G.eligible) return;
+  hipStream_t st = stream_of(i);
+  if (D.G.raw) {
+    raw_[k] = 1;
+    const size_t raw_len = static_cast<size_t>(D.G.scan_end - D.G.scan_begin), block = jpeg_destuff_block_bytes(raw_len), meta = jpeg_destuff_meta_bytes(raw_len);
+    if (ctx_->img_raw[k].grow(block, block / 4) || ctx_->img_huff[k].grow(block, block / 4) || ctx_->img_meta[k].grow(meta, meta / 4)) return;
+    started_[k] = 1;
+    if (hipMemcpyAsync(ctx_->img_raw[k].p, files_[i] + D.G.scan_begin, raw_len, hipMemcpyHostToDevice, st) != hipSuccess) { (void)hipGetLastError(); return; }
+    if (jpeg_launch_destuff(static_cast<const uint8_t*>(ctx_->img_raw[k].p), raw_len, static_cast<uint8_t*>(ctx_->img_huff[k].p), static_cast<uint32_t*>(ctx_->img_meta[k].p),
+                            static_cast<uint32_t*>(ctx_->destuff_res.p) + 2 * k, st) != IST_OK) return;
+    if (hipEventRecord(ctx_->img_event[k], st) != hipSuccess) { (void)hipGetLastError(); return; }
+    uploaded_[k] = 1;
+    return;
+  }
   const size_t bytes = D.G.stream.size();
   if (ctx_->img_huff[k].grow(bytes, bytes / 4)) return;
-  hipStream_t st = stream_of(i);
   started_[k] = 1;
   if (hipMemcpyAsync(ctx_->img_huff[k].p, D.G.stream.data(), bytes, hipMemcpyHostToDevice, st) != hipSuccess ||
       hipEventRecord(ctx_->img_event[k], st) != hipSuccess) { (void)hipGetLastError(); return; }
   uploaded_[k] = 1;
+}
+
+int FileDecoder::resolve_destuff(hipStream_t consumer) {
+  if (destuff_done_) return IST_OK;
+  join_all();
+  int rc = first_error();
+  if (rc) return rc;
+  destuff_done_ = true;
+  bool any = false, any_up = false;
+  for (int i = 0; i < n_; ++i) { any = any || raw_[static_cast<size_t>(i)]; any_up = any_up || (raw_[static_cast<size_t>(i)] && uploaded_[static_cast<size_t>(i)]); }
+  if (!any) return IST_OK;
+  struct Pin { uint32_t* p; ~Pin() { if (p) pool_give(p); } } pin{static_cast<uint32_t*>(pool_take(8 * static_cast<size_t>(n_)))};
+  if (!pin.p) return fail(IST_E_NOMEM, "out of pinned host memory for the de-stuffing results");
+  if (any_up) {
+    for (int i = 0; i < n_; ++i)
+      if (raw_[static_cast<size_t>(i)] && uploaded_[static_cast<size_t>(i)]) IST_HIP_OR(hipStreamWaitEvent(consumer, ctx_->img_event[static_cast<size_t>(i)], 0), "hipStreamWaitEvent failed");
+    const hipError_t e = hipMemcpyAsync(pin.p, ctx_->destuff_res.p, 8 * static_cast<size_t>(n_), hipMemcpyDeviceToHost, consumer);
+    const hipError_t e2 = hipStreamSynchronize(consumer);
+    if (e != hipSuccess || e2 != hipSuccess) { (void)hipGetLastError(); return fail(IST_E_HIP, "reading back the de-stuffing results failed"); }
+    tl_mark("decoder: de-stuffing results read back");
+  }
+  for (int i = 0; i < n_; ++i) {
+    const size_t k = static_cast<size_t>(i);
+    if (!raw_[k]) continue;
+    Dec& D = dec_[k];
+    const uint64_t raw_len = static_cast<uint64_t>(D.G.scan_end - D.G.scan_begin), kept = pin.p[2 * k], flag = pin.p[2 * k + 1];
+    if (uploaded_[k] && flag == 0 && kept <= raw_len && kept >= (raw_len + 1) / 2) {
+      D.G.destuffed = static_cast<int64_t>(kept); D.G.bits = static_cast<int64_t>(kept) * 8;
+      g_gpu_destuffed_files.fetch_add(1, std::memory_order_relaxed);
+      continue;
+    }
+    g_gpu_destuff_fallbacks.fetch_add(1, std::memory_order_relaxed);
+    raw_[k] = 0; uploaded_[k] = 0;
+    scan_to_device(i, false);
+  }
+  return first_error();
 }
 
 int check_denoms(const char* who, const int32_t* denom, int n) {
@@ -458,16 +528,68 @@
 
 int64_t ist_debug_gpu_entropy_files(void) { return g_gpu_entropy_files.load(std::memory_order_relaxed); }
 int64_t ist_debug_gpu_entropy_sync_launches(void) { return g_gpu_entropy_sync_launches.load(std::memory_order_relaxed); }
+int64_t ist_debug_gpu_destuffed_files(void) { return g_gpu_destuffed_files.load(std::memory_order_relaxed); }
+int64_t ist_debug_gpu_destuff_fallbacks(void) { return g_gpu_destuff_fallbacks.load(std::memory_order_relaxed); }
+
+int ist_debug_jpeg_destuff(ist_ctx* ctx, const uint8_t* file, int64_t len, uint8_t* out, int64_t cap, int64_t* out_len, int32_t* flag) {
+  if (!file || len <= 0 || !out_len || !flag || (out && cap < 0)) return fail(IST_E_INVALID, "ist_debug_jpeg_destuff: bad argument");
+  *out_len = 0; *flag = 0;
+  JpegImage J;
+  JpegGpuScan G;
+  G.want_raw = true;
+  int rc = jpeg_parse_and_entropy_decode(file, len, &J, false, &G);
+  if (rc) return rc;
+  if (!G.eligible || !G.raw) return fail(IST_E_UNSUPPORTED, "ist_debug_jpeg_destuff: not a file whose scan is de-stuffed on the device");
+  if (!ctx) return fail(IST_E_NO_CONTEXT, "无法获取绘图上下文");
+  std::lock_guard<std::mutex> lock(ctx->mu);
+  DeviceGuard g(ctx->device);
+  const size_t raw_len = static_cast<size_t>(G.scan_end - G.scan_begin), block = jpeg_destuff_block_bytes(raw_len);
+  size_t off = 0;
+  const size_t o_raw = arena_take(&off, block), o_out = arena_take(&off, block), o_meta = arena_take(&off, jpeg_destuff_meta_bytes(raw_len)), o_res = arena_take(&off, 8);
+  rc = ctx->scratch_arena.grow(off);
+  if (rc) return rc;
+  uint8_t* d = static_cast<uint8_t*>(ctx->scratch_arena.p);
+  uint32_t res[2] = {0, 0};
+  IST_HIP(hipMemcpyAsync(d + o_raw, file + G.scan_begin, raw_len, hipMemcpyHostToDevice, ctx->stream));
+  rc = jpeg_launch_destuff(d + o_raw, raw_len, d + o_out, reinterpret_cast<uint32_t*>(d + o_meta), reinterpret_cast<uint32_t*>(d + o_res), ctx->stream);
+  if (rc == IST_OK && hipMemcpyAsync(res, d + o_res, 8, hipMemcpyDeviceToHost, ctx->stream) != hipSuccess) { (void)hipGetLastError(); rc = fail(IST_E_HIP, "ist_debug_jpeg_destuff: readback failed"); }
+  IST_HIP(hipStreamSynchronize(ctx->stream));
+  if (rc) return rc;
+  if (res[0] > raw_len) return fail(IST_E_HIP, "ist_debug_jpeg_destuff: the device kept more bytes than the scan has");
+  *out_len = static_cast<int64_t>(res[0]) + 16; *flag = static_cast<int32_t>(res[1]);
+  if (!out) return IST_OK;
+  if (cap < *out_len) return fail(IST_E_INVALID, "ist_debug_jpeg_destuff: the output buffer is too small");
+  IST_HIP(hipMemcpy(out, d + o_out, static_cast<size_t>(*out_len), hipMemcpyDeviceToHost));
+  return IST_OK;
+}
+
+int ist_debug_jpeg_destuff_host(const uint8_t* file, int64_t len, uint8_t* out, int64_t cap, int64_t* out_len) {
+  if (!file || len <= 0 || !out_len || (out && cap < 0)) return fail(IST_E_INVALID, "ist_debug_jpeg_destuff_host: bad argument");
+  *out_len = 0;
+  JpegImage J;
+  JpegGpuScan G;
+  const int rc = jpeg_parse_and_entropy_decode(file, len, &J, false, &G);
+  if (rc) return rc;
+  if (!G.eligible || !G.iv.empty()) return fail(IST_E_UNSUPPORTED, "ist_debug_jpeg_destuff_host: not a file whose scan is one de-stuffed stream");
+  *out_len = static_cast<int64_t>(G.stream.size());
+  if (!out) return IST_OK;
+  if (cap < *out_len) return fail(IST_E_INVALID, "ist_debug_jpeg_destuff_host: the output buffer is too small");
+  std::memcpy(out, G.stream.data(), G.stream.size());
+  return IST_OK;
+}
 
 int ist_debug_jpeg_gpu_coefficients(ist_ctx* ctx, const uint8_t* file, int64_t len, int16_t* const* planes, const int64_t* plane_elems,
                                     ist_jpeg_coef_info* info) {
   if (!file || len <= 0 || !info || (planes && !plane_elems)) return fail(IST_E_INVALID, "ist_debug_jpeg_gpu_coefficients: bad argument");
+  const bool on_device = info->reserved == 1;
   std::memset(info, 0, sizeof *info);
   JpegImage J;
   JpegGpuScan G;
+  G.want_raw = on_device;
   int rc = jpeg_parse_and_entropy_decode(file, len, &J, false, &G);
   if (rc) return rc;
   if (!G.eligible) return fail(IST_E_UNSUPPORTED, "ist_debug_jpeg_gpu_coefficients: not a file the GPU entropy decoder takes");
+  if (on_device && !G.raw) return fail(IST_E_UNSUPPORTED, "ist_debug_jpeg_gpu_coefficients: not a file whose scan is de-stuffed on the device");
   info->ncomp = J.ncomp;
   for (int c = 0; c < J.ncomp; ++c) { info->blocks_x[c] = J.comp[c].blocks_x; info->blocks_y[c] = J.comp[c].blocks_y; }
   if (!planes) return IST_OK;
@@ -477,6 +599,8 @@
     if (!planes[c] || plane_elems[c] < 0 || static_cast<uint64_t>(plane_elems[c]) < nblk[c] * 64) return fail(IST_E_INVALID, "ist_debug_jpeg_gpu_coefficients: plane " + std::to_string(c) + " is too small");
     o_coef[c] = arena_take(&off, nblk[c] * 128);
   }
+  const size_t raw_len = G.raw ? static_cast<size_t>(G.scan_end - G.scan_begin) : 0, block = G.raw ? jpeg_destuff_block_bytes(raw_len) : 0;
+  const size_t o_raw = arena_take(&off, block), o_scan = arena_take(&off, block), o_meta = arena_take(&off, G.raw ? jpeg_destuff_meta_bytes(raw_len) : 0), o_res = arena_take(&off, 8);
   if (!ctx) return fail(IST_E_NO_CONTEXT, "无法获取绘图上下文");
   std::lock_guard<std::mutex> lock(ctx->mu);
   DeviceGuard g(ctx->device);
@@ -484,6 +608,17 @@
   if (rc) return rc;
   uint8_t* d = static_cast<uint8_t*>(ctx->scratch_arena.p);
   JpegGpuItem it; it.J = &J; it.S = &G;
+  if (G.raw) {
+    uint32_t res[2] = {0, 0};
+    IST_HIP(hipMemcpyAsync(d + o_raw, file + G.scan_begin, raw_len, hipMemcpyHostToDevice, ctx->stream));
+    rc = jpeg_launch_destuff(d + o_raw, raw_len, d + o_scan, reinterpret_cast<uint32_t*>(d + o_meta), reinterpret_cast<uint32_t*>(d + o_res), ctx->stream);
+    if (rc == IST_OK && hipMemcpyAsync(res, d + o_res, 8, hipMemcpyDeviceToHost, ctx->stream) != hipSuccess) { (void)hipGetLastError(); rc = fail(IST_E_HIP, "ist_debug_jpeg_gpu_coefficients: readback failed"); }
+    IST_HIP(hipStreamSynchronize(ctx->stream));
+    if (rc) return rc;
+    if (res[1] || res[0] > raw_len) return fail(IST_E_UNSUPPORTED, "ist_debug_jpeg_gpu_coefficients: the device flagged the scan (an FF that no 00 follows)");
+    G.destuffed = res[0]; G.bits = static_cast<int64_t>(res[0]) * 8;
+    it.d_stream = d + o_scan;
+  }
   for (int c = 0; c < 3; ++c) it.d_coef[c] = c < J.ncomp ? reinterpret_cast<int16_t*>(d + o_coef[c]) : nullptr;
   std::vector<JpegGpuItem> items(1, it);
   std::vector<uint8_t> okv;
diff --git a/imagestitching_amd/csrc/ist_decode.h b/imagestitching_amd/csrc/ist_decode.h
--- a/imagestitching_amd/csrc/ist_decode.h
+++ b/imagestitching_amd/csrc/ist_decode.h
@@ -44,6 +44,8 @@
   int huffman_all(hipStream_t consumer);
   int chroma_all(hipStream_t consumer);
   void worker(int i);
+  void scan_to_device(int i, bool on_device);
+  int resolve_destuff(hipStream_t consumer);
   int place(int i, hipStream_t consumer);
 
   ist_ctx* ctx_; const uint8_t* const* files_; const int64_t* lens_; int n_; Phases* ph_; const bool to_srgb_; const int32_t* denom_;
@@ -52,7 +54,8 @@
   std::vector<char> on_gpu_, taken_, uploaded_, started_, chroma_done_;
   std::vector<JpegDevLayout> jo_;
   uint8_t* arena_ = nullptr; uint8_t* const* img_ = nullptr; const size_t* pitch_ = nullptr;
-  bool gpu_huffman_ = true, huff_done_ = false, chroma_batch_done_ = false;
+  std::vector<char> raw_;
+  bool gpu_huffman_ = true, gpu_destuff_ = true, destuff_done_ = false, huff_done_ = false, chroma_batch_done_ = false;
 };
 
 int check_denoms(const char* who, const int32_t* denom, int n);
diff --git a/imagestitching_amd/csrc/ist_jpeg.cpp b/imagestitching_amd/csrc/ist_jpeg.cpp
--- a/imagestitching_amd/csrc/ist_jpeg.cpp
+++ b/imagestitching_amd/csrc/ist_jpeg.cpp
@@ -297,6 +297,16 @@
         const uint32_t ri = static_cast<uint32_t>(restart_interval);
         const uint32_t n_iv = ri ? (total_mcus + ri - 1) / ri : 0;
         bool in_sequence = n_iv <= kMaxGpuIntervals;
+        gs->raw = false;
+        if (gs->want_raw && !ri && qe - q > 2 && qe[-2] == 0xFF && qe[-1] == 0xD9) {
+          gs->raw = true; gs->scan_begin = q - f; gs->scan_end = n - 2;
+          gs->stream.clear(); gs->bits = 0; gs->destuffed = 0;
+          gs->eligible = true;
+          pos = n - 2;
+          J->scans++;
+          continue;
+        }
+        gs->host_loop = true;
         gs->stream.clear();
         if (in_sequence && !gs->stream.reserve(static_cast<size_t>(qe - q) + static_cast<size_t>(n_iv) * 272 + 32)) return fail(IST_E_NOMEM, "out of memory for the JPEG scan");
         uint8_t* const base = gs->stream.data();
@@ -342,6 +352,7 @@
           if (gs->iv.size() != n_iv) in_sequence = false;
         }
         if (in_sequence) {
+          gs->destuffed = static_cast<int64_t>(out - base);
           if (ri) {
             gs->bits = static_cast<int64_t>(out - base) * 8;
           } else {
diff --git a/imagestitching_amd/csrc/ist_jpeg.h b/imagestitching_amd/csrc/ist_jpeg.h
--- a/imagestitching_amd/csrc/ist_jpeg.h
+++ b/imagestitching_amd/csrc/ist_jpeg.h
@@ -92,6 +92,9 @@
   std::vector<JpegGpuInterval> iv;
   ScanBuf stream;
   int64_t bits = 0;
+  int64_t destuffed = 0;
+  bool want_raw = false, raw = false, host_loop = false;
+  int64_t scan_begin = 0, scan_end = 0;
   int slots = 0;
   uint8_t slot_comp[10], slot_idx[10];
   uint8_t dc_tab[3], ac_tab[3];
@@ -131,6 +134,11 @@
 int jpeg_gpu_entropy_decode(const std::vector<JpegGpuItem>& items, std::vector<uint8_t>* ok, void* stream, DevBuf* scratch = nullptr,
                             int* launches = nullptr);
 
+constexpr size_t kDestuffChunk = 4096;
+inline size_t jpeg_destuff_block_bytes(size_t raw_len) { return (raw_len + 32 + 255) & ~static_cast<size_t>(255); }
+inline size_t jpeg_destuff_meta_bytes(size_t raw_len) { return 12 * ((raw_len + kDestuffChunk - 1) / kDestuffChunk) + 256; }
+int jpeg_launch_destuff(const uint8_t* d_raw, size_t raw_len, uint8_t* d_out, uint32_t* d_meta, uint32_t* d_result, void* stream);
+
 }
 
 #endif
diff --git a/imagestitching_amd/csrc/ist_jpeg_destuff.hip b/imagestitching_amd/csrc/ist_jpeg_destuff.hip
--- /dev/null
+++ b/imagestitching_amd/csrc/ist_jpeg_destuff.hip
@@ -0,0 +1,135 @@
+#include <hip/hip_runtime.h>
+
+#include <string>
+
+#include "ist_internal.h"
+#include "ist_jpeg.h"
+
+namespace ist {
+namespace {
+
+constexpr int kThreads = 256, kPerLane = 16;
+static_assert(kThreads * kPerLane == static_cast<int>(kDestuffChunk), "one lane per 16 bytes of a chunk");
+
+__device__ __forceinline__ void classify(const uint8_t* __restrict__ raw, uint32_t len, uint32_t pos, uint32_t w[4], uint32_t* valid,
+                                         uint32_t* drop, uint32_t* flag) {
+  *valid = 0; *drop = 0;
+  if (pos >= len) { w[0] = w[1] = w[2] = w[3] = 0; return; }
+  const uint4 v = *reinterpret_cast<const uint4*>(raw + pos);
+  w[0] = v.x; w[1] = v.y; w[2] = v.z; w[3] = v.w;
+  const uint32_t n = min(len - pos, static_cast<uint32_t>(kPerLane));
+  uint32_t prev = pos > 0 ? raw[pos - 1] : 0u, d = 0, f = 0;
+#pragma unroll
+  for (int j = 0; j < kPerLane; ++j) {
+    const uint32_t b = (w[j >> 2] >> (8 * (j & 3))) & 0xFFu;
+    if (static_cast<uint32_t>(j) < n) {
+      if (prev == 0xFFu) { if (b == 0u) d |= 1u << j; else f = 1u; }
+      prev = b;
+    }
+  }
+  if (pos + n == len && prev == 0xFFu) f = 1u;
+  *valid = n; *drop = d; *flag |= f;
+}
+
+__global__ void __launch_bounds__(kThreads) ist_jpeg_destuff_count_kernel(const uint8_t* __restrict__ raw, uint32_t len, uint32_t* __restrict__ cnt,
+                                                                          uint32_t* __restrict__ flg) {
+  __shared__ uint32_t s_cnt, s_flag;
+  if (threadIdx.x == 0) { s_cnt = 0; s_flag = 0; }
+  __syncthreads();
+  uint32_t w[4], valid, drop, flag = 0;
+  classify(raw, len, blockIdx.x * static_cast<uint32_t>(kDestuffChunk) + threadIdx.x * kPerLane, w, &valid, &drop, &flag);
+  if (drop) atomicAdd(&s_cnt, static_cast<uint32_t>(__popc(drop)));
+  if (flag) atomicOr(&s_flag, 1u);
+  __syncthreads();
+  if (threadIdx.x == 0) { cnt[blockIdx.x] = s_cnt; flg[blockIdx.x] = s_flag; }
+}
+
+__device__ __forceinline__ uint32_t block_inclusive_sum(uint32_t v, uint32_t* s) {
+  s[threadIdx.x] = v;
+  __syncthreads();
+  for (int d = 1; d < kThreads; d <<= 1) {
+    const uint32_t add = static_cast<int>(threadIdx.x) >= d ? s[threadIdx.x - d] : 0u;
+    __syncthreads();
+    s[threadIdx.x] += add;
+    __syncthreads();
+  }
+  const uint32_t r = s[threadIdx.x];
+  __syncthreads();
+  return r;
+}
+
+__global__ void __launch_bounds__(kThreads) ist_jpeg_destuff_scan_kernel(const uint32_t* __restrict__ cnt, const uint32_t* __restrict__ flg, uint32_t n_chunks,
+                                                                         uint32_t len, uint32_t* __restrict__ at, uint32_t* __restrict__ result) {
+  __shared__ uint32_t s[kThreads];
+  __shared__ uint32_t s_flag;
+  if (threadIdx.x == 0) s_flag = 0;
+  __syncthreads();
+  uint32_t carry = 0, flag = 0;
+  for (uint32_t base = 0; base < n_chunks; base += kThreads) {
+    const uint32_t c = base + threadIdx.x;
+    const uint32_t mine = c < n_chunks ? cnt[c] : 0u;
+    if (c < n_chunks) flag |= flg[c];
+    const uint32_t incl = block_inclusive_sum(mine, s);
+    if (c < n_chunks) at[c] = c * static_cast<uint32_t>(kDestuffChunk) - (carry + incl - mine);
+    s[threadIdx.x] = incl;
+    __syncthreads();
+    carry += s[kThreads - 1];
+    __syncthreads();
+  }
+  if (flag) atomicOr(&s_flag, 1u);
+  __syncthreads();
+  if (threadIdx.x == 0) { result[0] = len - carry; result[1] = s_flag; }
+}
+
+__global__ void __launch_bounds__(kThreads) ist_jpeg_destuff_compact_kernel(const uint8_t* __restrict__ raw, uint32_t len, const uint32_t* __restrict__ at,
+                                                                            uint8_t* __restrict__ out, uint32_t out_cap) {
+  __shared__ uint32_t s[kThreads];
+  __shared__ uint32_t s_stage[(kDestuffChunk + 16) / 4];
+  uint8_t* const stage = reinterpret_cast<uint8_t*>(s_stage);
+  uint32_t w[4], valid, drop, flag = 0;
+  classify(raw, len, blockIdx.x * static_cast<uint32_t>(kDestuffChunk) + threadIdx.x * kPerLane, w, &valid, &drop, &flag);
+  const uint32_t kept = valid - static_cast<uint32_t>(__popc(drop));
+  const uint32_t incl = block_inclusive_sum(kept, s);
+  uint32_t o = incl - kept;
+#pragma unroll
+  for (int j = 0; j < kPerLane; ++j)
+    if (static_cast<uint32_t>(j) < valid && !((drop >> j) & 1u)) stage[o++] = static_cast<uint8_t>(w[j >> 2] >> (8 * (j & 3)));
+  s[threadIdx.x] = incl;
+  __syncthreads();
+  uint32_t total = s[kThreads - 1];
+  if (blockIdx.x == gridDim.x - 1) {
+    if (threadIdx.x < 16) stage[total + threadIdx.x] = 0;
+    total += 16;
+    __syncthreads();
+  }
+  const uint32_t base = at[blockIdx.x];
+  if (base > out_cap || total > out_cap - base) return;
+  const uint32_t head = min(total, (4u - (base & 3u)) & 3u);
+  const uint32_t n_dw = (total - head) >> 2, tail = (total - head) & 3u;
+  if (threadIdx.x < head) out[base + threadIdx.x] = stage[threadIdx.x];
+  uint32_t* const out_dw = reinterpret_cast<uint32_t*>(out + base + head);
+  for (uint32_t d = threadIdx.x; d < n_dw; d += kThreads) {
+    const uint8_t* p = stage + head + 4 * d;
+    out_dw[d] = static_cast<uint32_t>(p[0]) | (static_cast<uint32_t>(p[1]) << 8) | (static_cast<uint32_t>(p[2]) << 16) | (static_cast<uint32_t>(p[3]) << 24);
+  }
+  if (threadIdx.x < tail) out[base + head + 4 * n_dw + threadIdx.x] = stage[head + 4 * n_dw + threadIdx.x];
+}
+
+}
+
+int jpeg_launch_destuff(const uint8_t* d_raw, size_t raw_len, uint8_t* d_out, uint32_t* d_meta, uint32_t* d_result, void* stream) {
+  if (!d_raw || !d_out || !d_meta || !d_result || raw_len < 1 || raw_len > (size_t{1} << 28)) return fail(IST_E_INVALID, "jpeg_launch_destuff: bad argument");
+  hipStream_t st = static_cast<hipStream_t>(stream);
+  const uint32_t len = static_cast<uint32_t>(raw_len);
+  const uint32_t n_chunks = static_cast<uint32_t>((raw_len + kDestuffChunk - 1) / kDestuffChunk);
+  uint32_t* cnt = d_meta; uint32_t* flg = d_meta + n_chunks; uint32_t* at = d_meta + 2 * static_cast<size_t>(n_chunks);
+  hipLaunchKernelGGL(ist_jpeg_destuff_count_kernel, dim3(n_chunks), dim3(kThreads), 0, st, d_raw, len, cnt, flg);
+  hipLaunchKernelGGL(ist_jpeg_destuff_scan_kernel, dim3(1), dim3(kThreads), 0, st, cnt, flg, n_chunks, len, at, d_result);
+  hipLaunchKernelGGL(ist_jpeg_destuff_compact_kernel, dim3(n_chunks), dim3(kThreads), 0, st, d_raw, len, at, d_out,
+                     static_cast<uint32_t>(jpeg_destuff_block_bytes(raw_len)));
+  const hipError_t e = hipGetLastError();
+  if (e != hipSuccess) return fail(IST_E_HIP, std::string("JPEG de-stuffing launch: ") + hipGetErrorString(e));
+  return IST_OK;
+}
+
+}
diff --git a/imagestitching_amd/csrc/ist_jpeg_gpu.hip b/imagestitching_amd/csrc/ist_jpeg_gpu.hip
--- a/imagestitching_amd/csrc/ist_jpeg_gpu.hip
+++ b/imagestitching_amd/csrc/ist_jpeg_gpu.hip
@@ -600,7 +600,8 @@
     if (skip[k]) { o_stream[k] = 0; continue; }
     if (S.bits >= (1ll << 32) - 65536) return fail(IST_E_UNSUPPORTED, "JPEG scan too large for the GPU entropy decoder");
     if (S.slots < 1 || S.slots > 10) return fail(IST_E_DECODE, "JPEG scan with more than 10 blocks per MCU");
-    if (S.iv.empty() && S.stream.size() != static_cast<size_t>(S.bits / 8) + 16) return fail(IST_E_INVALID, "JPEG scan buffer without its padding");
+    if (S.iv.empty() && (S.destuffed != S.bits / 8 || (S.stream.empty() ? !items[k].d_stream : S.stream.size() != static_cast<size_t>(S.destuffed) + 16)))
+      return fail(IST_E_INVALID, "JPEG scan buffer without its padding");
     if (!S.iv.empty()) {
       int64_t at = 0;
       bool tiled = true;
diff --git a/imagestitching_amd/stitch.py b/imagestitching_amd/stitch.py
--- a/imagestitching_amd/stitch.py
+++ b/imagestitching_amd/stitch.py
@@ -694,14 +694,27 @@
     return out, imgs
 
 
-def debug_jpeg_gpu_coefficients(blob, device=0):
+def debug_jpeg_gpu_coefficients(blob, device=0, device_destuff=False):
     info = L.JpegCoefInfo()
     L.check(L.lib.ist_debug_jpeg_gpu_coefficients(None, blob, len(blob), None, None, C.byref(info)))
     planes = [np.zeros((info.blocks_y[c], info.blocks_x[c], 64), np.int16) for c in range(info.ncomp)]
     ptrs = (C.c_void_p * 3)(*[p.ctypes.data for p in planes])
     elems = (C.c_int64 * 3)(*[p.size for p in planes])
+    info.reserved = 1 if device_destuff else 0
     L.check(L.lib.ist_debug_jpeg_gpu_coefficients(_ctx(device), blob, len(blob), ptrs, elems, C.byref(info)))
     return {"ok": bool(info.ok), "launches": int(info.launches), "planes": planes if info.ok else None}
+
+
+def debug_jpeg_destuff(blob, device=0, host=False):
+    n, flag = C.c_int64(0), C.c_int32(0)
+    if host:
+        L.check(L.lib.ist_debug_jpeg_destuff_host(blob, len(blob), None, 0, C.byref(n)))
+        buf = np.zeros(n.value, np.uint8)
+        L.check(L.lib.ist_debug_jpeg_destuff_host(blob, len(blob), buf.ctypes.data, buf.size, C.byref(n)))
+        return buf[:n.value].tobytes(), False
+    buf = np.zeros(len(blob) + 16, np.uint8)
+    L.check(L.lib.ist_debug_jpeg_destuff(_ctx(device), blob, len(blob), buf.ctypes.data, buf.size, C.byref(n), C.byref(flag)))
+    return buf[:n.value].tobytes(), bool(flag.value)
 
 
 PHASES = ("host_decode", "plan_arena", "entropy_gpu", "reconstruct", "stitch", "png", "d2h")
diff --git a/include/imagestitch.h b/include/imagestitch.h
--- a/include/imagestitch.h
+++ b/include/imagestitch.h
@@ -101,6 +101,10 @@
 } ist_jpeg_coef_info;
 IST_API int ist_debug_jpeg_gpu_coefficients(ist_ctx* ctx, const uint8_t* file, int64_t len, int16_t* const* planes, const int64_t* plane_elems,
                                             ist_jpeg_coef_info* info);
+IST_API int64_t ist_debug_gpu_destuffed_files(void);
+IST_API int64_t ist_debug_gpu_destuff_fallbacks(void);
+IST_API int ist_debug_jpeg_destuff(ist_ctx* ctx, const uint8_t* file, int64_t len, uint8_t* out, int64_t cap, int64_t* out_len, int32_t* flag);
+IST_API int ist_debug_jpeg_destuff_host(const uint8_t* file, int64_t len, uint8_t* out, int64_t cap, int64_t* out_len);
 IST_API int64_t ist_debug_direct_images(void);
 IST_API int64_t ist_debug_host_sink_stitches(void);
 IST_API int64_t ist_debug_flat_launches(void);
```

Result: no change. 814,600 (-0.7%).
